# drscotthawley/flocoder

Hardware: AMD Instinct MI355X
Metric: latent samples/sec (64-step Euler, SD-VAE 4x32x32) (higher is better)
Workload: dtype f32; 1 GPU; flowers_sd.yaml shape: 64-step legacy Euler, batch 64 per GPU, latents 4x32x32, U-Net dim=32 dim_mults [1,2,4,8] n_classes=102, class-conditional, no CFG, ODE loop only (no VAE decode); global_batch=64, parallelism=sample-shard x1, weights broadcast once, plan_entries_per_forward=59, kernel_launches_per_forward=68, kernel_launches_per_euler_step=66, plan=exclusive device (cross-workgroup Block tails)

## Files before the change

### flocoder_amd/_binding.py

```python
from __future__ import annotations

import ctypes as C
import os
from typing import Optional

_HERE = os.path.dirname(os.path.abspath(__file__))
LIB_PATH = os.environ.get("FLOCODER_AMD_LIB") or os.path.join(_HERE, "_lib", "libflocoder_amd.so")

FC_OK, FC_E_ARG, FC_E_SHAPE, FC_E_ARCH, FC_E_HIP, FC_E_STATE = 0, -1, -2, -3, -4, -5
FC_METHOD_EULER, FC_METHOD_RK4 = 0, 1
FC_JACOBIAN_IDENTITY, FC_JACOBIAN_EXACT = 0, 1
FC_SDE_EULER_MARUYAMA, FC_SDE_HEUN = 0, 1
FC_LL_MAX_PROBES = 64
FC_PROBE_RADEMACHER, FC_PROBE_GAUSSIAN = 0, 1
FC_HIST_LDS_BINS = 8192
TILE_AUTO = -1
TILES = {"M128N32": 0, "M128N64": 1, "M64N32K2": 2, "M32N32K4": 3, "M64N64K2": 4, "M256N64": 5}


class fc_unet_config(C.Structure):
    _fields_ = [("dim", C.c_int), ("channels", C.c_int), ("n_levels", C.c_int), ("dim_mults", C.c_int * 8),
                ("groups", C.c_int), ("n_classes", C.c_int), ("mask_cond", C.c_int)]


_vp, _i, _f, _i64 = C.c_void_p, C.c_int, C.c_float, C.c_int64
_pi, _pf = C.POINTER(C.c_int), C.POINTER(C.c_float)

SIGNATURES = {
    "fc_abi_version": (_i, []),
    "fc_last_error": (C.c_char_p, []),
    "fc_check_device": (_i, [_i]),
    "fc_unet_create": (_i, [C.POINTER(fc_unet_config), _i, C.POINTER(_vp)]),
    "fc_unet_destroy": (None, [_vp]),
    "fc_unet_param_count": (_i, [_vp]),
    "fc_unet_param_info": (_i, [_vp, _i, C.POINTER(C.c_char_p), C.POINTER(_i64 * 4), C.POINTER(_i64)]),
    "fc_unet_param_numel": (_i64, [_vp]),
    "fc_unet_load_params": (_i, [_vp, _vp, _i64, _i, _vp]),
    "fc_unet_reserve": (_i, [_vp, _i, _i, _i]),
    "fc_unet_reserved": (_i, [_vp, _pi, _pi, _pi]),
    "fc_unet_forward": (_i, [_vp, _vp, _vp, _vp, _vp, _i, _vp, _i, _i, _i, _vp]),
    "fc_unet_integrate": (_i, [_vp, _i, _vp, _i, _i, _i, _pf, _i, _f, _f, _vp, _f, _vp, _i, _vp]),
    "fc_unet_integrate_rk45": (_i, [_vp, _vp, _i, _i, _i, C.c_double, C.c_double, C.c_double, C.c_double, _f, _vp, _f, _vp, _i, _pi, _vp]),
    "fc_unet_integrate_rk45_per_sample": (_i, [_vp, _vp, _i, _i, _i, C.c_double, C.c_double, C.c_double, C.c_double, _f, _vp, _f, _vp, _i,
                                              _pi, _vp]),
    "fc_unet_integrate_rk45_dense": (_i, [_vp, _i, _vp, _i, _i, _i, C.c_double, C.c_double, C.c_double, C.c_double, _f, _vp, _f, _vp, _i,
                                         C.POINTER(C.c_double), _i, _vp, _pi, _vp]),
    "fc_unet_chains": (_i, [_vp, _pi]),
    "fc_unet_plan_launches": (_i, [_vp]),
    "fc_unet_flops_per_sample": (C.c_double, [_vp]),
    "fc_unet_op_info": (_i, [_vp, _i, C.POINTER(C.c_char_p), C.POINTER(C.c_char_p), C.POINTER(C.c_double)]),
    "fc_unet_profile_ops": (_i, [_vp, _i, _i, _pf, _i, _vp]),
    "fc_unet_set_time_freqs": (_i, [_vp, _pf, _i]),
    "fc_unet_debug_tensor": (_i, [_vp, C.c_char_p, C.POINTER(_vp), _pi, _pi, _pi]),
    "fc_debug_copy": (_i, [_vp, _vp, _i64, _vp]),
    "fc_debug_set_poison": (_i, [_i]),
    "fc_debug_poison_check": (_i, [_pi, _pi]),
    "fc_debug_set_conv_stamps": (_i, [_vp]),
    "fc_debug_set_stamp_op": (_i, [_i, _vp]),
    "fc_debug_conv_routes": (_i, [_i]),
    "fc_debug_conv_routes_read": (_i, [C.c_char_p, _i]),
    "fc_debug_linattn_routes_read": (_i, [C.c_char_p, _i]),
    "fc_debug_conv": (_i, [_vp, _i, _vp, _i, _vp, _vp, _vp, _vp, _vp, _i, _pi, _pf, _i, _i, _i, _i, _i, _i, _i, _i, _i, _i, _i, _pf, _vp]),
    "fc_debug_set_fused_tail": (_i, [_i]),
    "fc_unet_fused_tail_errors": (_i, [_vp, C.POINTER(_i)]),
    "fc_unet_set_shared": (_i, [_vp, _i]),
    "fc_unet_meeting_launches": (_i, [_vp]),
    "fc_unet_check": (_i, [_vp, _vp, _i]),
    "fc_debug_unet_break_meeting": (_i, [_vp]),
    "fc_debug_unet_break_meeting_kind": (_i, [_vp, _i]),
    "fc_unet_train_reserve": (_i, [_vp, _i, _i, _i]),
    "fc_unet_backward": (_i, [_vp, _vp, _vp, _vp, _vp, _vp, _i64, _i, _i, _i, _vp]),
    "fc_unet_backward_ex": (_i, [_vp, _vp, _vp, _vp, _vp, _i, _vp, _vp, _i64, _vp, _vp, _i, _i, _i, _vp]),
    "fc_unet_backward_parts": (_i, [_vp, _vp, _vp, _vp, _vp, _i, _vp, _vp, _i64, _vp, _vp, _i, _i, _i, _i, _i, _vp]),
    "fc_unet_backward_accumulate": (_i, [_vp, _vp, _vp, _vp, _vp, _i, _vp, _vp, _i64, _vp, _vp, _i, _i, _i, _i, _i, _vp]),
    "fc_unet_grad_buckets": (_i, [_vp, C.POINTER(_i64)]),
    "fc_unet_set_grad_buckets": (_i, [_vp, _i]),
    "fc_unet_backward_launches": (_i, [_vp]),
    "fc_unet_backward_op_info": (_i, [_vp, _i, C.POINTER(C.c_char_p), C.POINTER(C.c_char_p)]),
    "fc_unet_vjp_x": (_i, [_vp, _vp, _vp, _vp, _vp, _i, _vp, _vp, _i, _i, _i, _vp]),
    "fc_unet_vjp_launches": (_i, [_vp]),
    "fc_unet_train_form": (_i, [_vp]),
    "fc_unet_train_release": (_i, [_vp]),
    "fc_unet_vjp_op_info": (_i, [_vp, _i, C.POINTER(C.c_char_p), C.POINTER(C.c_char_p)]),
    "fc_unet_log_likelihood": (_i, [_vp, _vp, _i, _i, _i, _pf, _i, _f, _vp, _vp, _i, _vp, _vp, _vp, _vp]),
    "fc_unet_log_likelihood_rk45": (_i, [_vp, _vp, _i, _i, _i, C.c_double, C.c_double, C.c_double, C.c_double, _f, _vp, _vp, _i, _vp, _i, _vp,
                                         _vp, _pi, _vp]),
    "fc_unet_log_likelihood_probes": (_i, [_vp, _vp, _i, _i, _i, _pf, _i, _f, _vp, _vp, _i, _vp, _i, _vp, _vp, _vp, _vp, _vp]),
    "fc_unet_log_likelihood_rk45_probes": (_i, [_vp, _vp, _i, _i, _i, C.c_double, C.c_double, C.c_double, C.c_double, _f, _vp, _vp, _i, _vp,
                                                _i, _i, _vp, _vp, _vp, _vp, _pi, _vp]),
    "fc_ode_probe_field": (_i, [_vp, _i, C.c_uint64, _i64, _vp, _i, _i64, _vp]),
    "fc_debug_probe_dot": (_i, [_vp, _vp, _vp, _i, _i64, _vp]),
    "fc_unet_integrate_guided": (_i, [_vp, _vp, _i, _i, _i, _pf, _i, _f, _vp, _f, _vp, _i, _vp, _vp, _f, _f, _i, _vp]),
    "fc_ode_guided_correct": (_i, [_vp, _vp, _vp, _vp, _i64, _f, _f, _f, _vp, _vp]),
    "fc_unet_integrate_sde": (_i, [_vp, _i, _vp, _i, _i, _i, _pf, _i, _f, _vp, _f, _vp, _i, _f, C.c_uint64, _vp, _vp, _vp]),
    "fc_ode_normal_field": (_i, [_vp, C.c_uint64, _i64, _vp, _i, _i64, _vp]),
    "fc_inpaint_masks": (_i, [_vp, _vp, C.c_uint64, _vp, _i, _i, _i, _pi, C.POINTER(C.c_double), _i, _i, _vp]),
    "fc_augment_images": (_i, [_vp, _vp, _vp, _i, _vp, _i, _i, _pf, _pf, _pf, _vp]),
    "fc_augment_midi": (_i, [_vp, _vp, _vp, _i, _vp, _i, _i, _i, _i, _f, _vp]),
    "fc_note_confusion": (_i, [_vp, _i, _vp, _i, _vp, _i, _i, _i, _f, C.c_double, _i, C.c_double, _i, _i, _vp, _vp, _vp, _vp, _vp]),
    "fc_index_histogram": (_i, [_vp, _i64, _i, _i, _vp, _vp, _vp, _vp]),
    "fc_debug_unet_guided_buffers": (_i, [_vp, C.POINTER(_vp), C.POINTER(_vp), C.POINTER(_vp), C.POINTER(_vp)]),
    "fc_unet_arena_serial": (C.c_uint64, [_vp]),
    "fc_unet_class_param_range": (_i, [_vp, C.POINTER(_i64), C.POINTER(_i64)]),
    "fc_flow_interp": (_i, [_vp, _vp, _vp, _vp, _vp, _i, _i64, _vp]),
    "fc_flow_prepare": (_i, [_vp, _vp, _vp, _vp, _f, _f, _f, _vp, _i, _vp, _vp, _vp, _vp, _vp, _i, _i64, _vp]),
    "fc_flow_prepare_rows": (_i, [_vp, _vp, _vp, _vp, _f, _f, _f, _vp, _i, _vp, _vp, _vp, _vp, _vp, _i, _i, _i, _i64, _vp]),
    "fc_mse_loss_grad_scaled": (_i, [_vp, _vp, _vp, _vp, _vp, _i64, _f, _vp]),
    "fc_mse_loss_grad": (_i, [_vp, _vp, _vp, _vp, _vp, _i64, _vp]),
    "fc_grad_clip_coef": (_i, [_vp, _i64, _vp, _i64, C.c_float, _vp, _vp, _vp]),
    "fc_adam_ema_step": (_i, [_vp, _vp, _vp, _vp, _vp, _i64, _vp, C.c_float, C.c_float, C.c_float, C.c_float, _i, C.c_float, _i, _vp]),
    "fc_adam_ema_step_guarded": (_i, [_vp, _vp, _vp, _vp, _vp, _i64, _vp, C.c_float, C.c_float, C.c_float, C.c_float, _i, C.c_float, _i, _vp, _vp]),
    "fc_debug_conv_wgrad": (_i, [_vp, _i, _vp, _i, _vp, _i, _i, _i, _i, _i, _i, _i, _i, _vp, _vp, _vp]),
    "fc_debug_conv_wgrad_ex": (_i, [_vp, _i, _vp, _i, _vp, _i, _i, _i, _i, _i, _i, _i, _i, _vp, _vp, _i, _i, _pi, _pi, _pi, _vp]),
    "fc_vae_create": (_i, [_i, C.POINTER(_vp)]),
# ... 101 lines not shown
```

### flocoder_amd/csrc/common.h

```cpp
#pragma once
#include <hip/hip_runtime.h>
#include <stdint.h>
#include <string>
#include <vector>

#include "../../include/flocoder_amd.h"

namespace fc {

void set_error(const std::string& msg);
int fail(int code, const std::string& msg);

#define FC_HIP(expr)                                                                              \
    do {                                                                                          \
        hipError_t _e = (expr);                                                                   \
        if (_e != hipSuccess)                                                                     \
            return ::fc::fail(FC_E_HIP, std::string(#expr) + ": " + hipGetErrorString(_e));       \
    } while (0)

#define FC_TRY(expr)                \
    do {                            \
        int _r = (expr);            \
        if (_r != FC_OK) return _r; \
    } while (0)

int dev_alloc(void** out, size_t bytes, const char* tag);
void dev_free(void* p);

static inline int ilog2(int v) { int l = 0; while ((1 << l) < v) ++l; return l; }
static inline bool is_pow2(int v) { return v > 0 && (v & (v - 1)) == 0; }
static inline int cdiv(int a, int b) { return (a + b - 1) / b; }

struct StatsRef {
    float* p = nullptr;
    int G = 0, T = 0;
    float n_t = 0.f;
};

struct SrcXform {
    int mode = 0;
    const float* stats = nullptr;
    int G = 1, T = 1;
    float n_t = 1.f;
    const float* gamma = nullptr;
    const float* beta = nullptr;
    const float* ss = nullptr;
    int ss_stride = 0;
    float eps = 1e-5f;
};

struct ConvSrc {
    const float* p = nullptr;
    int C = 0;
    SrcXform xf;
};

struct ConvFin {
    const float* gamma = nullptr;
    const float* beta = nullptr;
    float eps = 1e-5f;
    const float* res = nullptr;
    float* gn1_out = nullptr;
    unsigned* sync = nullptr;
    unsigned long long* gran = nullptr;
    int* err = nullptr;
};

struct ConvArgs {
    ConvSrc s0, s1;
    const float* w = nullptr;
    const float* bias = nullptr;
    float* out = nullptr;
    int out_act = 0;
    const float* add = nullptr;
    float* stats_out = nullptr;
    int Gout = 0;
    int stats_post = 0;
    const float* res_w = nullptr;
    const float* res_b = nullptr;
    float* res_out = nullptr;
    int B = 0, H = 0, W = 0;
    int Hs = 0, Ws = 0;
    int Cin = 0, Cout = 0;
    int KS = 1, pad = 0, stride = 1, ups = 0;
    int w_batch_stride = 0;
    const float* w4 = nullptr;
    const float* res_w4 = nullptr;
    const float* w_b3 = nullptr;
    int pad_y = -1, pad_x = -1;
    int out_sh = 0, out_oy = 0, out_ox = 0;
    int stats_tmul = 1, stats_toff = 0;
    int par4 = 0;
    int split_long_k = 0;
    int prec = 0;
    ConvFin fin;
};

enum ConvTile { TILE_AUTO = -1, TILE_M128N32 = 0, TILE_M128N64 = 1, TILE_M64N32K2 = 2, TILE_M32N32K4 = 3, TILE_M64N64K2 = 4,
                TILE_M256N64 = 5, TILE_COUNT = 6 };

struct ConvGeom {
    int tile = 0, grid = 0, T = 0, pipe = 0;
    float n_t = 0.f;
    size_t lds = 0;
    int T1 = 0;
    float n_t1 = 0.f;
    int groups = 0;
    int fin_local = 0;
};
bool conv_fin_possible(const ConvArgs& a, int tile);
int conv_init();
unsigned long long* conv_stamp_buffer();
void conv_set_stamp_buffer(unsigned long long* p);
void conv_route_log_set(bool on);
std::string conv_route_log_get();
int conv_plan(const ConvArgs& a, int tile, ConvGeom* g);
int conv_launch(const ConvArgs& a, int tile, hipStream_t s);

struct FinalizeArgs {
    const float* h = nullptr;
    SrcXform xf;
    const float* res = nullptr;
    SrcXform xf_res;
    int act_after_add = 0;
    float* y = nullptr;
    float* stats_out = nullptr;
    int B = 0, HW = 0, C = 0;
};
int finalize_blocks_per_sample(int HW, int C);
int finalize_launch(const FinalizeArgs& a, hipStream_t s);
size_t finalize_lds_bytes(const FinalizeArgs& a);
int finalize_table_launch(const FinalizeArgs* jobs_dev, const int* bps_dev, const int2* blocks_dev, int nblocks, size_t lds_bytes, hipStream_t s);
int gn_stats_launch(const float* x_nhwc, float* stats , int B, int HW, int C, int G, hipStream_t s);
int gn_fold_launch(const float* in, float* out, int B, int G, int T, float n_t, hipStream_t s);

struct CondFetch {
    const float* all = nullptr;
    const int* evalc = nullptr;
    float* dst = nullptr;
    int n4 = 0;
};

int init_conv_launch(const CondFetch& fetch, const float* x_nchw, int x_batch_mod, const float* w , const float* bias, float* out_nhwc,
                     int B, int Cin, int HW, int Cout, hipStream_t s);
struct EulerTail {
    int* evalc = nullptr;
    float* y = nullptr;
    float dt = 0.f;
    int* step = nullptr;
    const float* ts = nullptr;
    float t_scale = 1.f;
    float* sc = nullptr;
    float* tvec = nullptr;
    int rows = 0;
};
int final_conv_launch(const float* x_nhwc, const float* w , const float* bias, float* out_nchw, int B, int Cin,
                      int HW, int Cout, const EulerTail& tail, hipStream_t s);
int nchw_to_nhwc_launch(const float* src, float* dst, int B, int C, int HW, int Cpad, int src_batch_mod, hipStream_t s);
int nhwc_to_nchw_launch(const float* src, float* dst, int B, int C, int HW, int Cpad, hipStream_t s);
int pixel_shuffle2_nhwc_launch(const float* src, float* dst, int B, int H, int W, int C, hipStream_t s);
int bilinear_nhwc_launch(const float* src, float* dst, int B, int C, int Hs, int Ws, int Hd, int Wd, hipStream_t s);

struct TembArgs {
    const float* time = nullptr;
    const int64_t* class_ids = nullptr;
    int class_batch_mod = 0;
    int null_from = 0;
    int rows_per_eval = 0;
    const float* freqs = nullptr;
    const float *w1t, *b1, *w2t, *b2;
    const float *emb, *cw1t, *cb1, *cw2t, *cb2;
    int n_classes = 0;
    float* t_out = nullptr;
    int B = 0, dim = 0, td = 0;
};
int temb_init();
int temb_launch(const TembArgs& a, float* h, float* c1, hipStream_t s);
int ss_launch(const float* t, const float* wt, const float* bias, float* ss, int B, int td, int S, hipStream_t s);

int linattn_ctx_launch(const float* qkv, float* ctx , int B, int n, int heads, hipStream_t s);
int linattn_apply_launch(const float* qkv, const float* ctx, float* out , int B, int n, int heads,
                         hipStream_t s);
struct LaArgs {
    const float* x = nullptr;
    SrcXform xf;
    const float* wqkv = nullptr;
    const float* wout = nullptr;
    const float* wqkv4 = nullptr;
    const float* bout = nullptr;
    float* ctx = nullptr;
    float* y = nullptr;
    float* stats_out = nullptr;
    int B = 0, n = 0, C = 0, heads = 4;
    const float* g2 = nullptr;
    const float* b2 = nullptr;
    float eps2 = 1e-5f;
    float* out = nullptr;
    float* part = nullptr;
    unsigned long long* gran = nullptr;
    unsigned* sync = nullptr;
    int* err = nullptr;
};
int linattn_fused_init();
bool linattn_fused_supported(int n, int C, int heads);
int linattn_fused_tiles(int n);
float linattn_fused_nt(int n, int C);
int linattn_fused_launch(const LaArgs& a, hipStream_t s);
void linattn_route_log_set(bool on);
std::string linattn_route_log_get();
bool linattn_fused_meeting_ok(int B, int n, int C);
int linattn_sample_init();
bool linattn_sample_supported(int n, int C, int heads);
int linattn_sample_launch(const LaArgs& a, hipStream_t s);
bool attn_sample_supported(int n, int C, int heads);
int attn_sample_launch(const LaArgs& a, hipStream_t s);
int rope_attn_launch(const float* x, const float* wq, const float* bq, const float* wk, const float* bk, const float* wv, const float* bv,
                     const float* wo, const float* bo, float* out, int B, int n, int C, int Cr, hipStream_t s);
int attn_small_launch(const float* qkv, float* out, int B, int n, int heads, hipStream_t s);

int na2d_launch(const float* qkv, float* out, const float* gamma, int B, int H, int W, int C, int heads, int ksize, int mode, hipStream_t s);

int ode_all_times_launch(const float* ts, int n_steps, int rk4 , float t_scale, float* tv_out, hipStream_t s);
int ode_time_launch(int* step, const float* ts, float t_scale, int rk4, float* sc, float* tvec, int rows, hipStream_t s);
int ode_euler_update_launch(float* x, const float* v2, int n, int cfg_on, float cfg, float dt, hipStream_t s);
struct Rk4Guide { const float *gsc, *xin, *ym, *keep, *q; int tcur; };
int ode_rk4_stage_launch(const float* sc, const float* y, float* xs, float* k_out, const float* v2, int n, int cfg_on, float cfg,
                         int full, int tsel, float t_scale, float* tvec, int rows, const Rk4Guide* g, hipStream_t s);
int ode_rk4_final_launch(const float* sc, float* y, const float* k1, const float* k2, const float* k3, const float* v2, int n,
                         int cfg_on, float cfg, const Rk4Guide* g, hipStream_t s);
int ode_guide_w_launch(const float* sc, const float* gsc, const float* v, const float* xin, const float* ym, const float* keep, float* w,
                       int n, int tcur, hipStream_t s);
int ode_guided_correct_launch(const float* v, const float* x, const float* ym, const float* keep, float* out, int n, float t, float s2,
                              float gamma, hipStream_t s);
int ode_ll_stage_launch(const float* sc, const float* y, float* xs, float* k_out, const float* v, const float* g, const float* eps,
                        double* dst, int slot, int B, int m, int full, int tsel, float t_scale, float* tvec, int K, hipStream_t s);
int ode_ll_final_launch(const float* sc, float* y, const float* k1, const float* k2, const float* k3, const float* v, const float* g,
                        const float* eps, const double* dst, double* a, int B, int m, int K, hipStream_t s);
int ode_ll_logp_launch(const float* z, const double* a, double* logp, int B, int m, hipStream_t s);
int ode_ll_dot_launch(const float* eps, const float* g, double* out, double* dk, int B, int m, int K, hipStream_t s);
int ode_ll_mean_launch(const double* ak, int K, int B, double* abar, double* se, int mean_given, hipStream_t s);
int ode_probe_normal_field_launch(float* out, unsigned long long seed, unsigned probe, const int64_t* sids, int n, int m, hipStream_t s);
int ode_rademacher_field_launch(float* out, unsigned long long seed, unsigned probe, const int64_t* sids, int n, int m, hipStream_t s);
struct SdeParams { unsigned long long seed; const float* noise; };
int ode_sde_update_launch(const int* step, const float* ts, const SdeParams* prm, const int64_t* sids, float* y, float* xs, float* b1,
                          const float* v2, int n, int m, int cfg_on, float cfg, float sigma, int stage, int use_noise, float t_scale,
                          float* tvec, int rows, hipStream_t s);
int ode_normal_field_launch(float* out, unsigned long long seed, unsigned draw, const int64_t* sids, int n, int m, hipStream_t s);
int ode_iota_launch(int64_t* ids, int B, hipStream_t s);

struct Rk45State {
    double t, t_new, t_bound, dir, h, h_abs, rtol, atol, h0, d1, err, t_old;
    int nfev, accepted, rejected, attempts, done, failed, step_rejected, accepted_last, max_attempts, ev_cursor, ev_first, ev_end;
};
struct Rk45K { float* k[7]; };
struct Rk45Eval { float* frames; int n_eval, pad; };
__host__ __device__ inline const double* rk45_eval_times(const Rk45Eval* ev) { return reinterpret_cast<const double*>(ev + 1); }
struct Rk45Status { int unfinished, failed, pad0, pad1; };
struct Rk45Groups { int G, spg, m, chunks; };
struct Rk45LL { double *a, *d; int B; int K = 1; double *dk = nullptr, *ak = nullptr; };
int rk45_chunks(int m, int cap);
int rk45_setup_launch(const Rk45Groups& g, const float* x, double* y, float* xs, Rk45State* st, double t0, double t1, double rtol,
                      double atol, int max_attempts, float t_scale, float* tvec, int cfg_on, hipStream_t s);
// ... 136 lines not shown
```

### flocoder_amd/csrc/conv_dev.h

```cpp
#pragma once
#include "common.h"

namespace fc {

typedef float f32x16 __attribute__((ext_vector_type(16)));
typedef __attribute__((address_space(1))) unsigned long long gu64;
typedef __attribute__((address_space(1))) unsigned gu32;

struct ConvDev {
    ConvArgs a;
    int TWl, THl, TB, PH, PW, P;
    int tiles_x, tiles_y, ntiles, nblocks;
    int cpg, cpgt, NPG, rps;
    int gsz, o_fin;
    int fin_local;
    int act0, act1, any_xf;
    int o_pixoff, o_pixtb, o_gstat, o_aff, o_patch, o_wl, o_wres, o_red, o_part;
    int txl, tyl;
    unsigned magic_nt;
    int loader_prio;
    int o_out;
    int o_epoch, o_gran;
    const float* zeros16;
    int patch_stride, wl_stride;
// ... 12 lines not shown
        }
    }
}

struct TileInfo { int BM, BN, CC, WK, MTNT, WMWN; };

__device__ __forceinline__ int fastdiv(int x, unsigned magic) { return magic ? (int)__umulhi((unsigned)x, magic) : x; }

__device__ __forceinline__ float silu_f(float z) { return z / (1.0f + __expf(-z)); }
__device__ __forceinline__ void lds_only_barrier() { asm volatile("s_waitcnt lgkmcnt(0)\n\ts_barrier" ::: "memory"); }

__device__ __forceinline__ int xcd_remap(int bid, int nwg) {
    const int q = nwg >> 3, r = nwg & 7, xcd = bid & 7;
    return (xcd < r ? xcd * (q + 1) : r * (q + 1) + (xcd - r) * q) + (bid >> 3);
}
__device__ __forceinline__ int conv_parity_select(ConvDev& p, int bid) {
    if (!p.a.par4) return bid;
    const int nb1 = p.nblocks >> 2, par = bid >= 2 * nb1 ? (bid >= 3 * nb1 ? 3 : 2) : (bid >= nb1 ? 1 : 0);
    p.a.w += (size_t)par * 4 * p.a.Cin * p.a.Cout;
    if (p.a.w_b3) p.a.w_b3 += (size_t)par * 4 * (16 * p.nchunks) * p.a.Cout;
    p.a.pad_y = 1 - (par >> 1); p.a.pad_x = 1 - (par & 1);
    p.a.out_oy = par >> 1; p.a.out_ox = par & 1;
    p.a.stats_toff = par;
    return bid - par * nb1;
}


template <class T>
__device__ __forceinline__ T* as_global(T* q) {
    typedef __attribute__((address_space(1))) T* gp;
    return (T*)(gp)(size_t)q;
}
__device__ __forceinline__ void conv_params_from_lanes(ConvDev& p) {
    constexpr int ND = (int)(sizeof(ConvDev) / 4);
    static_assert(sizeof(ConvDev) % 4 == 0 && ND <= 256, "ConvDev must fit four lane-loads");
    const unsigned* ka = (const unsigned*)as_global((const unsigned*)__builtin_amdgcn_kernarg_segment_ptr());
    const int lane = threadIdx.x & 63;
    unsigned w[(ND + 63) / 64];
#pragma unroll
    for (int j = 0; j < (ND + 63) / 64; ++j) w[j] = (64 * j + lane < ND) ? ka[64 * j + lane] : 0u;
    unsigned* d = reinterpret_cast<unsigned*>(&p);
#pragma unroll
    for (int i = 0; i < ND; ++i) d[i] = __builtin_amdgcn_readlane(w[i / 64], i % 64);
    ConvArgs& a = p.a;
    a.s0.p = as_global(a.s0.p); a.s0.xf.stats = as_global(a.s0.xf.stats); a.s0.xf.gamma = as_global(a.s0.xf.gamma);
    a.s0.xf.beta = as_global(a.s0.xf.beta); a.s0.xf.ss = as_global(a.s0.xf.ss);
    a.s1.p = as_global(a.s1.p); a.s1.xf.stats = as_global(a.s1.xf.stats); a.s1.xf.gamma = as_global(a.s1.xf.gamma);
    a.s1.xf.beta = as_global(a.s1.xf.beta); a.s1.xf.ss = as_global(a.s1.xf.ss);
    a.w4 = as_global(a.w4); a.res_w4 = as_global(a.res_w4);
    a.w = as_global(a.w); a.bias = as_global(a.bias); a.out = as_global(a.out); a.add = as_global(a.add);
    a.stats_out = as_global(a.stats_out); a.res_w = as_global(a.res_w); a.res_b = as_global(a.res_b); a.res_out = as_global(a.res_out);
    a.fin.gamma = as_global(a.fin.gamma); a.fin.beta = as_global(a.fin.beta); a.fin.res = as_global(a.fin.res);
    a.fin.gn1_out = as_global(a.fin.gn1_out); a.fin.sync = as_global(a.fin.sync); a.fin.gran = as_global(a.fin.gran); a.fin.err = as_global(a.fin.err);
    p.zeros16 = as_global(p.zeros16); p.stamps = as_global(p.stamps);
}

constexpr int FL_FIN = 1, FL_RES = 2, FL_POST = 4, FL_XF = 8, FL_CAT = 16, FL_STAMP = 32, FL_STATS = 64, FL_GN1 = 128, FL_POSTOP = 256,
              FL_NARROW = 512, FL_MULTI = 1024, FL_MEET = 2048, FL_ALL = 4095, FL_W4 = 4096;
constexpr int FL_WW = 8192;
constexpr int GEO_PAIR = 1, GEO_FAST = 2;
constexpr int geo_log2(int v) { return v <= 1 ? 0 : 1 + geo_log2(v >> 1); }
constexpr int geo_key(int form, int TB, int TW, int cpg, int Tst) { return form | ((TB == 2 ? 1 : 0) << 2) | (geo_log2(TW) << 3) | (geo_log2(cpg) << 6) | (Tst << 10); }
constexpr int geo_form(int k) { return k & 3; }
constexpr int geo_TB(int k) { return 1 + ((k >> 2) & 1); }
constexpr int geo_TWl(int k) { return (k >> 3) & 7; }
constexpr int geo_cpg(int k) { return 1 << ((k >> 6) & 15); }
constexpr int geo_Tst(int k) { return (k >> 10) & 63; }
constexpr bool geo_conv1_mask(int FL) { return (FL & ~(FL_W4 | FL_STAMP)) == FL_STATS || (FL & ~(FL_W4 | FL_STAMP)) == (FL_STATS | FL_CAT | FL_RES); }

template <int WM, int WN, int WK, int MT, int NT, int FL = FL_ALL, int GEO = 0>
__device__ __forceinline__ void conv_epilogue(const ConvDev& p, f32x16 (&acc)[MT][NT], f32x16 (&accr)[MT][NT], float* smem, int tid, int lane,
                                              int wave, int b0, int y0, int x0, int n0, int tx, int ty, bool active = true,
                                              int nthr = 256, const float* pre = nullptr, bool staged_dead = false) {
    constexpr int BM = 32 * MT * WM, BN = 32 * NT * WN;
    const ConvArgs& a = p.a;
    const int half = lane >> 5, l31 = lane & 31;
    const int wk = wave % WK, wn = (wave / WK) % WN, wm = wave / (WK * WN);
    constexpr bool GEOC = GEO != 0;
    constexpr bool GEO1 = GEOC && !(FL & FL_FIN);
    static_assert(!GEOC || (FL != FL_ALL && (FL & FL_STATS) && !(FL & (FL_MULTI | FL_POST)) && ((FL & FL_FIN) ? !(FL & FL_RES) : geo_conv1_mask(FL))),
                  "a geometry key belongs to a lean Block-closing flavour or to a lean conv1 flavour");
    static_assert(!GEOC || geo_Tst(GEO) >= 1, "statistics slots of the key");
    static_assert(!GEOC || GEO1 || geo_TB(GEO) * (geo_cpg(GEO) >= BN ? 1 : BN / geo_cpg(GEO)) * geo_Tst(GEO) * 2 <= 512, "one granule per thread");
    const int g_TB = GEOC ? geo_TB(GEO) : p.TB;
    const int g_TWl = GEOC ? geo_TWl(GEO) : p.TWl;
    const int g_tbsh = GEOC ? geo_log2(BM / geo_TB(GEO)) : p.TWl + p.THl;
    const int g_THl = GEOC ? geo_log2(BM / geo_TB(GEO)) - geo_TWl(GEO) : p.THl;
    const int g_rps = GEOC ? BM / geo_TB(GEO) : p.rps;
    const int g_cpg = GEOC ? geo_cpg(GEO) : p.cpg;
    const int g_cpgt = GEOC ? (geo_cpg(GEO) < BN ? geo_cpg(GEO) : BN) : p.cpgt;
    const int g_NPG = GEOC ? (geo_cpg(GEO) >= BN ? geo_cpg(GEO) / BN : 1) : p.NPG;
    const int g_mt = GEOC ? (geo_TB(GEO) > 1 ? 1 : geo_Tst(GEO) / (geo_cpg(GEO) >= BN ? geo_cpg(GEO) / BN : 1)) : (p.TB > 1 ? 1 : p.tiles_x * p.tiles_y);
    const int TW = 1 << g_TWl, TH = 1 << g_THl, Cout = a.Cout;
    constexpr bool LEAN = FL != FL_ALL;
    const bool has_res = LEAN ? bool(FL & FL_RES) : a.res_out != nullptr;
    const bool stats_post = (FL & FL_POST) && a.stats_post;
    if (WK > 1) {
        if (!staged_dead) __syncthreads();
        float* red = smem + p.o_red;
        constexpr int TILE = 16 * 64;
        const int slot = ((wm * WN + wn) * (WK - 1) + (wk - 1)) * MT * NT * (has_res ? 2 : 1);
        if (active && wk > 0) {
#pragma unroll
            for (int mt = 0; mt < MT; ++mt)
#pragma unroll
                for (int nt = 0; nt < NT; ++nt) {
                    float* d = red + (size_t)(slot + mt * NT + nt) * TILE + lane;
#pragma unroll
                    for (int r = 0; r < 16; ++r) d[r * 64] = acc[mt][nt][r];
                    if (has_res) {
                        float* dr = red + (size_t)(slot + MT * NT + mt * NT + nt) * TILE + lane;
#pragma unroll
                        for (int r = 0; r < 16; ++r) dr[r * 64] = accr[mt][nt][r];
                    }
                }
        }
        __syncthreads();
        if (active && wk == 0) {
            for (int k2 = 1; k2 < WK; ++k2) {
                const int sl = ((wm * WN + wn) * (WK - 1) + (k2 - 1)) * MT * NT * (has_res ? 2 : 1);
#pragma unroll
                for (int mt = 0; mt < MT; ++mt)
#pragma unroll
                    for (int nt = 0; nt < NT; ++nt) {
                        const float* d = red + (size_t)(sl + mt * NT + nt) * TILE + lane;
#pragma unroll
// ... 132 lines not shown
        }
    };
    constexpr bool CAN_MULTI = (FL & FL_MULTI) || (WM * MT == 1);
    const bool fast_stats = GEOC ? geo_form(GEO) == GEO_FAST : (!CAN_MULTI || p.TB == 1);
    constexpr bool PAIR_TILE = (WM * MT == 1 && WN * NT == 1);
    const bool pair_stats = GEOC ? geo_form(GEO) == GEO_PAIR : (PAIR_TILE && p.TB == 2 && p.rps == 16);
    static_assert(!GEOC || geo_form(GEO) == GEO_FAST || (geo_form(GEO) == GEO_PAIR && PAIR_TILE && geo_TB(GEO) == 2), "statistics form of the key");
    auto stats_pair = [&](float* dst, int G, int cpg, int cpgt, int NPG, bool coherent, bool ltab, bool whole = false) {
        if (owner) {
            float s0 = 0.f, q0 = 0.f, s1 = 0.f, q1 = 0.f;
#pragma unroll
            for (int r = 0; r < 8; ++r) { const float v = acc[0][0][r], w = acc[0][0][r + 8]; s0 += v; q0 += v * v; s1 += w; q1 += w * w; }
            s0 += __shfl_xor(s0, 32); q0 += __shfl_xor(q0, 32); s1 += __shfl_xor(s1, 32); q1 += __shfl_xor(q1, 32);
            for (int o = cpgt >> 1; o > 0; o >>= 1) {
                s0 += __shfl_xor(s0, o); q0 += __shfl_xor(q0, o); s1 += __shfl_xor(s1, o); q1 += __shfl_xor(q1, o);
            }
            const int ncols = min(BN, Cout - n0);
            if (half == 0 && (l31 & (cpgt - 1)) == 0 && l31 < ncols) {
                if (b0 < a.B) publish(dst, G, cpg, cpgt, NPG, coherent, ltab, 0, l31 / cpgt, s0, q0, whole);
                if (b0 + 1 < a.B) publish(dst, G, cpg, cpgt, NPG, coherent, ltab, 1, l31 / cpgt, s1, q1, whole);
            }
        }
    };

    if (owner) {
#pragma unroll
        for (int mt = 0; mt < MT; ++mt)
#pragma unroll
            for (int nt = 0; nt < NT; ++nt) {
                const int ncol = (wn * NT + nt) * 32 + l31, n = n0 + ncol;
                const bool nok = n < Cout;
                const float bias = pre ? pre[nt] : ((a.bias && nok) ? a.bias[n] : 0.f);
#pragma unroll
                for (int r = 0; r < 16; ++r) acc[mt][nt][r] += bias;
                if (stats_post) {
                    float ad[16];
                    const bool addp = a.add && nok;
#pragma unroll
                    for (int r = 0; r < 16; ++r) {
                        const int px = pix_of(mt, r);
                        ad[r] = (addp && px >= 0) ? a.add[(size_t)px * Cout + n] : 0.f;
                    }
#pragma unroll
                    for (int r = 0; r < 16; ++r) {
                        float v = acc[mt][nt][r];
                        if (a.out_act) v = silu_f(v);
                        acc[mt][nt][r] = v + ad[r];
                    }
                }
            }
    }
    if (do_stats && !fast_stats && !pair_stats) block_sums();

    if (FL & FL_STAMP) conv_stamp(p, 7);
    if (do_stats) {
        if (pair_stats) stats_pair(a.stats_out, a.Gout, g_cpg, g_cpgt, g_NPG, meeting, fin && !meeting);
        else if (fast_stats) stats_fast(a.stats_out, a.Gout, g_cpg, g_cpgt, g_NPG, meeting, fin && !meeting);
        else {
            __syncthreads();
            emit(a.stats_out, a.Gout, p.cpg, p.cpgt, p.NPG, meeting, fin && !meeting);
        }
    }
    if (FL & FL_STAMP) conv_stamp(p, 14);

    if (fin) {
        float* tab = smem + p.o_fin;
        const int ngt = g_cpg >= BN ? 1 : BN / g_cpg;
        float rs[MT][NT][16];
        if (owner) {
#pragma unroll
            for (int mt = 0; mt < MT; ++mt)
#pragma unroll
                for (int nt = 0; nt < NT; ++nt) {
                    const int n = n0 + (wn * NT + nt) * 32 + l31;
                    const bool nok = n < Cout;
#pragma unroll
                    for (int r = 0; r < 16; ++r) {
                        const int px = pix_of(mt, r);
                        rs[mt][nt][r] = (a.fin.res && nok && px >= 0) ? a.fin.res[(size_t)px * Cout + n] : 0.f;
                    }
                }
        }
        if (meeting) {
            const int Tst = GEOC ? geo_Tst(GEO) : (p.TB > 1 ? 1 : p.tiles_x * p.tiles_y) * p.NPG;
            const int cnt = g_TB * ngt * Tst * 2;
            float* gv = smem + p.o_gran;
            for (int i = tid; i < cnt; i += nthr) {
                const int k = i & 1, t = (i >> 1) % Tst, j = (i >> 1) / Tst, tb = j / ngt, gl = j - tb * ngt;
                const int b = b0 + tb, g = n0 / g_cpg + gl;
                float val = 0.f;
                if (b < a.B && g < a.Gout) {
                    const gu64* gp = (const gu64*)(a.fin.gran + ((size_t)(b * a.Gout + g) * Tst + t) * 2 + k);
                    unsigned long long v = __hip_atomic_load(gp, __ATOMIC_RELAXED, __HIP_MEMORY_SCOPE_AGENT);
                    int spins = 0;
                    while ((unsigned)(v >> 32) != epoch) {
                        if (++spins > (1 << 20)) { if (a.fin.err) *a.fin.err = 1; v = 0x7fc00000ull; break; }
                        __builtin_amdgcn_s_sleep(2);
                        v = __hip_atomic_load(gp, __ATOMIC_RELAXED, __HIP_MEMORY_SCOPE_AGENT);
                    }
                    val = __uint_as_float((unsigned)v);
                }
                gv[i] = val;
                if (GEOC) break;
            }
            lds_only_barrier();
            for (int i = tid; i < g_TB * ngt; i += nthr) {
                const int tb = i / ngt, gl = i - tb * ngt, b = b0 + tb, g = n0 / g_cpg + gl;
                float mean = 0.f, rstd = 0.f;
                if (b < a.B && g < a.Gout) {
                    const float* sp = gv + (size_t)i * Tst * 2;
                    const float nt_ = (float)(g_rps * g_cpgt);
                    float sm = 0.f;
                    for (int t = 0; t < Tst; ++t) sm += sp[2 * t];
                    mean = sm / (float)Tst;
                    float m2 = 0.f, dv = 0.f;
                    for (int t = 0; t < Tst; ++t) {
                        const float d = sp[2 * t] - mean;
                        m2 += sp[2 * t + 1];
                        dv += d * d;
                    }
                    rstd = 1.0f / sqrtf((m2 + nt_ * dv) / (nt_ * (float)Tst) + a.fin.eps);
                }
                tab[2 * i] = mean;
                tab[2 * i + 1] = rstd;
                if (GEOC) break;
            }
        }
        lds_only_barrier();
        if ((FL & FL_STAMP) && active) conv_stamp(p, 12);
        if (owner) {
#pragma unroll
            for (int mt = 0; mt < MT; ++mt)
#pragma unroll
                for (int nt = 0; nt < NT; ++nt) {
                    const int ncol = (wn * NT + nt) * 32 + l31, n = n0 + ncol;
                    const bool nok = n < Cout;
                    const int gl = g_cpg >= BN ? 0 : ncol / g_cpg;
                    const float gam = pre ? pre[2 * NT + nt] : (nok ? a.fin.gamma[n] : 0.f), bet = pre ? pre[3 * NT + nt] : (nok ? a.fin.beta[n] : 0.f);
#pragma unroll
                    for (int r = 0; r < 16; ++r) {
                        const int m = (wm * MT + mt) * 32 + (r & 3) + 8 * (r >> 2) + 4 * half;
                        const int tb = m >> g_tbsh;
                        const float mean = tab[2 * (tb * ngt + gl)], rstd = tab[2 * (tb * ngt + gl) + 1];
                        const float A = rstd * gam;
                        const float v = silu_f(A * acc[mt][nt][r] + (bet - mean * A)) + rs[mt][nt][r];
                        acc[mt][nt][r] = (nok && b0 + tb < a.B) ? v : 0.f;
                    }
                }
        }
        if ((FL & FL_STAMP) && active) conv_stamp(p, 2);
        if (LEAN ? bool(FL & FL_GN1) : a.fin.gn1_out != nullptr) {
            lds_only_barrier();
            const int cpg1 = Cout, cpgt1 = GEOC ? BN : (Cout < BN ? Cout : BN), NPG1 = GEOC ? p.ntiles : (Cout >= BN ? Cout / BN : 1);
            if (pair_stats) stats_pair(a.fin.gn1_out, 1, cpg1, cpgt1, NPG1, false, false, GEOC);
            else if (fast_stats) stats_fast(a.fin.gn1_out, 1, cpg1, cpgt1, NPG1, false, false, GEOC);
            else {
                block_sums();
                lds_only_barrier();
                emit(a.fin.gn1_out, 1, cpg1, cpgt1, NPG1, false, false);
            }
        }
        if ((FL & FL_STAMP) && active) conv_stamp(p, 13);
    }

    const bool post = !stats_post && !fin;
    const bool act = (FL & FL_POSTOP) && post && a.out_act;
    const float* addp = ((FL & FL_POSTOP) && post) ? a.add : nullptr;
    if (owner) {
#pragma unroll
        for (int mt = 0; mt < MT; ++mt) {
            int pix[16];
#pragma unroll
            for (int r = 0; r < 16; ++r) pix[r] = pix_of(mt, r);
#pragma unroll
            for (int nt = 0; nt < NT; ++nt) {
                const int ncol = (wn * NT + nt) * 32 + l31, n = n0 + ncol;
                if (n >= Cout) continue;
                float* op = a.out + n;
                if (addp) {
                    float ad[16];
#pragma unroll
                    for (int r = 0; r < 16; ++r) ad[r] = pix[r] >= 0 ? addp[(size_t)pix[r] * Cout + n] : 0.f;
#pragma unroll
                    for (int r = 0; r < 16; ++r) acc[mt][nt][r] = (act ? silu_f(acc[mt][nt][r]) : acc[mt][nt][r]) + ad[r];
                } else if (act) {
#pragma unroll
                    for (int r = 0; r < 16; ++r) acc[mt][nt][r] = silu_f(acc[mt][nt][r]);
                }
                if (!LEAN && p.o_out < 0) {
#pragma unroll
                    for (int r = 0; r < 16; ++r)
                        if (pix[r] >= 0) op[(size_t)pix[r] * Cout] = acc[mt][nt][r];
                    if (has_res) {
                        const float rbias = pre ? pre[NT + nt] : (a.res_b ? a.res_b[n] : 0.f);
                        float* rp = a.res_out + n;
#pragma unroll
                        for (int r = 0; r < 16; ++r)
                            if (pix[r] >= 0) rp[(size_t)pix[r] * Cout] = accr[mt][nt][r] + rbias;
                    }
                }
            }
        }
    }
    if ((FL & FL_STAMP) && active) conv_stamp(p, 3);
    if (LEAN || p.o_out >= 0) {
        constexpr int OS = BN + 4, Q4 = BN / 4;
        float* ot = smem + p.o_out;
        for (int pass = 0; pass < (has_res ? 2 : 1); ++pass) {
            if (pass) lds_only_barrier();
            if (owner) {
#pragma unroll
                for (int mt = 0; mt < MT; ++mt)
#pragma unroll
                    for (int nt = 0; nt < NT; ++nt) {
                        const int ncol = (wn * NT + nt) * 32 + l31;
                        const float rbias = pass ? (pre ? pre[NT + nt] : ((a.res_b && n0 + ncol < Cout) ? a.res_b[n0 + ncol] : 0.f)) : 0.f;
#pragma unroll
                        for (int r = 0; r < 16; ++r) {
                            const int m = (wm * MT + mt) * 32 + (r & 3) + 8 * (r >> 2) + 4 * half;
                            ot[m * OS + ncol] = pass ? accr[mt][nt][r] + rbias : acc[mt][nt][r];
                        }
                    }
            }
            if (active && !pass) conv_stamp(p, 9);
            lds_only_barrier();
            if (active && !pass) conv_stamp(p, 10);
            float* gout = pass ? a.res_out : a.out;
            for (int i = tid; i < BM * Q4; i += nthr) {
                const int m = i / Q4, c4 = (i - m * Q4) * 4, n = n0 + c4;
                const int tw = m & (TW - 1), th = (m >> g_TWl) & (TH - 1), tb = m >> g_tbsh;
                const int b = b0 + tb;
                if (GEO1) {
                    if (b < a.B) *reinterpret_cast<float4*>(gout + (size_t)((b * a.H + y0 + th) * a.W + x0 + tw) * Cout + n) = *reinterpret_cast<const float4*>(ot + m * OS + c4);
                } else if (b < a.B && n < Cout) {
                    const float4 v = *reinterpret_cast<const float4*>(ot + m * OS + c4);
                    *reinterpret_cast<float4*>(gout + (size_t)((b * (a.H << a.out_sh) + ((y0 + th) << a.out_sh) + a.out_oy) * (a.W << a.out_sh) + ((x0 + tw) << a.out_sh) + a.out_ox) * Cout + n) = v;
                }
            }
        }
    }
    if (FL & FL_STAMP) conv_stamp(p, 8);
}

int conv_pipe_launch(const ConvDev& d, int tile, int grid, size_t lds, hipStream_t s);
int conv_pipe_blocks_per_cu(const ConvDev& d, int tile, size_t lds);
int conv_pipe_init();
bool conv_pipe_supports_ks(int ks);
const float* conv_zeros16();

}
```

### flocoder_amd/csrc/conv_igemm.hip

```cpp
#include <cstdlib>
#include <string>

#include "conv_dev.h"

namespace fc {

template <int WM, int WN, int WK, int MT, int NT, int CC>
__global__ void __launch_bounds__(256) conv_igemm_kernel(const ConvDev p) {
    constexpr int BN = 32 * NT * WN, CS = CC + 1, KSTEPS = CC / 2, KPW = KSTEPS / WK, Q = CC / 4;
    static_assert(WM * WN * WK == 4, "4 waves per workgroup");
    extern __shared__ __attribute__((aligned(16))) float smem[];
    const ConvArgs& a = p.a;
    int* pixoff = reinterpret_cast<int*>(smem + p.o_pixoff);
    int* pixtb = reinterpret_cast<int*>(smem + p.o_pixtb);
    float* gstat = smem + p.o_gstat;
    float2* aff = reinterpret_cast<float2*>(smem + p.o_aff);
    float* patch = smem + p.o_patch;
    float* wl = smem + p.o_wl;
    float* wres = smem + p.o_wres;

    const int tid = threadIdx.x, lane = tid & 63, wave = tid >> 6;
    const int half = lane >> 5, l31 = lane & 31;
    const int wk = wave % WK, wn = (wave / WK) % WN, wm = wave / (WK * WN);

// ... 245 lines not shown
        p.NPG = p.cpg >= t.BN ? p.cpg / t.BN : 1;
        g->T = (TB > 1 ? 1 : p.tiles_x * p.tiles_y) * p.NPG;
        g->n_t = (float)(p.rps * p.cpgt);
    }
    g->pipe = pipe ? 1 : 0;
    if (pipe) {
        if (!conv_pipe_supports_ks(a.KS)) return fail(FC_E_SHAPE, "conv: kernel size not instantiated in the pipelined kernel");
        if (p.P * (t.CC / 4) > (a.KS == 1 ? 256 : kPipeLoaderThreads[tile]) * kPipeNPL) return fail(FC_E_SHAPE, "conv: patch too large for the pipelined kernel");
        const int G0 = a.s0.xf.mode ? a.s0.xf.G : 0, G1 = a.s1.xf.mode ? a.s1.xf.G : 0;
        int o = 0;
        p.o_pixoff = p.o_pixtb = 0;
        p.o_epoch = o; o += 4;
        p.o_gstat = o; o += align4(2 * TB * (G0 + G1));
        p.o_aff = o; o += p.any_xf ? align4(2 * TB * a.Cin) : 0;
        p.o_patch = o;
        const bool direct_b = (t.WMWN == 1 && t.MTNT == 1 && a.KS == 3);
        p.bf3 = (a.prec == 1 && a.w_b3 && (tile == TILE_M128N32 || tile == TILE_M128N64 || tile == TILE_M256N64) && (a.KS == 1 || a.KS == 2 || a.KS == 3) && !a.res_out &&
                 !a.fin.gamma && !a.w_batch_stride) ? 1 : 0;
        p.patch_stride = align4(p.P * (t.CC + ((direct_b || p.bf3) ? 4 : 1)));
        p.o_wl = o + 2 * p.patch_stride;
        p.wl_stride = direct_b ? 0 : a.KS * a.KS * t.CC * t.BN + (a.res_out ? t.CC * t.BN : 0);
        p.o_wres = 0;
        p.nchunks = cdiv(a.Cin, t.CC);
        p.nwb = (p.nchunks >= 3 && (size_t)(o + 2 * p.patch_stride + 3 * p.wl_stride) * sizeof(float) <= 160 * 1024) ? 3 : 2;
        const int main_sz = 2 * p.patch_stride + p.nwb * p.wl_stride;
        int epi = 0;
        p.o_red = o;
        if (t.WK > 1) epi = t.WMWN * (t.WK - 1) * t.MTNT * (a.res_out ? 2 : 1) * 1024;
        p.o_part = o + epi;
        if (a.stats_out) epi += 2 * (t.BM / 16) * t.BN + 2 * TB * t.BN;
        p.o_fin = o + epi;
        if (a.fin.gamma) epi += 2 * TB * t.BN;
        p.o_gran = o + epi;
        if (a.fin.gamma) epi += align4(TB * (p.cpg >= t.BN ? 1 : t.BN / p.cpg) * g->T * 2);
        p.o_out = -1;
        if ((size_t)(o + epi + t.BM * (t.BN + 4)) * sizeof(float) <= 160 * 1024) { p.o_out = o + epi; epi += t.BM * (t.BN + 4); }
        o += main_sz > epi ? main_sz : epi;
        p.zeros16 = conv_zeros16();
        p.stamps = conv_stamp_buffer();
        p.loader_prio = 1;
        g->tile = tile; g->grid = p.nblocks; g->lds = (size_t)o * sizeof(float);
        if (g->lds > 160 * 1024) return fail(FC_E_SHAPE, "conv: tile does not fit in LDS");
        p.gsz = 1; p.fin_local = 0;
        if (a.fin.gamma) {
            if (!a.stats_out || a.stats_post || a.out_act || a.add || a.res_out) return fail(FC_E_ARG, "conv: fused tail excludes act / add / res outputs");
            if (a.Cout % t.BN && a.Cout > t.BN) return fail(FC_E_SHAPE, "conv: fused tail needs Cout to fill its column tiles");
            p.gsz = p.tiles_x * p.tiles_y * p.ntiles;
            g->groups = cdiv(a.B, TB);
            const int cpgt1 = a.Cout < t.BN ? a.Cout : t.BN, NPG1 = a.Cout >= t.BN ? a.Cout / t.BN : 1;
            g->T1 = (TB > 1 ? 1 : p.tiles_x * p.tiles_y) * NPG1;
            g->n_t1 = (float)(p.rps * cpgt1);
            p.fin_local = g->fin_local = (g->T == 1) ? 1 : 0;
            if (p.fin_local) p.gsz = 1;
            else {
                int per_cu = conv_pipe_blocks_per_cu(p, tile, g->lds);
                if (per_cu <= 0) return fail(FC_E_SHAPE, "conv: fused tail: occupancy of the kernel unknown");
                if (per_cu > 2) per_cu = 2;
                if (p.nblocks > conv_cu_count() * per_cu) return fail(FC_E_SHAPE, "conv: fused tail needs the whole grid resident");
            }
        }
        return FC_OK;
    }
    if (a.fin.gamma) return fail(FC_E_SHAPE, "conv: fused tail is implemented in the pipelined kernel only");
    if (tile == TILE_M256N64) return fail(FC_E_SHAPE, "conv: M256N64 exists in the pipelined kernel only");
    int o = 0;
    p.o_pixoff = o; o += align4(p.P);
    p.o_pixtb = o; o += align4(p.P);
    const int G0 = a.s0.xf.mode ? a.s0.xf.G : 0, G1 = a.s1.xf.mode ? a.s1.xf.G : 0;
    p.o_gstat = o; o += align4(2 * TB * (G0 + G1));
    p.o_aff = o; o += align4(2 * TB * t.CC);
    p.o_patch = o;
    int main_sz = align4(p.P * (t.CC + 1));
    p.o_wl = o + main_sz; main_sz += a.KS * a.KS * t.CC * t.BN;
    p.o_wres = o + main_sz; if (a.res_out) main_sz += t.CC * t.BN;
    int epi = 0;
    p.o_red = o;
    if (t.WK > 1) epi = t.WMWN * (t.WK - 1) * t.MTNT * (a.res_out ? 2 : 1) * 1024;
    p.o_part = o + epi;
    if (a.stats_out) epi += 2 * (t.BM / 16) * t.BN + 2 * TB * t.BN;
    o += main_sz > epi ? main_sz : epi;
    g->tile = tile; g->grid = p.nblocks; g->lds = (size_t)o * sizeof(float);
    if (g->lds > 160 * 1024) return fail(FC_E_SHAPE, "conv: tile does not fit in LDS");
    return FC_OK;
}

bool conv_fin_possible(const ConvArgs& a, int tile) {
    ConvDev d;
    ConvGeom g;
    ConvArgs b = a;
    if (!b.fin.gamma) b.fin.gamma = reinterpret_cast<const float*>(16);
    if (!b.stats_out) b.stats_out = reinterpret_cast<float*>(16);
    return conv_geometry(b, tile, true, &d, &g) == FC_OK;
}

static int auto_tile(const ConvArgs& a) {
    const long M = (long)a.B * a.H * a.W;
    const int hw = a.H * a.W;
    auto blocks = [&](int t) { return (M / kTiles[t].BM) * cdiv(a.Cout, kTiles[t].BN) * (a.par4 ? 4 : 1); };
    auto ok = [&](int t) { return !(a.w_batch_stride && hw < kTiles[t].BM) && M >= kTiles[t].BM; };
    if (a.split_long_k && hw <= 16 && (long)a.Cin * a.KS * a.KS >= 2048 && ok(TILE_M32N32K4)) return TILE_M32N32K4;
    if (a.Cout >= 64 && ok(TILE_M256N64) && blocks(TILE_M256N64) >= 512) {
        ConvDev d;
        ConvGeom g;
        if (conv_geometry(a, TILE_M256N64, true, &d, &g) == FC_OK) return TILE_M256N64;
    }
    if (a.par4) {
        if (ok(TILE_M128N32) && blocks(TILE_M128N32) >= 512) return TILE_M128N32;
        if (ok(TILE_M64N32K2) && blocks(TILE_M64N32K2) >= 512) return TILE_M64N32K2;
        return TILE_M32N32K4;
    }
    if ((a.KS == 1 || a.Cout >= 512) && a.Cout >= 64 && ok(TILE_M128N64) && blocks(TILE_M128N64) >= 512) return TILE_M128N64;
    if (ok(TILE_M128N32) && blocks(TILE_M128N32) >= 256) return TILE_M128N32;
    if (a.Cout >= 64 && ok(TILE_M64N64K2) && blocks(TILE_M64N64K2) >= 384) return TILE_M64N64K2;
    if (ok(TILE_M64N32K2) && blocks(TILE_M64N32K2) >= 256) return TILE_M64N32K2;
    return TILE_M32N32K4;
}

static unsigned long long* g_stamps = nullptr;
unsigned long long* conv_stamp_buffer() { return g_stamps; }
void conv_set_stamp_buffer(unsigned long long* p) { g_stamps = p; }

static int geometry_best(const ConvArgs& a, int tile, ConvDev* d, ConvGeom* g) {
    if (conv_geometry(a, tile, true, d, g) == FC_OK) return FC_OK;
    return conv_geometry(a, tile, false, d, g);
}

int conv_plan(const ConvArgs& a, int tile, ConvGeom* g) {
    ConvDev d;
    if (tile == TILE_AUTO) tile = auto_tile(a);
    return geometry_best(a, tile, &d, g);
}

template <int WM, int WN, int WK, int MT, int NT, int CC>
static int launch_t(const ConvDev& d, const ConvGeom& g, hipStream_t s) {
    hipLaunchKernelGGL((conv_igemm_kernel<WM, WN, WK, MT, NT, CC>), dim3(g.grid), dim3(256), g.lds, s, d);
    FC_HIP(hipGetLastError());
    return FC_OK;
}

template <int WM, int WN, int WK, int MT, int NT, int CC>
static int allow_big_lds() {
    FC_HIP(hipFuncSetAttribute(reinterpret_cast<const void*>(&conv_igemm_kernel<WM, WN, WK, MT, NT, CC>),
                               hipFuncAttributeMaxDynamicSharedMemorySize, 160 * 1024));
    return FC_OK;
}

int conv_init() {
// ... 37 lines not shown
```

### flocoder_amd/csrc/conv_pipe.hip

```cpp
#include <cstdlib>
#include <map>
#include <mutex>
#include <string>
#include <tuple>
#include "conv_dev.h"
#include "stats_dev.h"

namespace fc {

typedef __attribute__((address_space(3))) void* lptr_t;

__device__ __forceinline__ void lds_dma16(const float* gsrc, unsigned lds_byte) {
    const unsigned dst = __builtin_amdgcn_readfirstlane(lds_byte);
    unsigned keep;
    asm volatile("s_mov_b32 %0, m0\n\ts_mov_b32 m0, %2\n\ts_nop 0\n\tglobal_load_lds_dwordx4 %1, off\n\ts_mov_b32 m0, %0"
                 : "=&s"(keep) : "v"(gsrc), "s"(dst) : "memory");
}
typedef float f32x4 __attribute__((ext_vector_type(4)));
__device__ __forceinline__ void hidden_load16(f32x4& dst, const float* gsrc) {
    asm volatile("global_load_dwordx4 %0, %1, off" : "=v"(dst) : "v"(gsrc) : "memory");
}
__device__ __forceinline__ void wait_vmcnt(int n) {
    switch (__builtin_amdgcn_readfirstlane(n)) {
        case 0: asm volatile("s_waitcnt vmcnt(0)" ::: "memory"); break;
// ... 58 lines not shown
#ifndef FC_DB4_CHAINS
#define FC_DB4_CHAINS 2
#endif
    constexpr int DB4_CHAINS = FC_DB4_CHAINS;
    constexpr bool WW = (FL & FL_WW) != 0;
    static_assert(!WW || (DB4 && FL != FL_ALL && (FL & FL_FIN) && (FL & FL_XF) && !(FL & (FL_CAT | FL_RES))), "whole-window staging: register-fed Block-closing flavours");
    constexpr bool BF3 = PREC == 1;
    static_assert(!BF3 || (!DB && CC == 16 && FL == FL_ALL), "split-bf16: LDS-fed tiles, one 16-channel k-step per chunk, the all-in-one flavour");
    constexpr int CS = (DB4 || BF3) ? CC + 4 : CC + 1;
    extern __shared__ __attribute__((aligned(16))) float smem[];
    const ConvArgs& a = p.a;
    float* gstat = smem + p.o_gstat;
    float2* aff = reinterpret_cast<float2*>(smem + p.o_aff);
    float* patch0 = smem + p.o_patch;
    float* wl0 = smem + p.o_wl;
    const unsigned smem_lds = (unsigned)(size_t)(lptr_t)smem;

    const int tid = threadIdx.x, lane = tid & 63, wave8 = tid >> 6;
    const bool consumer = wave8 < 4;
    const int wave = wave8 & 3;
    const int lw = (wave8 - 4) & (NL - 1), ltid = (tid - 256) & (LT - 1);
    const int half = lane >> 5, l31 = lane & 31;
    const int wk = wave % WK, wn = (wave / WK) % WN, wm = wave / (WK * WN);

    constexpr bool GEOC = GEO != 0, GEO1 = GEOC && !(FL & FL_FIN);
    constexpr int G1_NT = GEO1 ? geo_cpg(GEO) * kFinGeomGroups / BN : 1;
    static_assert(!GEO1 || (KS == 3 && geo_conv1_mask(FL) && geo_cpg(GEO) * kFinGeomGroups % BN == 0), "conv1 geometry flavours: 3x3, whole column tiles");
    const int bid = GEO1 ? xcd_remap(blockIdx.x, p.nblocks) : conv_parity_select(p, xcd_remap(blockIdx.x, p.nblocks));
    const int mt_i = GEO1 ? bid / G1_NT : (p.ntiles == 1 ? bid : (p.magic_nt ? (int)__umulhi((unsigned)bid, p.magic_nt) : bid / p.ntiles));
    const int nt_i = bid - mt_i * (GEO1 ? G1_NT : p.ntiles);
    const int tx = mt_i & (p.tiles_x - 1), ty = (mt_i >> p.txl) & (p.tiles_y - 1), bg = mt_i >> (p.txl + p.tyl);
    constexpr int BM = 32 * MT * WM;
    static_assert(!GEOC || GEO1 || (!(FL & FL_CAT) && (FL & FL_XF) && geo_Tst(GEO) <= kPartPre), "Block-closing geometry flavours: transform loader, one source");
    const int g_TB = GEOC ? geo_TB(GEO) : p.TB;
    const int g_TWl = GEOC ? geo_TWl(GEO) : p.TWl;
    const int g_tbsh = GEOC ? geo_log2(BM / geo_TB(GEO)) : p.TWl + p.THl;
    const int g_THl = GEOC ? geo_log2(BM / geo_TB(GEO)) - geo_TWl(GEO) : p.THl;
    const int TW = 1 << g_TWl, TH = 1 << g_THl;
    const int b0 = bg * g_TB, y0 = ty * TH, x0 = tx * TW, n0 = nt_i * BN;
    constexpr int G1_PW = GEO1 ? (1 << geo_TWl(GEO)) + 2 : 1, G1_PHW = GEO1 ? (BM / geo_TB(GEO) / (1 << geo_TWl(GEO)) + 2) * G1_PW : 1;
    const int PW = GEO1 ? G1_PW : p.PW, PHW = GEO1 ? G1_PHW : p.PH * p.PW;
    const int C0 = a.s0.C, C1 = a.s1.C, Cin = a.Cin, Cout = a.Cout;
    constexpr bool LEAN = FL != FL_ALL;
    const bool has_res = LEAN ? bool(FL & FL_RES) : a.res_out != nullptr;
    const bool xf_on = LEAN ? bool(FL & FL_XF) : p.any_xf != 0;
    const int nchunks = p.nchunks;
    if (FL & FL_STAMP) conv_stamp(p, 0);
    const bool meet = LEAN ? bool(FL & FL_MEET) : (a.fin.gamma != nullptr && !p.fin_local);
    unsigned arrival = 0;
    if (meet && tid == 0) {
        const gu32* cnt = (const gu32*)(a.fin.sync + b0 / g_TB);
        asm volatile("global_atomic_add %0, %1, %2, off sc0" : "=v"(arrival) : "v"(cnt), "v"(1u) : "memory");
    }

    auto gn_tables = [&](const bool worker, const int id, const int nthr) {
      if (xf_on) {
        const int G0 = a.s0.xf.mode ? a.s0.xf.G : 0, G1 = ((FL & FL_CAT) && a.s1.xf.mode) ? a.s1.xf.G : 0;
        float pg = 1.f, pbt = 0.f, psc = 0.f, psh = 0.f;
        bool p_on = false, p_ss = false;
        int p_gs = 0;
       if (worker) {
        if (id < g_TB * Cin) {
            const int tb = GEOC ? ((geo_TB(GEO) > 1 && id >= Cin) ? 1 : 0) : id / Cin, c = id - tb * Cin, b = b0 + tb;
            const bool first = !(FL & FL_CAT) || c < C0;
            const SrcXform& xf = first ? a.s0.xf : a.s1.xf;
            if (b < a.B && xf.mode) {
                const int cs = first ? c : c - C0, Cs = first ? C0 : C1;
                p_on = true;
                p_gs = 2 * ((first ? 0 : p.TB * G0) + tb * xf.G + (GEOC ? cs / geo_cpg(GEO) : cs / (Cs / xf.G)));
                pg = xf.gamma[cs];
                pbt = xf.beta[cs];
                if (xf.ss) {
                    p_ss = true;
                    psc = xf.ss[(size_t)b * xf.ss_stride + cs];
                    psh = xf.ss[(size_t)b * xf.ss_stride + Cs + cs];
                }
            }
        }
        for (int i = id; i < g_TB * (G0 + G1); i += nthr) {
            const bool first = !(FL & FL_CAT) || i < p.TB * G0;
            const SrcXform& xf = first ? a.s0.xf : a.s1.xf;
            const int j = first ? i : i - p.TB * G0;
            const int tb = GEOC ? ((geo_TB(GEO) > 1 && j >= xf.G) ? 1 : 0) : j / xf.G, g = j - tb * xf.G, b = b0 + tb;
            float mean = 0.f, rstd = 0.f;
            if (b < a.B) {
                if constexpr (GEOC) combine_partials_fixed<geo_Tst(GEO)>(xf, b, g, &mean, &rstd);
                else combine_partials(xf, b, g, &mean, &rstd);
            }
            gstat[2 * i] = mean;
            gstat[2 * i + 1] = rstd;
            if (GEOC) break;
        }
       }
        if ((FL & FL_STAMP) && worker) conv_stamp(p, 2);
        lds_only_barrier();
        if ((FL & FL_STAMP) && worker) conv_stamp(p, 4);
       if (worker) {
        if (id < g_TB * Cin) {
            float A = 1.f, Bv = 0.f;
            if (p_on) {
                A = gstat[p_gs + 1] * pg;
                Bv = pbt - gstat[p_gs] * A;
                if (p_ss) {
                    const float sc = psc + 1.0f;
                    A *= sc;
                    Bv = Bv * sc + psh;
// ... 255 lines not shown
        __builtin_amdgcn_s_setprio(0);
      }
    } else {
        int abase[MT];
#pragma unroll
        for (int mt = 0; mt < MT; ++mt) {
            const int m = (wm * MT + mt) * 32 + l31;
            const int tw = m & (TW - 1), th = (m >> g_TWl) & (TH - 1), tb = m >> g_tbsh;
            const int st = GEO1 ? 1 : a.stride;
            abase[mt] = (tb * PHW + th * st * PW + tw * st) * CS + half;
        }
        const int bbase = half * BN + wn * NT * 32 + l31;
        const int kk0 = wk * KPW;
        const int abase4 = abase[0] - half + 8 * wk + 4 * half;
        unsigned long long dbg_cbar = 0;
        constexpr int NB = (DB && !DB4) ? KK * KPW : 1, NR = (DB && !DB4) ? KPW : 1;
        float wcur[NB], wnxt[NB], rcur[NR], rnxt[NR];
        const int ncol = n0 + l31;
        const bool colok = ncol < Cout;
        const float* wq = colok ? a.w + (size_t)b0 * a.w_batch_stride + ncol : p.zeros16;
        const float* rq = (colok && has_res) ? a.res_w + ncol : p.zeros16;
        const size_t wcs = colok ? (size_t)Cout : 0, wts = colok ? (size_t)Cin * Cout : 0;
        auto fetch_w = [&](int i, float (&w)[NB], float (&r)[NR]) {
#pragma unroll
            for (int kk = 0; kk < KPW; ++kk) {
                int c = i * CC + 2 * (kk0 + kk) + half;
                c = c < Cin ? c : Cin - 1;
                const float* q = wq + (size_t)c * wcs;
#pragma unroll
                for (int tap = 0; tap < KK; ++tap) w[tap * KPW + kk] = q[(size_t)tap * wts];
                if (has_res) r[kk] = rq[(size_t)c * wcs];
            }
        };
        constexpr int NQ = DB4 ? KK : 1;
        f32x4 wA[NQ], wB[NQ], rA, rB;
        const unsigned lane_off4 = DB4 ? (unsigned)(half * Cout + ncol) * 4u : 0u;
        const int wk_u = __builtin_amdgcn_readfirstlane(wk);
        auto fetch4 = [&](int i, f32x4 (&w)[NQ], f32x4& r) {
            const size_t blk = (size_t)((i * (CC / 8) + wk_u) * 2) * (size_t)Cout * 4;
            const float* ub = a.w4 + blk;
#pragma unroll
            for (int tap = 0; tap < NQ; ++tap) w[tap] = *reinterpret_cast<const f32x4*>(ub + (size_t)tap * ((size_t)Cin * Cout) + lane_off4);
            if (has_res) r = *reinterpret_cast<const f32x4*>(a.res_w4 + blk + lane_off4);
        };
        if (DB4) fetch4(0, wA, rA);
        else if (DB) fetch_w(0, wcur, rcur);
        if constexpr (WW) ww_request();
        if (FL & FL_STAMP) conv_stamp(p, 1);
        gn_tables(false, 0, 1);
        if constexpr (WW) ww_store();
        if (meet && tid == 0) {
            asm volatile("s_waitcnt vmcnt(0)" : "+v"(arrival) :: "memory");
            smem[p.o_epoch] = __uint_as_float(arrival / (unsigned)p.gsz + 1u);
        }
        __syncthreads();
        if (FL & FL_STAMP) conv_stamp(p, 4);
        f32x16 acc2;
#pragma unroll
        for (int r = 0; r < 16; ++r) acc2[r] = 0.f;
        if constexpr (DB4) {
            auto chunk = [&](int i, f32x4 (&wc)[NQ], f32x4& rc, f32x4 (&wn)[NQ], f32x4& rn) {
                const float* patch = patch0 + (WW ? i : (i & 1)) * p.patch_stride;
                fetch4(i + 1 < nchunks ? i + 1 : i, wn, rn);
                __builtin_amdgcn_sched_barrier(0);
                static_assert(!DB4 || KPW == 4, "one 16-byte operand read = the four k-steps of a wave");
                (void)patch;
                const unsigned pl = smem_lds + 4u * (unsigned)(p.o_patch + (WW ? i : (i & 1)) * p.patch_stride + abase4);
                const unsigned prow = 4u * (unsigned)(PW * CS);
                auto lds_quad = [&](f32x4& dst, int tapn) {
                    const unsigned ad = pl + (unsigned)(tapn / KS) * prow;
                    switch (tapn % KS) {
                        case 0: asm volatile("ds_read_b128 %0, %1" : "=v"(dst) : "v"(ad) : "memory"); break;
                        case 1: asm volatile("ds_read_b128 %0, %1 offset:%2" : "=v"(dst) : "v"(ad), "n"(4 * CS) : "memory"); break;
                        default: asm volatile("ds_read_b128 %0, %1 offset:%2" : "=v"(dst) : "v"(ad), "n"(8 * CS) : "memory"); break;
                    }
                };
                f32x4 av, an;
                lds_quad(av, 0);
                asm volatile("s_waitcnt lgkmcnt(0)" : "+v"(av) :: "memory");
                an = av;
#pragma unroll
                for (int tap = 0; tap < KK; ++tap) {
                    if (tap + 1 < KK || has_res) lds_quad(an, tap + 1 < KK ? tap + 1 : KK / 2);
                    __builtin_amdgcn_sched_barrier(0);
                    if (DB4_CHAINS == 2) {
                        acc[0][0] = __builtin_amdgcn_mfma_f32_32x32x2f32(av[0], wc[tap][0], acc[0][0], 0, 0, 0);
                        acc2 = __builtin_amdgcn_mfma_f32_32x32x2f32(av[1], wc[tap][1], acc2, 0, 0, 0);
                        acc[0][0] = __builtin_amdgcn_mfma_f32_32x32x2f32(av[2], wc[tap][2], acc[0][0], 0, 0, 0);
                        acc2 = __builtin_amdgcn_mfma_f32_32x32x2f32(av[3], wc[tap][3], acc2, 0, 0, 0);
                    } else {
#pragma unroll
                        for (int kk = 0; kk < KPW; ++kk) acc[0][0] = __builtin_amdgcn_mfma_f32_32x32x2f32(av[kk], wc[tap][kk], acc[0][0], 0, 0, 0);
                    }
                    __builtin_amdgcn_sched_barrier(0);
                    if (tap + 1 < KK || has_res) asm volatile("s_waitcnt lgkmcnt(0)" : "+v"(an) :: "memory");
                    av = an;
                }
                if (has_res) {
#pragma unroll
                    for (int kk = 0; kk < KPW; ++kk) accr[0][0] = __builtin_amdgcn_mfma_f32_32x32x2f32(av[kk], rc[kk], accr[0][0], 0, 0, 0);
                }
                if constexpr (!WW) {
                unsigned long long t0 = ((FL & FL_STAMP) && p.stamps) ? __builtin_amdgcn_s_memtime() : 0ull;
                loader_handover();
                if ((FL & FL_STAMP) && p.stamps) dbg_cbar += __builtin_amdgcn_s_memtime() - t0;
                }
// ... 49 lines not shown
            if (DB && i + 1 < nchunks) fetch_w(i + 1, wnxt, rnxt);
#pragma unroll
            for (int tap = 0; tap < KK; ++tap) {
                const int tapoff = ((tap / KS) * PW + (tap % KS)) * CS;
#pragma unroll
                for (int kk = 0; kk < KPW; ++kk) {
                    const int k = 2 * (kk0 + kk);
                    float av[MT], bv[NT];
#pragma unroll
                    for (int mt = 0; mt < MT; ++mt) av[mt] = patch[abase[mt] + tapoff + k];
#pragma unroll
                    for (int nt = 0; nt < NT; ++nt) bv[nt] = DB ? wcur[tap * KPW + kk] : wl[(tap * CC + k) * BN + nt * 32];
#pragma unroll
                    for (int mt = 0; mt < MT; ++mt)
#pragma unroll
                        for (int nt = 0; nt < NT; ++nt)
                            acc[mt][nt] = __builtin_amdgcn_mfma_f32_32x32x2f32(av[mt], bv[nt], acc[mt][nt], 0, 0, 0);
                }
            }
            if (has_res) {
                const int tapoff = GEO1 ? (PW + 1) * CS : (a.pad * PW + a.pad) * CS;
#pragma unroll
                for (int kk = 0; kk < KPW; ++kk) {
                    const int k = 2 * (kk0 + kk);
                    float av[MT], bv[NT];
#pragma unroll
                    for (int mt = 0; mt < MT; ++mt) av[mt] = patch[abase[mt] + tapoff + k];
#pragma unroll
                    for (int nt = 0; nt < NT; ++nt) bv[nt] = DB ? rcur[kk] : wl[(KK * CC + k) * BN + nt * 32];
#pragma unroll
                    for (int mt = 0; mt < MT; ++mt)
#pragma unroll
                        for (int nt = 0; nt < NT; ++nt)
                            accr[mt][nt] = __builtin_amdgcn_mfma_f32_32x32x2f32(av[mt], bv[nt], accr[mt][nt], 0, 0, 0);
                }
            }
            unsigned long long t0 = ((FL & FL_STAMP) && p.stamps) ? __builtin_amdgcn_s_memtime() : 0ull;
            if (DB) {
                loader_handover();
#pragma unroll
                for (int j = 0; j < NB; ++j) wcur[j] = wnxt[j];
#pragma unroll
                for (int j = 0; j < NR; ++j) rcur[j] = rnxt[j];
            } else {
                __syncthreads();
            }
            if ((FL & FL_STAMP) && p.stamps) dbg_cbar += __builtin_amdgcn_s_memtime() - t0;
        }
        }
        if ((FL & FL_STAMP) && p.stamps && lane == 0) p.stamps[((size_t)blockIdx.x * 8 + wave8) * 16 + 11] = dbg_cbar;
        if (FL & FL_STAMP) conv_stamp(p, 5);
    }
    if constexpr (WW) loader_handover();
    conv_epilogue<WM, WN, WK, MT, NT, FL, GEO>(p, acc, accr, smem, tid, lane, wave, b0, y0, x0, n0, tx, ty, consumer, NTHR, pre, true);
}

static float* g_zeros16 = nullptr;
const float* conv_zeros16() { return g_zeros16; }

#define FC_PIPE_TILES(X, KS)               \
    X(TILE_M128N32, 4, 1, 1, 1, 1, 16, KS, 4)  \
    X(TILE_M128N64, 4, 1, 1, 1, 2, 16, KS, 4)  \
    X(TILE_M64N32K2, 2, 1, 2, 1, 1, 32, KS, (KS == 1 ? 4 : 8)) \
    X(TILE_M32N32K4, 1, 1, 4, 1, 1, 32, KS, (KS == 1 ? 4 : 8)) \
    X(TILE_M64N64K2, 2, 1, 2, 1, 2, 16, KS, 4) \
    X(TILE_M256N64, 4, 1, 1, 2, 2, 16, KS, 4)

template <int KS>
static int pipe_attr_ks() {
#define X(T, WM, WN, WK, MT, NT, CC, K, NL)                                                                               \
    FC_HIP(hipFuncSetAttribute(reinterpret_cast<const void*>(&conv_pipe_kernel<WM, WN, WK, MT, NT, CC, 8, K, NL>),        \
                               hipFuncAttributeMaxDynamicSharedMemorySize, 160 * 1024));
    FC_PIPE_TILES(X, KS)
#undef X
    return FC_OK;
}

#define FC_LEAN_TILES(X, KS)               \
    X(TILE_M128N32, 4, 1, 1, 1, 1, 16, KS, 4)  \
    X(TILE_M64N32K2, 2, 1, 2, 1, 1, 32, KS, (KS == 1 ? 4 : 8)) \
    X(TILE_M32N32K4, 1, 1, 4, 1, 1, 32, KS, (KS == 1 ? 4 : 8))

#define FC_LEAN_FLAVOURS_3(X) X(0) X(FL_POSTOP) X(FL_STATS) X(FL_STATS | FL_STAMP) X(FL_STATS | FL_CAT | FL_STAMP) X(FL_STATS | FL_RES) X(FL_STATS | FL_CAT) X(FL_STATS | FL_RES | FL_CAT) X(FL_STATS | FL_XF) \
    X(FL_STATS | FL_XF | FL_FIN) X(FL_STATS | FL_XF | FL_FIN | FL_GN1) X(FL_STATS | FL_XF | FL_FIN | FL_MEET) X(FL_STATS | FL_XF | FL_FIN | FL_GN1 | FL_MEET) \
    X(FL_STATS | FL_XF | FL_FIN | FL_STAMP) X(FL_STATS | FL_XF | FL_FIN | FL_GN1 | FL_STAMP) X(FL_STATS | FL_XF | FL_FIN | FL_MEET | FL_STAMP) X(FL_STATS | FL_XF | FL_FIN | FL_GN1 | FL_MEET | FL_STAMP)
#define FC_LEAN_FLAVOURS_1(X) X(0) X(FL_POSTOP) X(FL_XF) X(FL_STATS) X(FL_STATS | FL_XF)

#define FC_LEAN_TILES_WIDE1(X)             \
    X(TILE_M128N64, 4, 1, 1, 1, 2, 16, 1, 4)   \
    X(TILE_M256N64, 4, 1, 1, 2, 2, 16, 1, 4)

constexpr int kLeanNPL = 4;
template <int KS, int FL>
static int lean_attr() {
#define X(T, WM, WN, WK, MT, NT, CC, K, NL)                                                                               \
    FC_HIP(hipFuncSetAttribute(reinterpret_cast<const void*>(&conv_pipe_kernel<WM, WN, WK, MT, NT, CC, kLeanNPL, K, NL, FL>),  \
                               hipFuncAttributeMaxDynamicSharedMemorySize, 160 * 1024));
    FC_LEAN_TILES(X, KS)
#undef X
    return FC_OK;
}

constexpr bool ww_flavour(int FL) { return (FL & FL_FIN) && (FL & FL_XF) && !(FL & (FL_CAT | FL_RES)); }
template <int FL>
static int lean_attr_db4() {
    FC_HIP(hipFuncSetAttribute(reinterpret_cast<const void*>(&conv_pipe_kernel<1, 1, 4, 1, 1, 32, kLeanNPL, 3, 8, FL | FL_W4>),
                               hipFuncAttributeMaxDynamicSharedMemorySize, 160 * 1024));
// ... 107 lines not shown
    const int cpg = d.cpg, NPG = cpg >= BN ? cpg / BN : 1, ngt = cpg >= BN ? 1 : BN / cpg;
    if (cpg < 1 || (cpg & (cpg - 1)) || cpg > (1 << 15) || d.cpgt != (cpg < BN ? cpg : BN) || d.NPG != NPG) return 0;
    const int Tst = (d.TB > 1 ? 1 : d.tiles_x * d.tiles_y) * NPG;
    if (Tst < 1 || Tst > kPartPre) return 0;
    if (a.Cout % BN || a.Cin != a.Cout || a.s0.xf.G <= 0 || a.s0.C != a.s0.xf.G * cpg || a.s0.xf.T != Tst) return 0;
    if (d.TB * a.Cin > nthr - 256 || d.TB * a.s0.xf.G > nthr - 256 || d.TB * ngt * Tst * 2 > nthr) return 0;
    return geo_key(form, d.TB, 1 << d.TWl, cpg, Tst);
}

template <int WM, int WN, int WK, int MT, int NT, int CC, int NL, int W4, int MEET, int GEO>
static int fin_geom_row_attr() {
#define Y(V) FC_HIP(hipFuncSetAttribute(reinterpret_cast<const void*>(&conv_pipe_kernel<WM, WN, WK, MT, NT, CC, kLeanNPL, 3, NL, kFinBase | W4 | MEET | (V), 0, GEO>), \
                                        hipFuncAttributeMaxDynamicSharedMemorySize, 160 * 1024));
    FC_FIN_VARIANTS(Y)
#undef Y
    if constexpr (W4 != 0) {
#define Y(V) FC_HIP(hipFuncSetAttribute(reinterpret_cast<const void*>(&conv_pipe_kernel<WM, WN, WK, MT, NT, CC, kLeanNPL, 3, NL, kFinBase | W4 | FL_WW | MEET | (V), 0, GEO>), \
                                        hipFuncAttributeMaxDynamicSharedMemorySize, 160 * 1024));
        FC_FIN_VARIANTS(Y)
#undef Y
    }
    return FC_OK;
}
static int fin_geom_attr() {
#define X(T, WM, WN, WK, MT, NT, CC, NL, W4, MEET, GEO) FC_TRY((fin_geom_row_attr<WM, WN, WK, MT, NT, CC, NL, W4, MEET, GEO>()));
    FC_FIN_GEOMS(X)
#undef X
    return FC_OK;
}

template <int WM, int WN, int WK, int MT, int NT, int CC, int NL, int W4, int MEET, int GEO>
static int fin_geom_row_launch(const ConvDev& d, int need, int grid, size_t lds, size_t lds_ww, hipStream_t s, int* occ) {
    if constexpr (W4 != 0) {
        if (lds_ww && d.a.Cin == kFinGeomGroups * geo_cpg(GEO)) {
#define Y(V) if (need == (kFinBase | MEET | (V))) return launch_pipe<WM, WN, WK, MT, NT, CC, kLeanNPL, 3, NL, kFinBase | W4 | FL_WW | MEET | (V), 0, GEO>(d, grid, lds_ww, s, occ);
            FC_FIN_VARIANTS(Y)
#undef Y
        }
    }
#define Y(V) if (need == (kFinBase | MEET | (V))) return launch_pipe<WM, WN, WK, MT, NT, CC, kLeanNPL, 3, NL, kFinBase | W4 | MEET | (V), 0, GEO>(d, grid, lds, s, occ);
    FC_FIN_VARIANTS(Y)
#undef Y
    return -1;
}

static int fin_geom_launch(const ConvDev& d, int tile, bool w4, int need, int grid, size_t lds, size_t lds_ww, hipStream_t s, int* occ) {
#define X(T, WM, WN, WK, MT, NT, CC, NL, W4, MEET, GEO)                                                         \
    if (tile == T && (w4 ? FL_W4 : 0) == (W4) && d.P * (CC / 4) <= 64 * NL * kLeanNPL &&                        \
        fin_geo_key(d, 32 * MT * WM, 32 * NT * WN, 256 + 64 * NL, WM * MT == 1 && WN * NT == 1) == (GEO))       \
        return fin_geom_row_launch<WM, WN, WK, MT, NT, CC, NL, W4, MEET, GEO>(d, need, grid, lds, lds_ww, s, occ);
    FC_FIN_GEOMS(X)
#undef X
    return -1;
}

constexpr int kConv1Up = FL_STATS | FL_CAT | FL_RES;
#define FC_CONV1_GEOMS(X)                                                                                    \
    X(TILE_M128N32, 4, 1, 1, 1, 1, 16, 4, 0, FL_STATS, geo_key(GEO_FAST, 1, 16, 8, 8))            \
    X(TILE_M128N32, 4, 1, 1, 1, 1, 16, 4, 0, kConv1Up, geo_key(GEO_FAST, 1, 16, 8, 8))       \
    X(TILE_M128N32, 4, 1, 1, 1, 1, 16, 4, 0, kConv1Up, geo_key(GEO_FAST, 1, 16, 16, 2))             \
    X(TILE_M64N32K2, 2, 1, 2, 1, 1, 32, 8, 0, FL_STATS, geo_key(GEO_FAST, 1, 16, 8, 4))           \
    X(TILE_M64N32K2, 2, 1, 2, 1, 1, 32, 8, 0, kConv1Up, geo_key(GEO_FAST, 1, 8, 32, 1))             \
    X(TILE_M32N32K4, 1, 1, 4, 1, 1, 32, 8, FL_W4, FL_STATS, geo_key(GEO_FAST, 1, 8, 16, 2))       \
    X(TILE_M32N32K4, 1, 1, 4, 1, 1, 32, 8, FL_W4, FL_STATS, geo_key(GEO_PAIR, 2, 4, 32, 1))       \
    X(TILE_M32N32K4, 1, 1, 4, 1, 1, 32, 8, FL_W4, FL_STATS, geo_key(GEO_PAIR, 2, 4, 64, 2))  \
    X(TILE_M32N32K4, 1, 1, 4, 1, 1, 32, 8, FL_W4, kConv1Up, geo_key(GEO_PAIR, 2, 4, 64, 2))

static int conv1_geo_key(const ConvDev& d, int BM, int BN, bool pair_tile) {
    const ConvArgs& a = d.a;
    if (a.fin.gamma || !a.stats_out || a.stats_post || a.par4 || a.stats_tmul != 1 || a.stats_toff != 0 || d.any_xf || a.out_act || a.add || d.o_out < 0) return 0;
    if (a.KS != 3 || a.stride != 1 || a.ups || a.pad != 1 || a.pad_y >= 0 || a.pad_x >= 0 || a.out_sh || a.out_oy || a.out_ox || a.Hs != a.H || a.Ws != a.W) return 0;
    if (d.TB != 1 && d.TB != 2) return 0;
    if (d.rps != BM / d.TB || (1 << (d.TWl + d.THl)) * d.TB != BM) return 0;
    const int form = (pair_tile && d.TB == 2 && d.rps == 16) ? GEO_PAIR : (d.TB == 1 ? GEO_FAST : 0);
    if (!form) return 0;
    const int cpg = d.cpg, NPG = cpg >= BN ? cpg / BN : 1;
    if (cpg < 1 || (cpg & (cpg - 1)) || cpg > (1 << 15) || d.cpgt != (cpg < BN ? cpg : BN) || d.NPG != NPG) return 0;
    const int Tst = (d.TB > 1 ? 1 : d.tiles_x * d.tiles_y) * NPG;
    if (Tst < 1 || Tst > 63) return 0;
    if (a.Gout != kFinGeomGroups || a.Cout != kFinGeomGroups * cpg || a.Cout % BN || d.ntiles != a.Cout / BN) return 0;
    const int TW = 1 << d.TWl, TH = 1 << d.THl;
    if (d.PW != TW + 2 || d.PH != TH + 2 || d.P != d.TB * d.PH * d.PW) return 0;
    return geo_key(form, d.TB, TW, cpg, Tst);
}

static int conv1_geom_attr() {
#define X(T, WM, WN, WK, MT, NT, CC, NL, W4, MASK, GEO)                                                                                            \
    FC_HIP(hipFuncSetAttribute(reinterpret_cast<const void*>(&conv_pipe_kernel<WM, WN, WK, MT, NT, CC, kLeanNPL, 3, NL, (MASK) | (W4), 0, 0, GEO>),    \
                               hipFuncAttributeMaxDynamicSharedMemorySize, 160 * 1024));                                                           \
    FC_HIP(hipFuncSetAttribute(reinterpret_cast<const void*>(&conv_pipe_kernel<WM, WN, WK, MT, NT, CC, kLeanNPL, 3, NL, (MASK) | (W4) | FL_STAMP, 0, 0, GEO>), \
                               hipFuncAttributeMaxDynamicSharedMemorySize, 160 * 1024));
    FC_CONV1_GEOMS(X)
#undef X
    return FC_OK;
}

static int conv1_geom_launch(const ConvDev& d, int tile, bool w4, int need, int grid, size_t lds, hipStream_t s, int* occ) {
#define X(T, WM, WN, WK, MT, NT, CC, NL, W4, MASK, GEO)                                                                                        \
    if (tile == T && (w4 ? FL_W4 : 0) == (W4) && (need & ~FL_STAMP) == (MASK) && d.P * (CC / 4) <= 64 * NL * kLeanNPL &&                       \
        conv1_geo_key(d, 32 * MT * WM, 32 * NT * WN, WM * MT == 1 && WN * NT == 1) == (GEO))                                                   \
        return (need & FL_STAMP) ? launch_pipe<WM, WN, WK, MT, NT, CC, kLeanNPL, 3, NL, (MASK) | (W4) | FL_STAMP, 0, 0, GEO>(d, grid, lds, s, occ) \
                                 : launch_pipe<WM, WN, WK, MT, NT, CC, kLeanNPL, 3, NL, (MASK) | (W4), 0, 0, GEO>(d, grid, lds, s, occ);
    FC_CONV1_GEOMS(X)
#undef X
    return -1;
}

#define FC_BF3_TILES(X, KS)                \
    X(TILE_M128N32, 4, 1, 1, 1, 1, 16, KS, 4)  \
    X(TILE_M128N64, 4, 1, 1, 1, 2, 16, KS, 4)  \
    X(TILE_M256N64, 4, 1, 1, 2, 2, 16, KS, 4)
template <int KS>
static int bf3_attr_ks() {
#define X(T, WM, WN, WK, MT, NT, CC, K, NL)                                                                                  \
    FC_HIP(hipFuncSetAttribute(reinterpret_cast<const void*>(&conv_pipe_kernel<WM, WN, WK, MT, NT, CC, 8, K, NL, FL_ALL, 1>), \
                               hipFuncAttributeMaxDynamicSharedMemorySize, 160 * 1024));
    FC_BF3_TILES(X, KS)
#undef X
    return FC_OK;
}
template <int KS>
static int bf3_launch_ks(const ConvDev& d, int tile, int grid, size_t lds, hipStream_t s, int* occ) {
    switch (tile) {
#define X(T, WM, WN, WK, MT, NT, CC, K, NL) \
    case T: return launch_pipe<WM, WN, WK, MT, NT, CC, 8, K, NL, FL_ALL, 1>(d, grid, lds, s, occ);
        FC_BF3_TILES(X, KS)
#undef X
        default: return fail(FC_E_ARG, "conv: no split-bf16 form of this tile");
    }
}

int conv_pipe_init() {
    static bool done = false;
    if (done) return FC_OK;
    FC_TRY(bf3_attr_ks<1>());
    FC_TRY(bf3_attr_ks<2>());
    FC_TRY(bf3_attr_ks<3>());
    {
        int dev = 0;
        hipDeviceProp_t prop;
        FC_HIP(hipGetDevice(&dev));
        FC_HIP(hipGetDeviceProperties(&prop, dev));
        g_pipe_cus = prop.multiProcessorCount;
    }
    FC_HIP(hipMalloc(reinterpret_cast<void**>(&g_zeros16), 256));
    FC_HIP(hipMemset(g_zeros16, 0, 256));
    FC_TRY(pipe_attr_ks<1>());
    FC_TRY(pipe_attr_ks<2>());
    FC_TRY(pipe_attr_ks<3>());
    FC_TRY(pipe_attr_ks<5>());
#define X(F) FC_TRY((lean_attr<3, (F)>())); FC_TRY((lean_attr_db4<(F)>()));
    FC_LEAN_FLAVOURS_3(X)
#undef X
#define X(F) FC_TRY((lean_attr<1, (F)>())); FC_TRY((lean_attr_wide1<(F)>()));
    FC_LEAN_FLAVOURS_1(X)
#undef X
    FC_TRY((lean_attr<2, 0>()));
    FC_TRY(fin_geom_attr());
    FC_TRY(conv1_geom_attr());
    done = true;
    return FC_OK;
}

bool conv_pipe_supports_ks(int ks) { return ks == 1 || ks == 2 || ks == 3 || ks == 5; }

template <int KS>
static int pipe_launch_ks(const ConvDev& d, int tile, int grid, size_t lds, hipStream_t s, int* occ) {
    switch (tile) {
#define X(T, WM, WN, WK, MT, NT, CC, K, NL) \
    case T: return launch_pipe<WM, WN, WK, MT, NT, CC, 8, K, NL>(d, grid, lds, s, occ);
        FC_PIPE_TILES(X, KS)
#undef X
        default: return fail(FC_E_ARG, "conv: bad tile id");
    }
}

static int conv_pipe_dispatch(const ConvDev& d, int tile, int grid, size_t lds, hipStream_t s, int* occ) {
    if (d.bf3) return d.a.KS == 1 ? bf3_launch_ks<1>(d, tile, grid, lds, s, occ) : d.a.KS == 2 ? bf3_launch_ks<2>(d, tile, grid, lds, s, occ) : bf3_launch_ks<3>(d, tile, grid, lds, s, occ);
    static const bool lean = [] { const char* e = std::getenv("FLOCODER_AMD_LEAN_KERNELS"); return !(e && std::string(e) == "0"); }();
    if (lean) {
        const bool small_tile = tile == TILE_M32N32K4;
        const int need = (d.a.fin.gamma ? FL_FIN : 0) | (d.a.res_out ? FL_RES : 0) | (d.a.stats_post ? FL_POST : 0) | (d.any_xf ? FL_XF : 0) |
                         (d.a.s1.C ? FL_CAT : 0) | (d.stamps ? FL_STAMP : 0) | (d.a.stats_out ? FL_STATS : 0) | (d.a.fin.gn1_out ? FL_GN1 : 0) |
                         ((d.a.out_act || d.a.add) ? FL_POSTOP : 0) | (d.o_out < 0 ? FL_NARROW : 0) |
                         ((d.TB > 1 && !small_tile) ? FL_MULTI : 0) |
                         ((d.a.fin.gamma && !d.fin_local) ? FL_MEET : 0);
        int r = -1;
        if (d.a.KS == 3) {
            const bool w4 = small_tile && d.a.w4 && d.a.Cin % 32 == 0 && d.a.Cout % 32 == 0 && d.a.pad == 1 && !d.a.w_batch_stride &&
                            (!d.a.res_out || d.a.res_w4);
            const size_t lds_ww = (w4 && (need & FL_FIN)) ? ww_lds(d, tile, lds) : 0;
            if (need & FL_FIN) r = fin_geom_launch(d, tile, w4, need, grid, lds, lds_ww, s, occ);
            else if (need & FL_STATS) r = conv1_geom_launch(d, tile, w4, need, grid, lds, s, occ);
            if (lds_ww) {
#define X(F) if (r == -1 && need == (F)) r = lean_launch_ww<(F)>(d, tile, grid, lds_ww, s, occ);
                FC_LEAN_FLAVOURS_3(X)
#undef X
            }
            if (w4) {
#define X(F) if (r == -1 && need == (F)) r = lean_launch_db4<(F)>(d, tile, grid, lds, s, occ);
                FC_LEAN_FLAVOURS_3(X)
#undef X
            }
#define X(F) if (r == -1 && need == (F)) r = lean_launch<3, (F)>(d, tile, grid, lds, s, occ);
            FC_LEAN_FLAVOURS_3(X)
#undef X
        } else if (d.a.KS == 1) {
#define X(F) if (r == -1 && need == (F)) { r = lean_launch<1, (F)>(d, tile, grid, lds, s, occ); if (r == -1) r = lean_launch_wide1<(F)>(d, tile, grid, lds, s, occ); }
            FC_LEAN_FLAVOURS_1(X)
#undef X
        } else if (d.a.KS == 2 && need == 0) {
            r = lean_launch<2, 0>(d, tile, grid, lds, s, occ);
        }
        if (r != -1) return r;
    }
    switch (d.a.KS) {
        case 1: return pipe_launch_ks<1>(d, tile, grid, lds, s, occ);
        case 2: return pipe_launch_ks<2>(d, tile, grid, lds, s, occ);
        case 3: return pipe_launch_ks<3>(d, tile, grid, lds, s, occ);
        case 5: return pipe_launch_ks<5>(d, tile, grid, lds, s, occ);
    }
    return fail(FC_E_SHAPE, "conv: kernel size not instantiated in the pipelined kernel");
}

int conv_pipe_launch(const ConvDev& d, int tile, int grid, size_t lds, hipStream_t s) { return conv_pipe_dispatch(d, tile, grid, lds, s, nullptr); }

int conv_pipe_blocks_per_cu(const ConvDev& d, int tile, size_t lds) {
    if (!d.a.fin.gamma) {
        int occ = 0;
        return conv_pipe_dispatch(d, tile, 1, lds, nullptr, &occ) == FC_OK ? occ : 0;
    }
    static std::map<std::tuple<int, int, int, size_t, int, int>, int> cache;
    static std::mutex mu;
    const int mask = (d.a.fin.gamma ? FL_FIN : 0) | (d.a.res_out ? FL_RES : 0) | (d.a.stats_post ? FL_POST : 0) | (d.any_xf ? FL_XF : 0) |
                     (d.a.s1.C ? FL_CAT : 0) | (d.stamps ? FL_STAMP : 0) | (d.a.stats_out ? FL_STATS : 0) | (d.a.fin.gn1_out ? FL_GN1 : 0) |
                     ((d.a.out_act || d.a.add) ? FL_POSTOP : 0) | (d.o_out < 0 ? FL_NARROW : 0) | (d.TB > 1 ? FL_MULTI : 0) |
                     ((d.a.fin.gamma && !d.fin_local) ? FL_MEET : 0);
    const int ww = (d.a.KS == 3 && d.a.w4 && ww_lds(d, tile, lds)) ? d.a.Cin : 0;
    const auto key = std::make_tuple(tile, d.a.KS, mask | (d.a.w4 ? FL_W4 : 0), lds, d.cpg, d.TB * 4096 + (d.TWl << 8) + d.tiles_x * d.tiles_y * d.NPG + (ww << 13));
    std::lock_guard<std::mutex> lk(mu);
    auto it = cache.find(key);
    if (it != cache.end()) return it->second;
    int occ = 0;
    if (conv_pipe_dispatch(d, tile, 1, lds, nullptr, &occ) != FC_OK) occ = 0;
    cache[key] = occ;
    return occ;
}

}
```

### flocoder_amd/csrc/elementwise.hip

```cpp
#include "common.h"
#include "stats_dev.h"

namespace fc {

__device__ __forceinline__ void finalize_body(const FinalizeArgs& a, const int bps, const int bx, const int b) {
    extern __shared__ __attribute__((aligned(16))) float sm[];
    float* gm = sm;
    float* A = sm + 2 * a.xf.G;
    float* Bv = A + a.C;
    float* gr = Bv + a.C;
    float* Ar = gr + 2 * (a.xf_res.mode ? a.xf_res.G : 0);
    float* Br = Ar + (a.xf_res.mode ? a.C : 0);
    __shared__ float red[4];
    const int tid = threadIdx.x;
    const int per = a.HW * a.C / bps;
    const size_t base = (size_t)b * a.HW * a.C + (size_t)bx * per;
    const bool act = a.xf.mode == 2 && !a.act_after_add, act2 = a.act_after_add != 0, nres = a.xf_res.mode != 0;
    constexpr int NPF = 4;
    float4 hv[NPF], rv[NPF];
#pragma unroll
    for (int k = 0; k < NPF; ++k) {
        const int i = 4 * tid + 1024 * k;
        hv[k] = rv[k] = make_float4(0.f, 0.f, 0.f, 0.f);
        if (i < per) {
            hv[k] = *reinterpret_cast<const float4*>(a.h + base + i);
            if (a.res) rv[k] = *reinterpret_cast<const float4*>(a.res + base + i);
        }
    }
    float pg = 1.f, pb = 0.f, psc = 0.f, psh = 0.f;
    if (tid < a.C) {
        pg = a.xf.gamma[tid];
        pb = a.xf.beta[tid];
        if (a.xf.ss) {
            psc = a.xf.ss[(size_t)b * a.xf.ss_stride + tid];
            psh = a.xf.ss[(size_t)b * a.xf.ss_stride + a.C + tid];
        }
    }
    for (int g = tid; g < a.xf.G; g += 256) combine_partials(a.xf, b, g, &gm[2 * g], &gm[2 * g + 1]);
    if (a.xf_res.mode)
        for (int g = tid; g < a.xf_res.G; g += 256) combine_partials(a.xf_res, b, g, &gr[2 * g], &gr[2 * g + 1]);
    __syncthreads();
    if (a.xf_res.mode) {
        const int cpr = a.C / a.xf_res.G;
        for (int c = tid; c < a.C; c += 256) {
            const float s = gr[2 * (c / cpr) + 1] * a.xf_res.gamma[c];
            Ar[c] = s;
            Br[c] = a.xf_res.beta[c] - gr[2 * (c / cpr)] * s;
        }
    }
    const int cpg = a.C / a.xf.G;
    for (int c = tid; c < a.C; c += 256) {
        const int g = c / cpg;
// ... 103 lines not shown
    const float* sp = in + (size_t)(b * G + g) * T * 2;
    float sm = 0.f;
    for (int t = lane; t < T; t += 64) sm += sp[2 * t];
#pragma unroll
    for (int o = 32; o > 0; o >>= 1) sm += __shfl_xor(sm, o);
    const float mean = sm / (float)T;
    float m2 = 0.f, dv = 0.f;
    for (int t = lane; t < T; t += 64) { const float d = sp[2 * t] - mean; m2 += sp[2 * t + 1]; dv += d * d; }
#pragma unroll
    for (int o = 32; o > 0; o >>= 1) { m2 += __shfl_xor(m2, o); dv += __shfl_xor(dv, o); }
    if (lane == 0) {
        out[(size_t)(b * G + g) * 2] = mean;
        out[(size_t)(b * G + g) * 2 + 1] = m2 + n_t * dv;
    }
}
int gn_fold_launch(const float* in, float* out, int B, int G, int T, float n_t, hipStream_t s) {
    hipLaunchKernelGGL(gn_fold_kernel, dim3(G, B), dim3(64), 0, s, in, out, G, T, n_t);
    FC_HIP(hipGetLastError());
    return FC_OK;
}

int gn_stats_launch(const float* x, float* stats, int B, int HW, int C, int G, hipStream_t s) {
    hipLaunchKernelGGL(gn_stats_kernel, dim3(G, B), dim3(256), 0, s, x, stats, HW, C, G);
    FC_HIP(hipGetLastError());
    return FC_OK;
}

__global__ void __launch_bounds__(256) init_conv_kernel(const float* x, int bmod, const float* w, const float* bias, float* out,
                                                        int B, int Cin, int HW, int Cout, int conv_blocks, const CondFetch f) {
    if ((int)blockIdx.x >= conv_blocks) {
        const float4* src = reinterpret_cast<const float4*>(f.all) + (size_t)(*f.evalc) * f.n4;
        float4* dst = reinterpret_cast<float4*>(f.dst);
        const int nb = gridDim.x - conv_blocks;
        for (int i = (blockIdx.x - conv_blocks) * 256 + threadIdx.x; i < f.n4; i += nb * 256) dst[i] = src[i];
        return;
    }
    const int q = Cout / 4;
    const size_t total = (size_t)B * HW * q;
    for (size_t i = blockIdx.x * 256ull + threadIdx.x; i < total; i += (size_t)conv_blocks * 256) {
        const int co = (int)(i % q) * 4;
        const size_t bp = i / q;
        const int pix = (int)(bp % HW), b = (int)(bp / HW);
        const float* xb = x + (size_t)(b % bmod) * Cin * HW + pix;
        float4 acc = bias ? *reinterpret_cast<const float4*>(bias + co) : make_float4(0.f, 0.f, 0.f, 0.f);
        for (int ci = 0; ci < Cin; ++ci) {
            const float xv = xb[(size_t)ci * HW];
            const float4 wv = *reinterpret_cast<const float4*>(w + (size_t)ci * Cout + co);
            acc.x += xv * wv.x; acc.y += xv * wv.y; acc.z += xv * wv.z; acc.w += xv * wv.w;
        }
        *reinterpret_cast<float4*>(out + bp * Cout + co) = acc;
    }
}

int init_conv_launch(const CondFetch& fetch, const float* x, int bmod, const float* w, const float* bias, float* out, int B, int Cin, int HW,
                     int Cout, hipStream_t s) {
    if (Cout & 3) return fail(FC_E_SHAPE, "init_conv: Cout must be a multiple of 4");
    const size_t total = (size_t)B * HW * (Cout / 4);
    const int grid = (int)((total + 255) / 256 < 4096 ? (total + 255) / 256 : 4096);
    const int extra = fetch.all ? (fetch.n4 + 255) / 256 < 512 ? (fetch.n4 + 255) / 256 : 512 : 0;
    hipLaunchKernelGGL(init_conv_kernel, dim3(grid + extra), dim3(256), 0, s, x, bmod, w, bias, out, B, Cin, HW, Cout, grid, fetch);
    FC_HIP(hipGetLastError());
    return FC_OK;
}

__global__ void __launch_bounds__(256) final_conv_kernel(const float* x, const float* w, const float* bias, float* out, int B, int Cin,
                                                         int HW, int Cout, const EulerTail e) {
    extern __shared__ float wsm[];
    for (int i = threadIdx.x; i < Cin * Cout; i += 256) wsm[i] = w[i];
    for (int i = threadIdx.x; i < Cout; i += 256) wsm[Cin * Cout + i] = bias ? bias[i] : 0.f;
    __syncthreads();
    const size_t total = (size_t)B * HW;
    for (size_t i = blockIdx.x * 256ull + threadIdx.x; i < total; i += (size_t)gridDim.x * 256) {
        const int pix = (int)(i % HW), b = (int)(i / HW);
        const float* xp = x + i * Cin;
        for (int co0 = 0; co0 < Cout; co0 += 4) {
            float acc[4];
#pragma unroll
            for (int j = 0; j < 4; ++j) acc[j] = (co0 + j < Cout) ? wsm[Cin * Cout + co0 + j] : 0.f;
            for (int ci = 0; ci < Cin; ci += 4) {
                const float4 xv = *reinterpret_cast<const float4*>(xp + ci);
                const float xs[4] = {xv.x, xv.y, xv.z, xv.w};
#pragma unroll
                for (int k = 0; k < 4; ++k)
#pragma unroll
                    for (int j = 0; j < 4; ++j)
                        if (co0 + j < Cout) acc[j] += xs[k] * wsm[(ci + k) * Cout + co0 + j];
            }
#pragma unroll
            for (int j = 0; j < 4; ++j)
                if (co0 + j < Cout) {
                    const size_t o = ((size_t)b * Cout + co0 + j) * HW + pix;
                    if (e.y) e.y[o] = __fadd_rn(e.y[o], __fmul_rn(acc[j], e.dt));
                    else out[o] = acc[j];
                }
        }
    }
    if (e.y && blockIdx.x == 0) {
        const int i = *e.step;
        const float t = e.ts[i];
        __syncthreads();
        if (threadIdx.x == 0) {
            e.sc[0] = t;
            e.sc[1] = 0.f;
            *e.step = i + 1;
        }
        const float tv = __fmul_rn(t, e.t_scale);
        for (int r = threadIdx.x; r < e.rows; r += 256) e.tvec[r] = tv;
    }
    if (e.evalc && blockIdx.x == 0 && threadIdx.x == 0) *e.evalc += 1;
// ... 6 lines not shown
    const size_t total = (size_t)B * HW, i = blockIdx.x * 256ull + threadIdx.x;
    float4 xv[CIN / 4];
    float yv[4] = {0.f, 0.f, 0.f, 0.f};
    const int pix = (int)(i % HW), b = (int)(i / HW);
    if (i < total) {
#pragma unroll
        for (int k = 0; k < CIN / 4; ++k) xv[k] = *reinterpret_cast<const float4*>(x + i * CIN + 4 * k);
        if (e.y) {
#pragma unroll
            for (int j = 0; j < 4; ++j) if (j < Cout) yv[j] = e.y[((size_t)b * Cout + j) * HW + pix];
        }
    }
    for (int k = threadIdx.x; k < CIN * 4; k += 256) wsm[k] = (k & 3) < Cout ? w[(k >> 2) * Cout + (k & 3)] : 0.f;
    if (threadIdx.x < 4) wsm[CIN * 4 + threadIdx.x] = (bias && (int)threadIdx.x < Cout) ? bias[threadIdx.x] : 0.f;
    __syncthreads();
    if (i < total) {
        float acc[4];
#pragma unroll
        for (int j = 0; j < 4; ++j) acc[j] = wsm[CIN * 4 + j];
#pragma unroll
        for (int k = 0; k < CIN / 4; ++k) {
            const float xs[4] = {xv[k].x, xv[k].y, xv[k].z, xv[k].w};
#pragma unroll
            for (int q = 0; q < 4; ++q)
#pragma unroll
                for (int j = 0; j < 4; ++j) acc[j] += xs[q] * wsm[(4 * k + q) * 4 + j];
        }
#pragma unroll
        for (int j = 0; j < 4; ++j)
            if (j < Cout) {
                const size_t o = ((size_t)b * Cout + j) * HW + pix;
                if (e.y) e.y[o] = __fadd_rn(yv[j], __fmul_rn(acc[j], e.dt));
                else out[o] = acc[j];
            }
    }
    if (e.y && blockIdx.x == 0) {
        const int s = *e.step;
        const float t = e.ts[s];
        __syncthreads();
        if (threadIdx.x == 0) {
            e.sc[0] = t;
            e.sc[1] = 0.f;
            *e.step = s + 1;
        }
        const float tv = __fmul_rn(t, e.t_scale);
        for (int r = threadIdx.x; r < e.rows; r += 256) e.tvec[r] = tv;
    }
    if (e.evalc && blockIdx.x == 0 && threadIdx.x == 0) *e.evalc += 1;
}

int final_conv_launch(const float* x, const float* w, const float* bias, float* out, int B, int Cin, int HW, int Cout, const EulerTail& tail,
                      hipStream_t s) {
    if (Cin & 3) return fail(FC_E_SHAPE, "final_conv: Cin must be a multiple of 4");
    const size_t total = (size_t)B * HW;
    if (Cout <= 4 && total < (1ull << 31) && (Cin == 8 || Cin == 16 || Cin == 32 || Cin == 64)) {
        const dim3 g((unsigned)((total + 255) / 256));
        switch (Cin) {
            case 8: hipLaunchKernelGGL(final_conv_small_kernel<8>, g, dim3(256), 0, s, x, w, bias, out, B, HW, Cout, tail); break;
            case 16: hipLaunchKernelGGL(final_conv_small_kernel<16>, g, dim3(256), 0, s, x, w, bias, out, B, HW, Cout, tail); break;
            case 32: hipLaunchKernelGGL(final_conv_small_kernel<32>, g, dim3(256), 0, s, x, w, bias, out, B, HW, Cout, tail); break;
            default: hipLaunchKernelGGL(final_conv_small_kernel<64>, g, dim3(256), 0, s, x, w, bias, out, B, HW, Cout, tail); break;
        }
        FC_HIP(hipGetLastError());
        return FC_OK;
    }
    const int grid = (int)((total + 255) / 256 < 4096 ? (total + 255) / 256 : 4096);
    hipLaunchKernelGGL(final_conv_kernel, dim3(grid), dim3(256), (size_t)(Cin * Cout + Cout) * sizeof(float), s, x, w, bias, out, B,
                       Cin, HW, Cout, tail);
    FC_HIP(hipGetLastError());
    return FC_OK;
}

__global__ void __launch_bounds__(256) nchw_to_nhwc_kernel(const float* src, float* dst, int B, int C, int HW, int Cpad, int bmod) {
    const size_t total = (size_t)B * HW * Cpad;
    for (size_t i = blockIdx.x * 256ull + threadIdx.x; i < total; i += (size_t)gridDim.x * 256) {
        const int c = (int)(i % Cpad);
        const size_t bp = i / Cpad;
        const int pix = (int)(bp % HW), b = (int)(bp / HW);
        dst[i] = c < C ? src[((size_t)(b % bmod) * C + c) * HW + pix] : 0.f;
    }
}
__global__ void __launch_bounds__(256) nhwc_to_nchw_kernel(const float* src, float* dst, int B, int C, int HW, int Cpad) {
    const size_t total = (size_t)B * C * HW;
    for (size_t i = blockIdx.x * 256ull + threadIdx.x; i < total; i += (size_t)gridDim.x * 256) {
        const int pix = (int)(i % HW);
        const size_t bc = i / HW;
        const int c = (int)(bc % C), b = (int)(bc / C);
        dst[i] = src[((size_t)b * HW + pix) * Cpad + c];
    }
}
static int grid_for(size_t total) { size_t g = (total + 255) / 256; return (int)(g < 8192 ? (g ? g : 1) : 8192); }

int nchw_to_nhwc_launch(const float* src, float* dst, int B, int C, int HW, int Cpad, int bmod, hipStream_t s) {
    hipLaunchKernelGGL(nchw_to_nhwc_kernel, dim3(grid_for((size_t)B * HW * Cpad)), dim3(256), 0, s, src, dst, B, C, HW, Cpad,
                       bmod > 0 ? bmod : B);
    FC_HIP(hipGetLastError());
    return FC_OK;
}
int nhwc_to_nchw_launch(const float* src, float* dst, int B, int C, int HW, int Cpad, hipStream_t s) {
    hipLaunchKernelGGL(nhwc_to_nchw_kernel, dim3(grid_for((size_t)B * C * HW)), dim3(256), 0, s, src, dst, B, C, HW, Cpad);
    FC_HIP(hipGetLastError());
    return FC_OK;
}

__global__ void __launch_bounds__(256) pixel_shuffle2_kernel(const float* src, float* dst, int B, int H, int W, int C) {
    const size_t total = (size_t)B * 4 * H * W * C;
// ... 41 lines not shown
```

### flocoder_amd/csrc/plan.h

```cpp
#pragma once
#include <cmath>
#include <functional>
#include <map>
#include <string>
#include <unordered_map>
#include <vector>

#include "common.h"

namespace fc {

struct Param {
    std::string name;
    int64_t shape[4] = {0, 0, 0, 0};
    int64_t numel = 0, offset = 0;
};

struct Act { float* p = nullptr; int C = 0, H = 0, W = 0; };
struct Stat { float* p = nullptr; int G = 0, T = 0; float n_t = 0.f; };

struct FwdCtx {
    const float* x = nullptr;
    int x_mod = 0;
    const float* time = nullptr;
    const int64_t* ids = nullptr;
    int ids_mod = 0, null_from = 0;
    const float* mask = nullptr;
    int mask_fuse = 0;
    float* out = nullptr;
    int B = 0;
    const float* d_out = nullptr;
    float* grads = nullptr;
    bool grads_acc = false;
    float* dx_out = nullptr;
    float* dmask_out = nullptr;
    EulerTail euler;
    CondFetch fetch;
};
using Op = std::function<int(const FwdCtx&, hipStream_t)>;

struct ResRec { std::string p; Act x, skip, h1, h2, rb, out; Stat st1, st2; int cout = 0; };
struct LinRec { std::string p; Act x, qkv, lao, yb, out; float* ctx = nullptr; Stat gn1, sty; };
struct MidRec { Act x, qkv, ao, out; Stat gn1; };
struct ConvRec { std::string name; Act x, out; int KS = 1, pad = 0, stride = 1, ups = 0; };
struct InjRec { std::string name; Act x, mr, z, out; };
struct FuseRec { bool present = false; Act xi, mask, z1, f1, z2, f2, x0; };
struct TapeItem { int kind, idx; };

struct Plan {
    int maxB = 0, H = 0, W = 0;
    std::vector<Op> ops;
    std::vector<std::string> op_kernel, op_what;
    std::vector<double> op_flops;
    std::vector<char> op_param_only;
    std::vector<double> op_bytes_ps, op_bytes_fixed;
    std::vector<void*> allocs;
    double flops = 0.0;
    double flops_executed = 0.0;
    float *t_emb = nullptr, *ss = nullptr;
    std::map<std::string, Act> named;
    std::vector<ResRec> res; std::vector<LinRec> lin; std::vector<MidRec> mid; std::vector<ConvRec> convs; std::vector<InjRec> inj;
    FuseRec fuse;
    std::vector<TapeItem> tape;
    Act x0, head;
    int n_meet = 0;
    std::vector<unsigned*> fin_sync;
    std::vector<int> fin_kind;
    void release() {
        for (void* p : allocs) dev_free(p);
        *this = Plan();
    }
};

struct PackOp { int kind; int64_t src, dst; int a, b, c, d, e = 0; };

static const char* const kTileNames[] = {"conv_igemm<M128,N32>", "conv_igemm<M128,N64>", "conv_igemm<M64,N32,K2>", "conv_igemm<M32,N32,K4>",
                                         "conv_igemm<M64,N64,K2>", "conv_igemm<M256,N64>"};

struct ParamStore {
    std::vector<Param> params;
    std::unordered_map<std::string, int> pidx;
    int64_t raw_numel = 0, packed_numel = 0;
    float *raw = nullptr, *packed = nullptr;
    std::unordered_map<std::string, int64_t> pk;
    std::vector<PackOp> packops;
    PackTable pack_table;
    bool loaded = false;

    bool want_b3 = false;
    std::unordered_map<int64_t, int64_t> b3_of;
    const float* B3(const float* w) const {
        auto it = b3_of.find(w - packed);
        return it == b3_of.end() ? nullptr : packed + it->second;
    }
    bool want_k8 = false;
    const float* P8(const std::string& n) const { auto it = pk.find(n + "#k8"); return it == pk.end() ? nullptr : packed + it->second; }
    const float* R(const std::string& n) const { return raw + params[pidx.at(n)].offset; }
    const float* P(const std::string& n) const { return packed + pk.at(n); }
    bool has(const std::string& n) const { return pidx.count(n) != 0; }

    void declare(const std::string& name, std::initializer_list<int64_t> shape) {
        Param p;
        p.name = name;
        p.numel = 1;
        int i = 0;
        for (int64_t s : shape) { p.shape[i++] = s; p.numel *= s; }
        p.offset = raw_numel;
        raw_numel += (p.numel + 3) & ~3ll;
        pidx[name] = (int)params.size();
        params.push_back(p);
    }
    int64_t pk_alloc(const std::string& name, int64_t numel) {
        const int64_t off = packed_numel;
        pk[name] = off;
        packed_numel += (numel + 3) & ~3ll;
        return off;
    }
    void decl_conv(const std::string& n, int O, int I, int K, bool bias = true) {
        declare(n + ".weight", {O, I, K, K});
        if (bias) declare(n + ".bias", {O});
// ... 41 lines not shown
        FC_HIP(hipMemset(raw, 0, (size_t)(raw_numel ? raw_numel : 4) * sizeof(float)));
        std::vector<PackJob> jobs;
        for (const PackOp& o : packops) jobs.push_back({raw + o.src, packed + o.dst, o.kind, o.a, o.b, o.kind == 0 ? o.c * o.d : o.c, o.d, o.e, 0});
        return pack_table_build(jobs, &pack_table);
    }
    void free_device() {
        pack_table.release();
        if (raw) dev_free(raw);
        if (packed) dev_free(packed);
        raw = packed = nullptr;
    }
    int run_pack(hipStream_t s) const {
        if (pack_table.nblocks) return pack_table_launch(pack_table, s);
        for (const PackOp& o : packops) {
            const float* src = raw + o.src;
            float* dst = packed + o.dst;
            switch (o.kind) {
                case 0: FC_TRY(pack_conv_launch(src, dst, o.a, o.b, o.c, o.d, s)); break;
                case 1: FC_TRY(pack_s2d_conv_launch(src, dst, o.a, o.b, s)); break;
                case 2: FC_TRY(pack_transpose_launch(src, dst, o.a, o.b, o.c, o.d, s)); break;
                case 3: FC_HIP(hipMemcpyAsync(dst, src, (size_t)o.a * sizeof(float), hipMemcpyDeviceToDevice, s)); break;
                case 4: FC_TRY(pack_conv_pad_launch(src, dst, o.a, o.b, o.c, o.d, o.e, s)); break;
                case 6: return fail(FC_E_STATE, "pack: the k-step-quad layout exists in the table launch only");
            }
        }
        return FC_OK;
    }
    int load(const float* flat, int64_t numel, int on_device, hipStream_t s) {
        if (numel != raw_numel) return fail(FC_E_ARG, "load_params: expected " + std::to_string(raw_numel) + " floats (padded table layout)");
        FC_HIP(hipMemcpyAsync(raw, flat, (size_t)numel * sizeof(float), on_device ? hipMemcpyDeviceToDevice : hipMemcpyHostToDevice, s));
        FC_TRY(run_pack(s));
        if (!on_device) FC_HIP(hipStreamSynchronize(s));
        loaded = true;
        return FC_OK;
    }
    int info(int i, const char** name, int64_t shape[4], int64_t* offset) const {
        if (i < 0 || i >= (int)params.size()) return fail(FC_E_ARG, "param_info: index out of range");
        const Param& p = params[i];
        if (name) *name = p.name.c_str();
        if (shape) for (int k = 0; k < 4; ++k) shape[k] = p.shape[k];
        if (offset) *offset = p.offset;
        return FC_OK;
    }
};

struct PlanBuilder {
    Plan* pl = nullptr;
    int B = 0;
    int err = FC_OK;
    std::string scope;
    int* fin_err_word = nullptr;
    int conv_prec = 0;
    const ParamStore* store = nullptr;

    int guard = 0;
    bool param_only = false;
    void push(Op op, const std::string& kernel, double flops = 0.0, double bytes_ps = 0.0, double bytes_fixed = 0.0, double flops_ref = 0.0) {
        if (guard) {
            const int g = guard;
            Op inner = std::move(op);
            op = [inner, g](const FwdCtx& c, hipStream_t s) -> int {
                const bool on = g == 1 ? c.mask != nullptr : g == 2 ? c.mask_fuse != 0 : g == 3 ? c.mask == nullptr : (c.mask != nullptr && !c.mask_fuse);
                return on ? inner(c, s) : FC_OK;
            };
        }
        pl->ops.push_back(std::move(op));
        pl->op_kernel.push_back(kernel);
        pl->op_what.push_back(scope);
        pl->op_flops.push_back(flops);
        pl->op_param_only.push_back(param_only ? 1 : 0);
        pl->op_bytes_ps.push_back(bytes_ps);
        pl->op_bytes_fixed.push_back(bytes_fixed);
        pl->flops += flops_ref > 0.0 ? flops_ref : flops;
        pl->flops_executed += flops;
    }
    float* dmalloc(size_t floats) {
        void* p = nullptr;
        if (dev_alloc(&p, (floats ? floats : 1) * sizeof(float), scope.c_str()) != FC_OK) { err = fail(FC_E_HIP, "hipMalloc failed while reserving the arena"); return nullptr; }
        pl->allocs.push_back(p);
        return static_cast<float*>(p);
    }
    std::multimap<size_t, float*> pool;
    Act act(int C, int H, int W) {
        Act a; a.C = C; a.H = H; a.W = W;
        const size_t n = (size_t)B * H * W * C;
        auto it = pool.find(n);
        if (it != pool.end()) { a.p = it->second; pool.erase(it); }
        else a.p = dmalloc(n);
        return a;
    }
    bool keep_all = false;
    void release(const Act& a) { if (a.p && !keep_all) pool.emplace((size_t)B * a.H * a.W * a.C, a.p); }
    void tap(const std::string& name, const Act& a) { if (keep_all && !err) pl->named[name] = a; }
    Stat stat(int G, int T, float n_t) { Stat s; s.G = G; s.T = T; s.n_t = n_t; s.p = dmalloc((size_t)B * G * T * 2); return s; }

    static SrcXform xf_of(const Stat& st, int mode, const float* gamma, const float* beta, const float* ss = nullptr, int ss_stride = 0,
                          float eps = 1e-5f) {
        SrcXform x;
        x.mode = mode; x.stats = st.p; x.G = st.G; x.T = st.T; x.n_t = st.n_t;
        x.gamma = gamma; x.beta = beta; x.ss = ss; x.ss_stride = ss_stride; x.eps = eps;
        return x;
    }

    static double conv_bytes_ps(const ConvArgs& a) {
        double e = (double)a.Hs * a.Ws * a.Cin + (double)a.H * a.W * a.Cout;
        if (a.res_out) e += (double)a.H * a.W * a.Cout;
// ... 46 lines not shown
        a.s0 = src; a.Hs = x.H; a.Ws = x.W; a.KS = 2; a.pad = 0; a.stride = 1;
        a.B = B; a.H = x.H; a.W = x.W; a.Cout = out.C; a.out = out.p; a.bias = bias;
        a.Cin = a.s0.C;
        a.prec = conv_prec;
        a.w = w4;
        if (conv_prec && store) a.w_b3 = store->B3(w4);
        a.par4 = 1; a.out_sh = 1; a.stats_tmul = 4; a.pad_y = 1; a.pad_x = 1;
        const bool fused = want_G > 0;
        ConvGeom g;
        if (fused) { a.Gout = want_G; a.stats_out = reinterpret_cast<float*>(1); }
        if (conv_plan(a, TILE_AUTO, &g) != FC_OK || !g.pipe) return false;
        if (fused) { *st = stat(want_G, 4 * g.T, g.n_t); a.stats_out = st->p; }
        const int tile = g.tile;
        const double fl = 2.0 * out.H * out.W * 4.0 * (double)a.Cin * a.Cout;
        push([a, tile](const FwdCtx& c, hipStream_t s) { ConvArgs b = a; b.B = c.B; return conv_launch(b, tile, s); }, kTileNames[tile], fl,
             4.0 * ((double)x.H * x.W * a.Cin + (double)out.H * out.W * a.Cout), 4.0 * 16.0 * a.Cin * a.Cout,
             2.0 * out.H * out.W * 9.0 * (double)a.Cin * a.Cout);
        if (fused && st->T > 16) {
            const Stat raw = *st;
            *st = stat(want_G, 1, raw.n_t * (float)raw.T);
            const float* ip = raw.p; float* op = st->p;
            const int G = want_G, T = raw.T; const float nt = raw.n_t;
            push([=](const FwdCtx& c, hipStream_t s) { return gn_fold_launch(ip, op, c.B, G, T, nt, s); }, "gn_fold");
        }
        return true;
    }

    bool conv_fin(ConvArgs a, const Act& out, int G, const float* gamma, const float* beta, const float* res, bool want_gn1, Stat* gn1,
                  bool only_local = false) {
        if (err) return false;
        a.B = B; a.H = out.H; a.W = out.W; a.Cout = out.C; a.out = out.p;
        a.Cin = a.s0.C + a.s1.C;
        if ((out.H * out.W) % 16) return false;
        a.Gout = G; a.stats_out = reinterpret_cast<float*>(16);
        a.fin.gamma = gamma; a.fin.beta = beta; a.fin.res = res;
        if (want_gn1) a.fin.gn1_out = reinterpret_cast<float*>(16);
        ConvGeom g;
        if (conv_plan(a, TILE_AUTO, &g) != FC_OK || !g.pipe) return false;
        if (only_local && !g.fin_local) return false;
        Stat st = stat(G, g.T, g.n_t);
        a.stats_out = st.p;
        if (want_gn1) { *gn1 = stat(1, g.T1, g.n_t1); a.fin.gn1_out = gn1->p; }
        unsigned* sync = reinterpret_cast<unsigned*>(dmalloc((size_t)g.groups + 1));
        if (err) return false;
        if (hipMemset(sync, 0, ((size_t)g.groups + 1) * sizeof(unsigned)) != hipSuccess) { err = fail(FC_E_HIP, "hipMemset failed"); return false; }
        const size_t ngran = (size_t)B * G * g.T * 2;
        a.fin.gran = reinterpret_cast<unsigned long long*>(dmalloc(2 * ngran));
        if (err) return false;
        if (hipMemset(a.fin.gran, 0, ngran * sizeof(unsigned long long)) != hipSuccess) { err = fail(FC_E_HIP, "hipMemset failed"); return false; }
        a.fin.sync = sync;
        a.fin.err = fin_err_word ? fin_err_word : reinterpret_cast<int*>(sync + g.groups);
        if (!g.fin_local) { ++pl->n_meet; pl->fin_sync.push_back(sync); pl->fin_kind.push_back(0); }
        const int tile = g.tile;
        const double fl = 2.0 * out.H * out.W * a.KS * a.KS * (double)a.Cin * a.Cout;
        push([a, tile](const FwdCtx& c, hipStream_t s) { ConvArgs b = a; b.B = c.B; return conv_launch(b, tile, s); }, std::string(kTileNames[tile]) + "+fin", fl,
             conv_bytes_ps(a), conv_bytes_fixed(a));
        return true;
    }

    struct AttnWeights { const float *wq, *bq, *wk, *bk, *wv, *bv, *wo, *bo; };
    Act attention_block(const Act& x, const SrcXform& norm_x, const AttnWeights& w, int want_G, Stat* so) {
        const int C = x.C, hw = x.H * x.W;
        Act q = act(C, x.H, x.W), k = act(C, x.H, x.W), vv = act(C, x.H, x.W);
        const float* ws[3] = {w.wq, w.wk, w.wv};
        const float* bs[3] = {w.bq, w.bk, w.bv};
        const Act* outs[3] = {&q, &k, &vv};
        for (int i = 0; i < 3; ++i) {
            ConvArgs a;
            a.s0.p = x.p; a.s0.C = C; a.s0.xf = norm_x;
            a.Hs = x.H; a.Ws = x.W; a.KS = 1;
            a.w = ws[i]; a.bias = bs[i];
            conv(a, *outs[i], 0, nullptr);
        }
        float* kt = dmalloc((size_t)B * C * hw);
        const float* kp = k.p;
        push([=](const FwdCtx& c, hipStream_t s) { return transpose_batched_launch(kp, kt, c.B, hw, C, s); }, "transpose");
        Act sc = act(hw, x.H, x.W);
        {
            ConvArgs a;
            a.s0.p = q.p; a.s0.C = C; a.Hs = x.H; a.Ws = x.W; a.KS = 1;
            a.w = kt; a.w_batch_stride = C * hw;
            conv(a, sc, 0, nullptr);
        }
        float* sp = sc.p;
        const float scale = 1.0f / sqrtf((float)C);
        push([=](const FwdCtx& c, hipStream_t s) { return softmax_rows_launch(sp, (long)c.B * hw, hw, scale, s); }, "softmax_rows");
        Act o = act(C, x.H, x.W);
        {
            ConvArgs a;
            a.s0.p = sc.p; a.s0.C = hw; a.Hs = x.H; a.Ws = x.W; a.KS = 1;
            a.w = vv.p; a.w_batch_stride = hw * C;
            conv(a, o, 0, nullptr);
        }
        Act out = act(C, x.H, x.W);
        {
            ConvArgs a;
            a.s0.p = o.p; a.s0.C = C; a.Hs = x.H; a.Ws = x.W; a.KS = 1;
            a.w = w.wo; a.bias = w.bo;
            a.add = x.p; a.stats_post = 1;
            conv(a, out, want_G, so);
        }
        tap(scope + ".q", q); tap(scope + ".k", k); tap(scope + ".v", vv); tap(scope + ".p", sc); tap(scope + ".o", o);
        release(q); release(k); release(vv); release(sc); release(o);
        return out;
    }
};

inline int run_plan(const Plan& pl, const FwdCtx& c, hipStream_t s) {
    for (const Op& op : pl.ops) FC_TRY(op(c, s));
// ... 29 lines not shown
```

### flocoder_amd/csrc/unet.hip

```cpp
#include <algorithm>
#include <cmath>
#include <cstdint>
#include <cstdlib>
#include <cstring>
#include <map>
#include <memory>
#include <mutex>
#include <string>
#include <unordered_map>
#include <vector>

#include "plan.h"
#include "unet_priv.h"
#include "unet_sample.h"

namespace fc {

static thread_local std::string g_err;
void set_error(const std::string& m) { g_err = m; }
int fail(int code, const std::string& m) { g_err = m; return code; }
const char* last_error() { return g_err.c_str(); }

}

// ... 528 lines not shown
    if (!is_pow2(H) || !is_pow2(W) || (H >> (L - 1)) < 1 || (W >> (L - 1)) < 1)
        return fail(FC_E_SHAPE, "unet: latent height/width must be powers of two >= 2^(levels-1)");
    if ((ch & 3) || (dim & 3)) return fail(FC_E_SHAPE, "unet: channels and dim must be multiples of 4");
    Builder b(u, pl, maxB);
    pl->flops = 0.0;
    pl->t_emb = b.dmalloc((size_t)maxB * u->td);
    pl->ss = b.dmalloc((size_t)maxB * u->S);
    const std::vector<int>& cs = u->chans;
    const int td = u->td, S = u->S, ncls = c.n_classes;

    {
        TembArgs t;
        t.freqs = u->freqs;
        t.w1t = u->P("time_mlp.1.weight"); t.b1 = u->R("time_mlp.1.bias");
        t.w2t = u->P("time_mlp.3.weight"); t.b2 = u->R("time_mlp.3.bias");
        t.emb = t.cw1t = t.cb1 = t.cw2t = t.cb2 = nullptr;
        if (ncls > 0) {
            t.emb = u->R("class_cond_mlp.0.weight");
            t.cw1t = u->P("class_cond_mlp.1.weight"); t.cb1 = u->R("class_cond_mlp.1.bias");
            t.cw2t = u->P("class_cond_mlp.3.weight"); t.cb2 = u->R("class_cond_mlp.3.bias");
        }
        t.n_classes = ncls; t.t_out = pl->t_emb; t.dim = dim; t.td = td;
        u->temb_proto = t;
        b.scope = "time_mlp";
        float *hid = b.dmalloc((size_t)maxB * td), *chid = b.dmalloc((size_t)maxB * td);
        b.push([t, hid, chid](const FwdCtx& cx, hipStream_t s) {
            if (cx.fetch.all) return (int)FC_OK;
            TembArgs a = t; a.B = cx.B; a.time = cx.time; a.class_ids = cx.ids; a.class_batch_mod = cx.ids_mod; a.null_from = cx.null_from;
            return temb_launch(a, hid, chid, s);
        }, "temb", 2.0 * ((double)dim * td + (double)td * td * (ncls > 0 ? 3 : 1)));
        const float *te = pl->t_emb, *wt = u->P("__ss_wt"), *sb = u->P("__ss_bias");
        float* ss = pl->ss;
        b.scope = "resblock.mlp";
        b.push([=](const FwdCtx& cx, hipStream_t s) { return cx.fetch.all ? (int)FC_OK : ss_launch(te, wt, sb, ss, cx.B, td, S, s); }, "ss", 2.0 * (double)td * S);
    }

    {
        const int r = build_sample_plan(u, pl, b, maxB, H, W);
        if (r != 1) {
            if (r != FC_OK) return r;
            pl->maxB = maxB; pl->H = H; pl->W = W;
            return FC_OK;
        }
    }
    Act x0 = b.act(dim, H, W);
    pl->named["init"] = x0;
    pl->x0 = x0;
    Act mask_nhwc;
    {
        const float *w = u->P("init_conv.weight"), *bias = u->R("init_conv.bias");
        float* x0p = x0.p;
        b.scope = "init_conv";
        if (!c.mask_cond) {
            b.push([=](const FwdCtx& cx, hipStream_t s) { return init_conv_launch(cx.fetch, cx.x, cx.x_mod, w, bias, x0p, cx.B, ch, HW, dim, s); }, "init_conv", 2.0 * HW * ch * dim);
        } else {
            Act xi = b.act(dim, H, W), f1 = b.act(2 * dim, H, W), f2 = b.act(2 * dim, H, W);
            const bool keep = u->keep_all;
            Act z1 = keep ? b.act(2 * dim, H, W) : Act(), z2 = keep ? b.act(2 * dim, H, W) : Act();
            mask_nhwc = b.act(ch, H, W);
            float *xip = xi.p, *mp = mask_nhwc.p;
            b.push([=](const FwdCtx& cx, hipStream_t s) -> int {
                if (cx.mask) FC_TRY(nchw_to_nhwc_launch(cx.mask, mp, cx.B, ch, HW, ch, cx.x_mod, s));
                return init_conv_launch(cx.fetch, cx.x, cx.x_mod, w, bias, cx.mask_fuse ? xip : x0p, cx.B, ch, HW, dim, s);
            }, "init_conv", 2.0 * HW * ch * dim);
            ConvArgs a[3];
            const char* names[3] = {"mask_fusion_conv.0", "mask_fusion_conv.2", "mask_fusion_conv.4"};
            const Act* srcs[3] = {&xi, &f1, &f2};
            const Act* dsts[3] = {keep ? &z1 : &f1, keep ? &z2 : &f2, &x0};
            int tiles[3];
            for (int i = 0; i < 3 && !b.err; ++i) {
                a[i].s0.p = srcs[i]->p; a[i].s0.C = srcs[i]->C;
                if (i == 0) { a[i].s1.p = mask_nhwc.p; a[i].s1.C = ch; }
                a[i].Hs = H; a[i].Ws = W; a[i].KS = i == 0 ? 5 : 3; a[i].pad = i == 0 ? 2 : 1; a[i].out_act = (i < 2 && !keep);
                a[i].w = u->P(std::string(names[i]) + ".weight"); a[i].bias = u->R(std::string(names[i]) + ".bias");
                a[i].B = maxB; a[i].H = H; a[i].W = W; a[i].Cout = dsts[i]->C; a[i].out = dsts[i]->p; a[i].Cin = a[i].s0.C + a[i].s1.C;
                ConvGeom g;
                b.err = conv_plan(a[i], TILE_AUTO, &g);
                tiles[i] = g.tile;
            }
            if (b.err) return b.err;
            const ConvArgs a0 = a[0], a1 = a[1], a2 = a[2];
            const int t0 = tiles[0], t1 = tiles[1], t2 = tiles[2];
            const float *z1p = z1.p, *z2p = z2.p;
            float *f1p = f1.p, *f2p = f2.p;
            const size_t nf = (size_t)HW * 2 * dim;
            b.scope = "mask_fusion_conv";
            b.push([=](const FwdCtx& cx, hipStream_t s) -> int {
                if (!cx.mask_fuse) return FC_OK;
                ConvArgs q = a0; q.B = cx.B; FC_TRY(conv_launch(q, t0, s));
                if (keep) FC_TRY(silu_fwd_launch(z1p, nullptr, f1p, nf * cx.B, s));
                q = a1; q.B = cx.B; FC_TRY(conv_launch(q, t1, s));
                if (keep) FC_TRY(silu_fwd_launch(z2p, nullptr, f2p, nf * cx.B, s));
                q = a2; q.B = cx.B; return conv_launch(q, t2, s);
            }, "mask_fusion(3 x conv_igemm)", 2.0 * HW * (25.0 * (dim + ch) * 2 * dim + 9.0 * 2 * dim * 2 * dim + 9.0 * 2 * dim * dim));
            pl->fuse.present = true;
            pl->fuse.xi = xi; pl->fuse.mask = mask_nhwc; pl->fuse.z1 = z1; pl->fuse.f1 = f1; pl->fuse.z2 = z2; pl->fuse.f2 = f2; pl->fuse.x0 = x0;
        }
    }

    std::vector<Act> skips;
    Act x = x0;
    for (int i = 0; i < L && !b.err; ++i) {
        const std::string p = "downs." + std::to_string(i);
        Stat gn1;
        x = b.resblock(p + ".0", x, nullptr, cs[i], false, nullptr);
        skips.push_back(x);
        x = b.resblock(p + ".1", x, nullptr, cs[i], true, &gn1);
// ... 10 lines not shown
            pl->tape.push_back({3, (int)pl->convs.size()});
            pl->convs.push_back({p + ".3", x, o, 3, 1, 1, 0});
            x = o;
            pl->named[p + ".3"] = o;
        } else {
            a.KS = 2; a.pad = 0; a.stride = 2; a.w = u->P(p + ".3.1.weight"); a.bias = u->R(p + ".3.1.bias");
            Act o = b.act(cs[i + 1], x.H / 2, x.W / 2);
            b.conv(a, o, 0, nullptr);
            pl->tape.push_back({3, (int)pl->convs.size()});
            pl->convs.push_back({p + ".3.1", x, o, 2, 0, 2, 0});
            x = o;
            pl->named[p + ".3"] = o;
        }
    }
    {
        Stat gn1;
        x = b.resblock("mid_block1", x, nullptr, cs[L], true, &gn1);
        if (!b.err) x = b.midattn(x, gn1);
        if (!b.err) x = b.resblock("mid_block2", x, nullptr, cs[L], false, nullptr);
    }
    for (int i = 0; i < L && !b.err; ++i) {
        const std::string p = "ups." + std::to_string(i);
        const int din = cs[L - 1 - i], dout = cs[L - i];
        Stat gn1;
        Act s1 = skips.back(); skips.pop_back();
        x = b.resblock(p + ".0", x, &s1, dout, false, nullptr);
        Act s2 = skips.back(); skips.pop_back();
        x = b.resblock(p + ".1", x, &s2, dout, true, &gn1);
        x = b.linattn(p + ".2", x, gn1);
        if (c.mask_cond && i < 2) x = b.mask_inject("up_mask_fusions." + std::to_string(i) + ".0", x, mask_nhwc);
        b.scope = p + ".3";
        ConvArgs a;
        a.s0.p = x.p; a.s0.C = x.C; a.Hs = x.H; a.Ws = x.W; a.KS = 3; a.pad = 1;
        if (i == L - 1) {
            a.w = u->P(p + ".3.weight"); a.bias = u->R(p + ".3.bias"); a.w4 = u->P8(p + ".3.weight");
            Act o = b.act(din, x.H, x.W);
            b.conv(a, o, 0, nullptr);
            pl->tape.push_back({3, (int)pl->convs.size()});
            pl->convs.push_back({p + ".3", x, o, 3, 1, 1, 0});
            x = o;
        } else {
            Act o = b.act(din, x.H * 2, x.W * 2);
            if (!b.conv_up2(a.s0, x, u->PUP(p + ".3.1.weight"), u->R(p + ".3.1.bias"), o, 0, nullptr)) {
                a.ups = 1; a.w = u->P(p + ".3.1.weight"); a.bias = u->R(p + ".3.1.bias"); a.w4 = u->P8(p + ".3.1.weight");
                b.conv(a, o, 0, nullptr);
            }
            pl->tape.push_back({3, (int)pl->convs.size()});
            pl->convs.push_back({p + ".3.1", x, o, 3, 1, 1, 1});
            x = o;
        }
        pl->named[p + ".3"] = x;
    }
    if (b.err) return b.err;
    x = b.resblock("final_res_block", x, &x0, dim, false, nullptr);
    if (b.err) return b.err;
    pl->head = x;
    {
        const float *xp = x.p, *w = u->P("final_conv.weight"), *bias = u->R("final_conv.bias");
        b.scope = "final_conv";
        b.push([=](const FwdCtx& cx, hipStream_t s) { return final_conv_launch(xp, w, bias, cx.out, cx.B, dim, HW, ch, cx.euler, s); }, "final_conv", 2.0 * HW * dim * ch);
    }
    if (b.err) return b.err;
    pl->maxB = maxB; pl->H = H; pl->W = W;
    return FC_OK;
}

struct MeetGuard { std::mutex mu; hipEvent_t ev = nullptr; hipStream_t s = nullptr; const fc_unet* owner = nullptr; };
static MeetGuard g_meet[16];
static MeetGuard& meet_guard(int device) { return g_meet[device & 15]; }

static int plan_meets(const fc_unet* u) { return u->plan.n_meet; }

int meet_enter(fc_unet* u, hipStream_t s) {
    if (!plan_meets(u)) return FC_OK;
    MeetGuard& g = meet_guard(u->device);
    std::lock_guard<std::mutex> lk(g.mu);
    if (g.ev && g.s != s && hipEventQuery(g.ev) != hipSuccess) FC_HIP(hipStreamWaitEvent(s, g.ev, 0));
    return FC_OK;
}
int meet_leave(fc_unet* u, hipStream_t s) {
    if (!plan_meets(u)) return FC_OK;
    MeetGuard& g = meet_guard(u->device);
    std::lock_guard<std::mutex> lk(g.mu);
    FC_HIP(hipEventRecord(u->ev_meet, s));
    g.ev = u->ev_meet; g.s = s; g.owner = u;
    FC_HIP(hipMemcpyAsync(const_cast<int*>(u->host_err), u->dev_err, sizeof(int), hipMemcpyDeviceToHost, s));
    return FC_OK;
}
static void meet_forget(const fc_unet* u) {
    MeetGuard& g = meet_guard(u->device);
    std::lock_guard<std::mutex> lk(g.mu);
    if (g.owner == u) { g.ev = nullptr; g.s = nullptr; g.owner = nullptr; }
}
int check_poison(fc_unet* u) {
    if (u->host_err && *u->host_err) u->tail_failed = true;
    if (u->tail_failed)
        return fail(FC_E_STATE, "unet: a fused Block tail timed out waiting for its sample group (the GPU was shared with other work while "
                                "the exclusive plan ran); the affected samples are NaN.  Rebuild the plan -- fc_unet_set_shared(handle, 1) "
                                "selects the plan without cross-workgroup waits");
    return FC_OK;
}

int check_ready(const fc_unet* u, int rows, int H, int W) {
    if (!u) return fail(FC_E_ARG, "null fc_unet");
    if (u->device < 0) return fail(FC_E_STATE, "unet: created with device < 0 (description only)");
    if (!u->loaded) return fail(FC_E_STATE, "unet: weights not loaded (fc_unet_load_params)");
    if (u->maxB < rows || u->H != H || u->W != W)
        return fail(FC_E_STATE, "unet: no plan for this shape; call fc_unet_reserve(rows >= " + std::to_string(rows) + ")");
    return FC_OK;
}

}

// ... 220 lines not shown

int fc_unet_train_release(fc_unet* u) {
    if (!u) return fail(FC_E_ARG, "fc_unet_train_release: null handle");
    if (u->device < 0 || !u->keep_all) return FC_OK;
    FC_HIP(hipSetDevice(u->device));
    FC_HIP(hipDeviceSynchronize());
    free_plan(u);
    u->keep_all = false;
    u->arena_touched(0);
    return FC_OK;
}

int fc_unet_debug_tensor(const fc_unet* u, const char* name, const float** ptr, int* C, int* H, int* W) {
    if (!u || !name) return fail(FC_E_ARG, "fc_unet_debug_tensor: null argument");
    auto it = u->plan.named.find(name);
    if (it == u->plan.named.end()) {
        it = u->bwd.named.find(name);
        if (it == u->bwd.named.end()) return fail(FC_E_ARG, std::string("fc_unet_debug_tensor: no tap named ") + name);
    }
    *ptr = it->second.p; *C = it->second.C; *H = it->second.H; *W = it->second.W;
    return FC_OK;
}

int fc_debug_unet_break_meeting(fc_unet* u) {
    if (!u || u->plan.fin_sync.empty()) return fail(FC_E_STATE, "fc_debug_unet_break_meeting: the plan has no meeting launch");
    FC_HIP(hipDeviceSynchronize());
    unsigned v = 0;
    FC_HIP(hipMemcpy(&v, u->plan.fin_sync[0], sizeof(unsigned), hipMemcpyDeviceToHost));
    ++v;
    FC_HIP(hipMemcpy(u->plan.fin_sync[0], &v, sizeof(unsigned), hipMemcpyHostToDevice));
    return FC_OK;
}

int fc_debug_unet_break_meeting_kind(fc_unet* u, int kind) {
    if (!u) return fail(FC_E_ARG, "fc_debug_unet_break_meeting_kind: null handle");
    const Plan& pl = u->plan;
    for (size_t i = 0; i < pl.fin_sync.size(); ++i)
        if (pl.fin_kind[i] == kind) {
            FC_HIP(hipDeviceSynchronize());
            unsigned v = 0;
            FC_HIP(hipMemcpy(&v, pl.fin_sync[i], sizeof(unsigned), hipMemcpyDeviceToHost));
            ++v;
            FC_HIP(hipMemcpy(pl.fin_sync[i], &v, sizeof(unsigned), hipMemcpyHostToDevice));
            return FC_OK;
        }
    return fail(FC_E_STATE, "fc_debug_unet_break_meeting_kind: the plan has no meeting launch of that kind");
}

int fc_debug_set_fused_tail(int on) {
    fc::g_fused_tail = on < 0 ? -1 : (on ? 1 : 0);
    return FC_OK;
}

int fc_debug_conv_routes(int on) { conv_route_log_set(on != 0); linattn_route_log_set(on != 0); return FC_OK; }
int fc_debug_conv_routes_read(char* buf, int cap) {
    const std::string r = conv_route_log_get();
    if (buf && cap > 0) { const size_t n = r.size() < (size_t)cap - 1 ? r.size() : (size_t)cap - 1; memcpy(buf, r.data(), n); buf[n] = 0; }
    return (int)r.size();
}

int fc_debug_linattn_routes_read(char* buf, int cap) {
    const std::string r = linattn_route_log_get();
    if (buf && cap > 0) { const size_t n = r.size() < (size_t)cap - 1 ? r.size() : (size_t)cap - 1; memcpy(buf, r.data(), n); buf[n] = 0; }
    return (int)r.size();
}

int fc_debug_set_conv_stamps(void* buf_dev) {
    conv_set_stamp_buffer(static_cast<unsigned long long*>(buf_dev));
    return FC_OK;
}

int fc_debug_copy(void* dst_dev, const void* src_dev, int64_t bytes, void* stream) {
    FC_HIP(hipMemcpyAsync(dst_dev, src_dev, (size_t)bytes, hipMemcpyDeviceToDevice, static_cast<hipStream_t>(stream)));
    return FC_OK;
}

static int g_debug_conv_prec = 0;
int fc_debug_set_conv_precision(int mode) { g_debug_conv_prec = mode == 1 ? 1 : 0; return FC_OK; }

int fc_debug_conv(const float* src0, int c0, const float* src1, int c1, const float* w_oihw, const float* bias, const float* add,
                  float* out, float* stats_out, int groups_out, int* stats_T, float* stats_nt, int batch, int hs, int ws, int cout,
                  int ksize, int pad, int stride, int upsample, int out_act, int tile_cfg, int repeats, float* ms_out, void* stream) {
    hipStream_t s = static_cast<hipStream_t>(stream);
    FC_TRY(conv_init());
    ConvArgs a;
    a.s0.p = src0; a.s0.C = c0; a.s1.p = src1; a.s1.C = src1 ? c1 : 0;
    a.Cin = a.s0.C + a.s1.C; a.Cout = cout; a.B = batch; a.Hs = hs; a.Ws = ws;
    a.KS = ksize; a.pad = pad; a.stride = stride; a.ups = upsample;
    a.H = upsample ? hs * 2 : (hs + 2 * pad - ksize) / stride + 1;
    a.W = upsample ? ws * 2 : (ws + 2 * pad - ksize) / stride + 1;
    a.bias = bias; a.add = add; a.out = out; a.out_act = out_act;
    a.stats_out = stats_out; a.Gout = groups_out;
    a.prec = g_debug_conv_prec;
    float* wp = nullptr;
    FC_HIP(hipMalloc(reinterpret_cast<void**>(&wp), (size_t)cout * a.Cin * ksize * ksize * sizeof(float)));
    int r = pack_conv_launch(w_oihw, wp, cout, a.Cin, ksize, ksize, s);
    a.w = wp;
    float* wp8 = nullptr;
    if (r == FC_OK && ksize == 3 && a.Cin % 32 == 0 && cout % 32 == 0) {
        FC_HIP(hipMalloc(reinterpret_cast<void**>(&wp8), (size_t)cout * a.Cin * 9 * sizeof(float)));
        r = pack_conv_k8_launch(w_oihw, wp8, cout, a.Cin, 9, s);
        a.w4 = wp8;
    }
    float* wp3 = nullptr;
    if (r == FC_OK && a.prec == 1 && (ksize == 3 || ksize == 1)) {
        const int ipad = (a.Cin + 15) / 16 * 16;
        FC_HIP(hipMalloc(reinterpret_cast<void**>(&wp3), (size_t)cout * ipad * ksize * ksize * sizeof(float)));
// ... 111 lines not shown
```

### flocoder_amd/csrc/unet_integrate.hip

```cpp
#include <algorithm>
#include <cmath>
#include <cstdlib>
#include <cstring>
#include <functional>

#include "plan.h"
#include "unet_priv.h"

using namespace fc;

namespace fc {

void IntegratorState::drop_graphs() {
    for (auto& kv : graphs) (void)hipGraphExecDestroy(kv.second);
    graphs.clear();
}
void IntegratorState::release_plan() {
    drop_graphs();
    for (void* p : allocs) dev_free(p);
    static_cast<IntegratorPlanState&>(*this) = IntegratorPlanState{};
}
void IntegratorState::release_handle() {
    release_plan();
    for (void* p : {(void*)ts_dev, (void*)rk_ev, (void*)pre}) if (p) dev_free(p);
// ... 147 lines not shown

static int ll_reserve(fc_unet* u, int n_probes, hipStream_t s) {
    IntegratorState& ig = u->ig;
    if (n_probes <= ig.ll_k) return FC_OK;
    const size_t m = (size_t)u->cfg.channels * u->H * u->W;
    if (ig.ll_k) FC_HIP(hipStreamSynchronize(s));
    ig.ll_k = 0;
    for (double** b : {&ig.ll_d, &ig.rk_dk, &ig.rk_ak}) ig.drop(b);
    ig.drop(&ig.ll_g);
    FC_TRY(ig.get(&ig.ll_d, (size_t)n_probes * u->maxB * 3, "integrator.likelihood"));
    FC_TRY(ig.get(&ig.ll_g, (size_t)n_probes * u->maxB * m, "integrator.likelihood"));
    ig.ll_k = n_probes;
    return FC_OK;
}

static int check_probes(const char* fn, int n_probes, const double* a_probes_out, const double* stderr_out) {
    if (n_probes < 1 || n_probes > FC_LL_MAX_PROBES)
        return fail(FC_E_ARG, std::string(fn) + ": n_probes must lie in [1, " + std::to_string(FC_LL_MAX_PROBES) + "] (the cap on probes per call)");
    if (!a_probes_out != !stderr_out || (n_probes > 1 && !a_probes_out))
        return fail(FC_E_ARG, std::string(fn) + ": several probes need a_probes_out_dev and stderr_out_dev");
    return FC_OK;
}

static int enqueue_rk4_interval(const CallFrame& f, const Rk4Variant& v, float cfg, float t_scale) {
    fc_unet* u = f.u;
    const IntegratorState& ig = u->ig;
    const int n = f.n, m = f.n / f.B, cf = f.cfg_on ? 1 : 0;
    hipStream_t s = f.s;
    const struct { float* k_out; int full, tcur, tsel; } stages[4] = {{ig.k1, 0, 0, 1}, {ig.k2, 0, 1, 1}, {ig.k3, 1, 1, 2}, {nullptr, 0, 2, 0}};
    FwdCtx c = v.c;
    FC_TRY(ode_time_launch(ig.step, ig.ts_dev, t_scale, 1, ig.sc, ig.tvec, v.trows, s));
    for (int j = 0; j < 4; ++j) {
        const auto& st = stages[j];
        const float* x = c.x = j == 0 ? ig.y : ig.xs;
        FC_TRY(run_plan(u->plan, c, s));
        if (v.eval == Rk4Variant::ForwardGuideWVjp) FC_TRY(ode_guide_w_launch(ig.sc, ig.g_sc, ig.v2, x, ig.g_y, ig.g_keep, ig.g_w, n, st.tcur, s));
        if (v.close == Rk4Variant::Likelihood) {
            FC_TRY(probe_chains(u, c, v.probe, v.n_probes, n, s));
            FC_TRY(j < 3 ? ode_ll_stage_launch(ig.sc, ig.y, ig.xs, st.k_out, ig.v2, ig.ll_g, v.probe, ig.ll_d, j, f.B, m, st.full, st.tsel, t_scale, ig.tvec, v.n_probes, s)
                         : ode_ll_final_launch(ig.sc, ig.y, ig.k1, ig.k2, ig.k3, ig.v2, ig.ll_g, v.probe, ig.ll_d, v.a, f.B, m, v.n_probes, s));
            continue;
        }
        if (v.eval != Rk4Variant::Forward) FC_TRY(vjp_run(u, c, s));
        const Rk4Guide guide{ig.g_sc, x, ig.g_y, ig.g_keep, v.q, st.tcur};
        const Rk4Guide* g = v.close == Rk4Variant::Guided ? &guide : nullptr;
        FC_TRY(j < 3 ? ode_rk4_stage_launch(ig.sc, ig.y, ig.xs, st.k_out, ig.v2, n, cf, cfg, st.full, st.tsel, t_scale, ig.tvec, v.trows, g, s)
                     : ode_rk4_final_launch(ig.sc, ig.y, ig.k1, ig.k2, ig.k3, ig.v2, n, cf, cfg, g, s));
    }
    return FC_OK;
}

static bool euler_tail_ok(int method, bool cfg_on) { return method == FC_METHOD_EULER && !cfg_on; }

static int enqueue_step(const CallFrame& f, int method, float cfg, float dt_euler, float t_scale, bool pre_on) {
    fc_unet* u = f.u;
    const IntegratorState& ig = u->ig;
    const bool cfg_on = f.cfg_on;
    const int rows = f.rows, n = f.n;
    hipStream_t s = f.s;
    FwdCtx c = step_ctx(f, pre_on);
    if (method == FC_METHOD_RK4) return enqueue_rk4_interval(f, {Rk4Variant::Forward, Rk4Variant::Plain, rows, c}, cfg, t_scale);
    if (euler_tail_ok(method, cfg_on)) {
        c.x = ig.y;
        c.euler.y = ig.y; c.euler.dt = dt_euler; c.euler.step = ig.step; c.euler.ts = ig.ts_dev; c.euler.t_scale = t_scale;
        c.euler.sc = ig.sc; c.euler.tvec = ig.tvec; c.euler.rows = rows;
        return run_plan(u->plan, c, s);
    }
    FC_TRY(ode_time_launch(ig.step, ig.ts_dev, t_scale, 0, ig.sc, ig.tvec, rows, s));
    c.x = ig.y;
    FC_TRY(run_plan(u->plan, c, s));
    return ode_euler_update_launch(ig.y, ig.v2, n, cfg_on, cfg, dt_euler, s);
}

static int integrator_prologue(const CallFrame& f, const float* x_dev, const float* ts_host, int n_points) {
    IntegratorState& ig = f.u->ig;
    hipStream_t s = f.s;
    if (n_points + 1 > ig.ts_cap) {
        FC_HIP(hipStreamSynchronize(s));
        if (ig.ts_dev) dev_free(ig.ts_dev);
        ig.ts_cap = n_points < 1024 ? 1024 : n_points + 1;
        FC_TRY(dev_alloc(reinterpret_cast<void**>(&ig.ts_dev), ig.ts_cap * sizeof(float), "integrator.ts"));
        ig.drop_graphs();
    }
    FC_HIP(hipMemcpyAsync(ig.ts_dev, ts_host, n_points * sizeof(float), hipMemcpyHostToDevice, s));
    FC_HIP(hipMemsetAsync(ig.step, 0, 2 * sizeof(int), s));
    FC_HIP(hipMemcpyAsync(ig.y, x_dev, f.nbytes, hipMemcpyDeviceToDevice, s));
    return FC_OK;
}

static constexpr int kTimesPair = 2;
static_assert(FC_METHOD_EULER == 0 && FC_METHOD_RK4 == 1, "ode_all_times_launch takes the method codes as its pattern");
static int cond_table(const CallFrame& f, int pattern, int n_steps, float t_scale, bool* pre_on_out) {
    fc_unet* u = f.u;
    IntegratorState& ig = u->ig;
    const bool has_ids = f.has_ids, cfg_on = f.cfg_on;
    const int rows = f.rows, B = f.B;
    hipStream_t s = f.s;
    const int n_evals = pattern == FC_METHOD_RK4 ? 4 * n_steps : (pattern == kTimesPair ? 2 * n_steps : n_steps);
    const size_t R = (size_t)n_evals * rows, tvn = ((size_t)n_evals + 3) & ~(size_t)3;
    const size_t need = tvn + R * u->td * 3 + R * u->S;
    const bool pre_on = *pre_on_out = n_steps >= 2 && need * sizeof(float) <= (2ull << 30) && R < (1u << 30) / (unsigned)u->S;
    if (!pre_on) return FC_OK;
    {
        if (need > ig.pre_cap) {
            FC_HIP(hipStreamSynchronize(s));
            if (ig.pre) dev_free(ig.pre);
            ig.pre = nullptr; ig.pre_cap = 0;
            FC_TRY(dev_alloc(reinterpret_cast<void**>(&ig.pre), need * sizeof(float), "integrator.cond_table"));
            ig.pre_cap = need;
            ig.drop_graphs();
        }
        float *tv = ig.pre, *te = tv + tvn, *hh = te + R * u->td, *c1 = hh + R * u->td;
        if (ig.pre_ss != c1 + R * u->td)
            ig.drop_graphs();
        ig.pre_ss = c1 + R * u->td;
        FC_TRY(ode_all_times_launch(ig.ts_dev, n_steps, pattern, t_scale, tv, s));
        TembArgs ta = u->temb_proto;
        ta.B = (int)R; ta.time = tv; ta.rows_per_eval = rows; ta.class_ids = has_ids ? ig.ids_own : nullptr; ta.class_batch_mod = B;
// ... 5 lines not shown
        ca.w = u->P("__ss_wt"); ca.bias = u->P("__ss_bias"); ca.out = ig.pre_ss;
        FC_TRY(conv_launch(ca, TILE_AUTO, s));
    }
    return FC_OK;
}

static int replay_steps(const CallFrame& f, GraphKey key, int n_steps, int evals_per_step, const std::function<int()>& step) {
    fc_unet* u = f.u;
    hipStream_t s = f.s;
    if (no_graph()) {
        for (int i = 0; i < n_steps; ++i) FC_TRY(step());
        return FC_OK;
    }
    {
        const int nodes_per_step = (int)u->plan.ops.size() * evals_per_step + 16;
        int per = 6144 / nodes_per_step > 0 ? 6144 / nodes_per_step : 1;
        if (per > 255) per = 255;
        for (int left = n_steps; left > 0;) {
            const int k = left < per ? left : per;
            key.steps = k;
            hipGraphExec_t exec = nullptr;
            FC_TRY(cached_graph(u, key, s, [&] {
                int r = FC_OK;
                for (int j = 0; j < k && r == FC_OK; ++j)
                    r = step();
                return r;
            }, &exec));
            if (left == n_steps) FC_HIP(hipStreamSynchronize(s));
            FC_HIP(hipGraphLaunch(exec, s));
            left -= k;
        }
    }
    return FC_OK;
}

int fc_unet_integrate(fc_unet* u, int method, float* x_dev, int B, int H, int W, const float* ts_host, int n_points, float dt_euler,
                      float t_scale, const int64_t* ids, float cfg_strength, const float* mask, int mask_is_ones, void* stream) {
    if (!u || !x_dev || !ts_host || B < 1 || n_points < 1) return fail(FC_E_ARG, "fc_unet_integrate: bad argument");
    if (method != FC_METHOD_EULER && method != FC_METHOD_RK4) return fail(FC_E_ARG, "fc_unet_integrate: unknown method");
    CallFrame f;
    FC_TRY(f.begin(u, B, H, W, ids, cfg_strength, mask, mask_is_ones, stream));
    FC_TRY(f.enter());
    IntegratorState& ig = u->ig;
    const bool cfg_on = f.cfg_on;
    const int rows = f.rows, n_steps = method == FC_METHOD_RK4 ? n_points - 1 : n_points;
    hipStream_t s = f.s;
    FC_TRY(integrator_prologue(f, x_dev, ts_host, n_points));
    bool pre_on = false;
    FC_TRY(cond_table(f, method, n_steps, t_scale, &pre_on));
    if (euler_tail_ok(method, cfg_on))
        FC_TRY(ode_time_launch(ig.step, ig.ts_dev, t_scale, 0, ig.sc, ig.tvec, rows, s));
    GraphKey key = graph_key(f, method == FC_METHOD_RK4 ? GraphKey::Rk4 : GraphKey::Euler, cfg_strength, t_scale);
    key.pre_on = pre_on; key.dt_euler = fbits(dt_euler);
    FC_TRY(replay_steps(f, key, n_steps, method == FC_METHOD_RK4 ? 4 : 1,
                        [&] { return enqueue_step(f, method, cfg_strength, dt_euler, t_scale, pre_on); }));
    return f.finish(x_dev);
}

static int log_likelihood_rk4(const char* fn, fc_unet* u, float* x_dev, int B, int H, int W, const float* ts_host, int n_points, float t_scale,
                              const int64_t* ids, const float* mask, int mask_is_ones, const float* probes_dev, int n_probes,
                              double* a_out_dev, double* logp_out_dev, double* a_probes_out_dev, double* stderr_out_dev, void* stream) {
    if (!u || !x_dev || !ts_host || !probes_dev || !a_out_dev || !logp_out_dev || B < 1) return fail(FC_E_ARG, std::string(fn) + ": null argument");
    if (n_points < 2) return fail(FC_E_ARG, std::string(fn) + ": the time grid needs at least two points");
    FC_TRY(check_probes(fn, n_probes, a_probes_out_dev, stderr_out_dev));
    FC_TRY(check_aligned16({probes_dev}, (std::string(fn) + ": probe_dev must be 16-byte aligned (the kernels read it as float4)").c_str()));
    CallFrame f;
    FC_TRY(f.begin(u, B, H, W, ids, 0.0f, mask, mask_is_ones, stream));
    if (!u->keep_all) return fail(FC_E_STATE, std::string(fn) + ": no backward plan for this shape; call fc_unet_train_reserve");
    FC_TRY(vjp_check(u, B, H, W, fn));
    IntegratorState& ig = u->ig;
    const int m = u->cfg.channels * H * W;
    FC_TRY(ll_reserve(u, n_probes, f.s));
    FC_TRY(f.enter());
    FC_TRY(integrator_prologue(f, x_dev, ts_host, n_points));
    double* acc = a_probes_out_dev ? a_probes_out_dev : a_out_dev;
    FC_HIP(hipMemsetAsync(acc, 0, (size_t)n_probes * B * sizeof(double), f.s));
    Rk4Variant v{Rk4Variant::ForwardVjp, Rk4Variant::Likelihood, B, integrator_ctx(f)};
    v.probe = probes_dev; v.a = acc; v.n_probes = n_probes;
    for (int i = 0; i + 1 < n_points; ++i) FC_TRY(enqueue_rk4_interval(f, v, 0.0f, t_scale));
    if (a_probes_out_dev) FC_TRY(ode_ll_mean_launch(a_probes_out_dev, n_probes, B, a_out_dev, stderr_out_dev, 0, f.s));
    FC_TRY(ode_ll_logp_launch(ig.y, a_out_dev, logp_out_dev, B, m, f.s));
    return f.finish(x_dev);
}

int fc_unet_log_likelihood(fc_unet* u, float* x_dev, int B, int H, int W, const float* ts_host, int n_points, float t_scale,
                           const int64_t* ids, const float* mask, int mask_is_ones, const float* probe_dev, double* a_out_dev,
                           double* logp_out_dev, void* stream) {
    return log_likelihood_rk4("fc_unet_log_likelihood", u, x_dev, B, H, W, ts_host, n_points, t_scale, ids, mask, mask_is_ones, probe_dev, 1,
                              a_out_dev, logp_out_dev, nullptr, nullptr, stream);
}

int fc_unet_log_likelihood_probes(fc_unet* u, float* x_dev, int B, int H, int W, const float* ts_host, int n_points, float t_scale,
                                  const int64_t* ids, const float* mask, int mask_is_ones, const float* probes_dev, int n_probes,
                                  double* a_out_dev, double* logp_out_dev, double* a_probes_out_dev, double* stderr_out_dev, void* stream) {
    if (!a_probes_out_dev || !stderr_out_dev) return fail(FC_E_ARG, "fc_unet_log_likelihood_probes: null argument");
    return log_likelihood_rk4("fc_unet_log_likelihood_probes", u, x_dev, B, H, W, ts_host, n_points, t_scale, ids, mask, mask_is_ones,
                              probes_dev, n_probes, a_out_dev, logp_out_dev, a_probes_out_dev, stderr_out_dev, stream);
}

int fc_debug_probe_dot(const float* probe_dev, const float* g_dev, double* out_dev, int batch, int64_t per_sample, void* stream) {
    if (!probe_dev || !g_dev || !out_dev) return fail(FC_E_ARG, "fc_debug_probe_dot: null argument");
    FC_TRY(check_aligned16({probe_dev, g_dev}, "fc_debug_probe_dot: inputs must be 16-byte aligned (read as float4)"));
    if (per_sample < 1 || per_sample > 0x7fffffff) return fail(FC_E_SHAPE, "fc_debug_probe_dot: bad element count");
    return ode_ll_dot_launch(probe_dev, g_dev, out_dev, nullptr, batch, (int)per_sample, 1, static_cast<hipStream_t>(stream));
}

static int alloc_guided(fc_unet* u, bool exact) {
    IntegratorState& ig = u->ig;
// ... 413 lines not shown
```

### flocoder_amd/csrc/unet_priv.h

```cpp
#pragma once
#include <algorithm>
#include <map>
#include <tuple>

#include "plan.h"

namespace fc {

struct GraphKey {
    enum Kind { Euler, Rk4, Rk45Coupled, Rk45PerSample, Rk4Guided, Sde };
    Kind kind = Euler;
    int B = 0, mask_mode = 0;
    bool cfg_on = false, has_ids = false;
    bool pre_on = false;
    int steps = 0;
    bool dense = false;
    uint32_t cfg_strength = 0, dt_euler = 0, t_scale = 0;
    int sde_scheme = 0, sde_noise = 0;
    uint32_t sde_sigma = 0;
    auto tie() const {
        return std::tie(kind, B, mask_mode, cfg_on, has_ids, pre_on, steps, dense, cfg_strength, dt_euler, t_scale, sde_scheme, sde_noise,
                        sde_sigma);
    }
    bool operator<(const GraphKey& o) const { return tie() < o.tie(); }
};

struct IntegratorPlanState {
    std::vector<void*> allocs;
    int* step = nullptr;
    float *sc = nullptr, *tvec = nullptr;
    float *y = nullptr, *xs = nullptr, *k1 = nullptr, *k2 = nullptr, *k3 = nullptr, *v2 = nullptr, *mask_own = nullptr;
    int64_t* ids_own = nullptr;
    double *rk_y = nullptr, *rk_ynew = nullptr, *rk_part = nullptr;
    Rk45K rk_k{};
    Rk45State* rk_st = nullptr;
    Rk45Status* rk_sum = nullptr;
    double *rk_a = nullptr, *rk_d = nullptr, *rk_dk = nullptr, *rk_ak = nullptr;
    float* ll_g = nullptr;
    double* ll_d = nullptr;
    int ll_k = 0;
    float *g_y = nullptr, *g_keep = nullptr, *g_sc = nullptr, *g_w = nullptr, *g_q = nullptr;
    SdeParams* sde_prm = nullptr;
    int64_t* sde_ids = nullptr;

    template <class T> int get(T** out, size_t count, const char* tag) {
        void* p = nullptr;
        FC_TRY(dev_alloc(&p, (count ? count : 1) * sizeof(T), tag));
        allocs.push_back(p);
        *out = static_cast<T*>(p);
        return FC_OK;
    }
    template <class T> void drop(T** buf) {
        if (!*buf) return;
        allocs.erase(std::remove(allocs.begin(), allocs.end(), static_cast<void*>(*buf)), allocs.end());
        dev_free(*buf);
        *buf = nullptr;
    }
};
struct IntegratorState : IntegratorPlanState {
    hipStream_t stream = nullptr;
    hipEvent_t ev_in = nullptr, ev_out = nullptr;
    fc::Rk45Status* rk_host = nullptr;
    hipEvent_t ev_rk = nullptr;
    float* ts_dev = nullptr;
    int ts_cap = 0;
    float* pre = nullptr;
    size_t pre_cap = 0;
    float* pre_ss = nullptr;
    Rk45Eval* rk_ev = nullptr;
    int rk_ev_cap = 0;
    std::map<GraphKey, hipGraphExec_t> graphs;

    void drop_graphs();
    void release_plan();
// ... 53 lines not shown
```

### include/flocoder_amd.h

```cpp
#ifndef FLOCODER_AMD_H
#define FLOCODER_AMD_H

#include <stdint.h>

#ifdef __cplusplus
extern "C" {
#endif

#define FC_OK 0
#define FC_E_ARG (-1)
#define FC_E_SHAPE (-2)
#define FC_E_ARCH (-3)
#define FC_E_HIP (-4)
#define FC_E_STATE (-5)

#define FC_ABI_VERSION 1

int fc_abi_version(void);
const char* fc_last_error(void);
int fc_check_device(int device);

typedef struct fc_unet fc_unet;

typedef struct fc_unet_config {
// ... 89 lines not shown
                             const float* y_meas_dev, const float* keep_dev, float sigma_y, float gamma, int jacobian, void* stream);
int fc_ode_guided_correct(const float* v_dev, const float* x_dev, const float* y_dev, const float* a_dev, int64_t n, float t, float sigma_y,
                          float gamma, float* out_dev, void* stream);

#define FC_SDE_EULER_MARUYAMA 0
#define FC_SDE_HEUN 1
int fc_unet_integrate_sde(fc_unet* u, int scheme, float* x_dev, int batch, int height, int width, const float* ts_host, int n_points,
                          float t_scale, const int64_t* class_ids_dev, float cfg_strength, const float* mask_dev, int mask_is_ones,
                          float sigma, uint64_t seed, const int64_t* sample_ids_dev, const float* noise_dev, void* stream);
int fc_ode_normal_field(float* out_dev, uint64_t seed, int64_t draw_index, const int64_t* sample_ids_dev, int batch, int64_t per_sample,
                        void* stream);

#define FC_MASK_TOTAL 0
#define FC_MASK_BRUSH 1
#define FC_MASK_RECTANGLES 2
#define FC_MASK_NOISE 3
#define FC_MASK_NOTHING 4
#define FC_MASK_MIN_SIZE 16
#define FC_MASK_MAX_SIZE 1024
#define FC_MASK_KEY_OFFSET 0x4D41534B464C4431ULL
int fc_inpaint_masks(float* masks_out_dev, int* types_out_dev, uint64_t seed, const int64_t* sample_ids_dev, int batch, int height, int width,
                     const int* choice_types_host, const double* probs_host, int n_choices, int forced_type, void* stream);

int fc_note_confusion(const float* pred_dev, int pred_channels, const float* target_dev, int target_channels, const float* region_dev, int batch,
                      int height, int width, float threshold, double minval, int derive_min, double maxval, int derive_max, int keep_gray,
                      void* ws_dev, int64_t* counts_out_dev, float* masks_out_dev, float* overlay_out_dev, void* stream);

#define FC_HIST_LDS_BINS 8192
int fc_index_histogram(const int64_t* indices_dev, int64_t n, int levels, int codebook_size, int64_t* counts_inout_dev, int64_t* keys_out_dev,
                       int64_t* bad_rows_inout_dev, void* stream);

#define FC_AUG_KEY_OFFSET 0x415547464C443031ULL
#define FC_AUG_MIN_SIZE 16
#define FC_AUG_MAX_SIZE 1024
#define FC_AUG_MAX_SIDE 8192
#define FC_AUG_IMAGE_WORDS 16
#define FC_AUG_MIDI_WORDS 8
#define FC_AUG_LDS_PIXELS 6144
int fc_augment_images(float* out_dev, const uint8_t* pool_dev, const int64_t* table_dev, int n_sources, const int* sample_table_dev, int batch,
                      int size, const float* mean_host, const float* std_host, const float* fill_host, void* stream);
int fc_augment_midi(float* out_dev, const uint8_t* pool_dev, const int64_t* table_dev, int n_sources, const int* sample_table_dev, int batch,
                    int size, int out_channels, int gray, float threshold, void* stream);

int fc_debug_unet_guided_buffers(const fc_unet* u, const float** stage_x, const float** stage_time, const float** w, const float** q);
int fc_debug_probe_dot(const float* probe_dev, const float* g_dev, double* out_dev, int batch, int64_t per_sample, void* stream);
int fc_unet_debug_tensor(const fc_unet* u, const char* name, const float** ptr, int* channels, int* height, int* width);
int fc_debug_copy(void* dst_dev, const void* src_dev, int64_t bytes, void* stream);
int fc_debug_set_poison(int on);
int fc_debug_poison_check(int* corrupted, int* live);
int fc_debug_set_conv_stamps(void* buf_dev);
int fc_debug_conv_routes(int on);
int fc_debug_conv_routes_read(char* buf, int cap);
int fc_debug_linattn_routes_read(char* buf, int cap);
int fc_debug_set_stamp_op(int op_index, void* buf_dev);
int fc_debug_set_conv_precision(int mode);
int fc_debug_conv(const float* src0_nhwc, int c0, const float* src1_nhwc, int c1, const float* w_oihw_dev, const float* bias_dev,
                  const float* add_nhwc, float* out_nhwc, float* stats_out, int groups_out, int* stats_T, float* stats_nt, int batch,
                  int hs, int ws, int cout, int ksize, int pad, int stride, int upsample, int out_act, int tile_cfg, int repeats,
                  float* ms_out, void* stream);

int fc_unet_train_reserve(fc_unet* u, int max_batch, int height, int width);
int fc_unet_backward(fc_unet* u, const float* x_dev, const float* time_dev, const int64_t* class_ids_dev, const float* d_out_dev,
                     float* grads_flat_dev, int64_t numel, int batch, int height, int width, void* stream);
int fc_unet_backward_ex(fc_unet* u, const float* x_dev, const float* time_dev, const int64_t* class_ids_dev, const float* mask_dev,
                        int mask_is_ones, const float* d_out_dev, float* grads_flat_dev, int64_t numel, float* dx_out_dev,
                        float* dmask_out_dev, int batch, int height, int width, void* stream);
int fc_unet_backward_parts(fc_unet* u, const float* x_dev, const float* time_dev, const int64_t* class_ids_dev, const float* mask_dev,
                           int mask_is_ones, const float* d_out_dev, float* grads_flat_dev, int64_t numel, float* dx_out_dev,
                           float* dmask_out_dev, int batch, int height, int width, int first_part, int last_part, void* stream);
int fc_unet_backward_accumulate(fc_unet* u, const float* x_dev, const float* time_dev, const int64_t* class_ids_dev, const float* mask_dev,
                                int mask_is_ones, const float* d_out_dev, float* grads_flat_dev, int64_t numel, float* dx_out_dev,
                                float* dmask_out_dev, int batch, int height, int width, int first_part, int last_part, void* stream);
int fc_unet_set_grad_buckets(fc_unet* u, int on);
int fc_unet_grad_buckets(const fc_unet* u, int64_t* split_offset);
int fc_unet_backward_launches(const fc_unet* u);
int fc_unet_backward_op_info(const fc_unet* u, int i, const char** kernel, const char** module);
int fc_unet_train_form(const fc_unet* u);
int fc_unet_train_release(fc_unet* u);
int fc_unet_vjp_x(fc_unet* u, const float* x_dev, const float* time_dev, const int64_t* class_ids_dev, const float* mask_dev,
                  int mask_is_ones, const float* d_out_dev, float* dx_out_dev, int batch, int height, int width, void* stream);
int fc_unet_vjp_launches(const fc_unet* u);
int fc_unet_vjp_op_info(const fc_unet* u, int i, const char** kernel, const char** module);
uint64_t fc_unet_arena_serial(const fc_unet* u);
int fc_unet_class_param_range(const fc_unet* u, int64_t* lo, int64_t* hi);
int fc_flow_interp(const float* source_dev, const float* target_dev, const float* t_dev, float* x_out_dev, float* v_out_dev, int batch,
                   int64_t per_sample, void* stream);
int fc_flow_prepare(const float* source_dev, const float* target_dev, const int64_t* pairing_dev, const float* u_dev, float t_eps, float warp_s,
                    float t_scale, const int64_t* class_ids_dev, int n_classes, float* t_out_dev, float* time_out_dev, float* x_out_dev,
                    float* v_out_dev, int* id_flag_dev, int batch, int64_t per_sample, void* stream);
int fc_flow_prepare_rows(const float* source_dev, const float* target_dev, const int64_t* pairing_dev, const float* u_dev, float t_eps, float warp_s,
                         float t_scale, const int64_t* class_ids_dev, int n_classes, float* t_out_dev, float* time_out_dev, float* x_out_dev,
                         float* v_out_dev, int* id_flag_dev, int batch, int first_row, int target_rows, int64_t per_sample, void* stream);
int fc_mse_loss_grad_scaled(const float* v_dev, const float* target_dev, float* dv_out_dev, float* loss_acc_dev, float* ws256_dev, int64_t numel,
                            float scale, void* stream);
int fc_mse_loss_grad(const float* v_dev, const float* target_dev, float* dv_out_dev, float* loss_out_dev, float* ws256_dev, int64_t numel,
                     void* stream);
int fc_grad_clip_coef(const float* grads_dev, int64_t numel, const float* grads2_dev, int64_t numel2, float max_norm, float* norm_coef_out_dev,
                      float* ws256_dev, void* stream);
int fc_adam_ema_step(float* params_dev, const float* grads_dev, float* exp_avg_dev, float* exp_avg_sq_dev, float* ema_dev, int64_t numel,
                     const float* clip_coef_dev, float lr, float beta1, float beta2, float eps, int step, float ema_decay, int apply_adam,
                     void* stream);
int fc_adam_ema_step_guarded(float* params_dev, const float* grads_dev, float* exp_avg_dev, float* exp_avg_sq_dev, float* ema_dev, int64_t numel,
                             const float* clip_coef_dev, float lr, float beta1, float beta2, float eps, int step, float ema_decay, int apply_adam,
                             const int* skip_flag_dev, void* stream);
int fc_debug_conv_wgrad(const float* src0, int c0, const float* src1, int c1, const float* dy, int cout, int batch, int hs, int ws, int ksize,
                        int pad, int stride, int upsample, float* dw_out, float* db_out, void* stream);
// ... 90 lines not shown
```

Measured before the change: 919.8 samples/s.

## Fuse final conv, Euler update, and next-step init conv into final resblock tail

Adds a step-closing flavour of the final_res_block's cross-workgroup fused-tail conv. Its epilogue applies final_conv (32→4), performs the Euler update of y, computes the next step's init_conv (4→32) into the x0 buffer, and advances the step and time bookkeeping plus conditioning slices. This removes the separate final_conv and init_conv launches, and the time-setup work, from each Euler step. In exchange it adds a more complex specialised kernel instantiation, a one-time prologue launch, and register and LDS pressure in the epilogue.

```diff
diff --git a/flocoder_amd/_binding.py b/flocoder_amd/_binding.py
--- a/flocoder_amd/_binding.py
+++ b/flocoder_amd/_binding.py
@@ -60,6 +60,7 @@
     "fc_debug_conv_routes": (_i, [_i]),
     "fc_debug_conv_routes_read": (_i, [C.c_char_p, _i]),
     "fc_debug_linattn_routes_read": (_i, [C.c_char_p, _i]),
+    "fc_debug_step_routes_read": (_i, [C.c_char_p, _i]),
     "fc_debug_conv": (_i, [_vp, _i, _vp, _i, _vp, _vp, _vp, _vp, _vp, _i, _pi, _pf, _i, _i, _i, _i, _i, _i, _i, _i, _i, _i, _i, _pf, _vp]),
     "fc_debug_set_fused_tail": (_i, [_i]),
     "fc_unet_fused_tail_errors": (_i, [_vp, C.POINTER(_i)]),
diff --git a/flocoder_amd/csrc/common.h b/flocoder_amd/csrc/common.h
--- a/flocoder_amd/csrc/common.h
+++ b/flocoder_amd/csrc/common.h
@@ -55,6 +55,26 @@
     SrcXform xf;
 };
 
+struct StepCloseHdr {
+    float* y = nullptr;
+    const float* ts = nullptr;
+    float *sc = nullptr, *tvec = nullptr;
+    int *step = nullptr, *evalc = nullptr;
+    const float* ss_all = nullptr;
+    float* ss_dst = nullptr;
+    float dt = 0.f, t_scale = 1.f;
+    int rows = 0, S = 0, n_slices = 0;
+};
+constexpr int kStepDim = 32, kStepCh = 4;
+constexpr int kStepWeights = kStepDim * kStepCh + kStepCh + kStepCh * kStepDim + kStepDim;
+struct StepClose {
+    StepCloseHdr h;
+    float w[kStepWeights];
+    unsigned base[4];
+};
+int step_close_setup_launch(StepClose* blk, const StepCloseHdr& h, const float* fw, const float* fb, const float* iw, const float* ib,
+                            const unsigned* sync, int gsz, hipStream_t s);
+
 struct ConvFin {
     const float* gamma = nullptr;
     const float* beta = nullptr;
@@ -64,6 +84,7 @@
     unsigned* sync = nullptr;
     unsigned long long* gran = nullptr;
     int* err = nullptr;
+    const StepClose* step = nullptr;
 };
 
 struct ConvArgs {
@@ -106,9 +127,11 @@
     int T1 = 0;
     float n_t1 = 0.f;
     int groups = 0;
+    int gsz = 0;
     int fin_local = 0;
 };
 bool conv_fin_possible(const ConvArgs& a, int tile);
+bool conv_step_close_possible(const ConvArgs& a, int tile);
 int conv_init();
 unsigned long long* conv_stamp_buffer();
 void conv_set_stamp_buffer(unsigned long long* p);
@@ -208,6 +231,9 @@
 int linattn_fused_launch(const LaArgs& a, hipStream_t s);
 void linattn_route_log_set(bool on);
 std::string linattn_route_log_get();
+void step_route_log_set(bool on);
+std::string step_route_log_get();
+void step_route_log_add(const char* what);
 bool linattn_fused_meeting_ok(int B, int n, int C);
 int linattn_sample_init();
 bool linattn_sample_supported(int n, int C, int heads);
diff --git a/flocoder_amd/csrc/conv_dev.h b/flocoder_amd/csrc/conv_dev.h
--- a/flocoder_amd/csrc/conv_dev.h
+++ b/flocoder_amd/csrc/conv_dev.h
@@ -88,12 +88,14 @@
     a.stats_out = as_global(a.stats_out); a.res_w = as_global(a.res_w); a.res_b = as_global(a.res_b); a.res_out = as_global(a.res_out);
     a.fin.gamma = as_global(a.fin.gamma); a.fin.beta = as_global(a.fin.beta); a.fin.res = as_global(a.fin.res);
     a.fin.gn1_out = as_global(a.fin.gn1_out); a.fin.sync = as_global(a.fin.sync); a.fin.gran = as_global(a.fin.gran); a.fin.err = as_global(a.fin.err);
+    a.fin.step = as_global(a.fin.step);
     p.zeros16 = as_global(p.zeros16); p.stamps = as_global(p.stamps);
 }
 
 constexpr int FL_FIN = 1, FL_RES = 2, FL_POST = 4, FL_XF = 8, FL_CAT = 16, FL_STAMP = 32, FL_STATS = 64, FL_GN1 = 128, FL_POSTOP = 256,
               FL_NARROW = 512, FL_MULTI = 1024, FL_MEET = 2048, FL_ALL = 4095, FL_W4 = 4096;
 constexpr int FL_WW = 8192;
+constexpr int FL_STEP = 16384;
 constexpr int GEO_PAIR = 1, GEO_FAST = 2;
 constexpr int geo_log2(int v) { return v <= 1 ? 0 : 1 + geo_log2(v >> 1); }
 constexpr int geo_key(int form, int TB, int TW, int cpg, int Tst) { return form | ((TB == 2 ? 1 : 0) << 2) | (geo_log2(TW) << 3) | (geo_log2(cpg) << 6) | (Tst << 10); }
@@ -107,7 +109,8 @@
 template <int WM, int WN, int WK, int MT, int NT, int FL = FL_ALL, int GEO = 0>
 __device__ __forceinline__ void conv_epilogue(const ConvDev& p, f32x16 (&acc)[MT][NT], f32x16 (&accr)[MT][NT], float* smem, int tid, int lane,
                                               int wave, int b0, int y0, int x0, int n0, int tx, int ty, bool active = true,
-                                              int nthr = 256, const float* pre = nullptr, bool staged_dead = false) {
+                                              int nthr = 256, const float* pre = nullptr, bool staged_dead = false,
+                                              const StepCloseHdr* shdr = nullptr) {
     constexpr int BM = 32 * MT * WM, BN = 32 * NT * WN;
     const ConvArgs& a = p.a;
     const int half = lane >> 5, l31 = lane & 31;
@@ -346,6 +349,16 @@
     }
     if (do_stats && !fast_stats && !pair_stats) block_sums();
 
+    constexpr bool STEP = (FL & FL_STEP) != 0;
+    static_assert(!STEP || (GEOC && !GEO1 && (FL & FL_MEET) && !(FL & (FL_GN1 | FL_RES | FL_NARROW)) && WK == 1 && BM == 128 && BN == kStepDim &&
+                            kStepCh == 4 && geo_TB(GEO) == 1 && 2 * (BM / 16) * BN >= kStepWeights),
+                  "the step-closing flavour: final_res_block's closing launch of the dim-32 plan, 512 threads, weights in the dead statistics scratch");
+    const StepClose* sp = STEP ? a.fin.step : nullptr;
+    const StepCloseHdr sh = STEP ? *shdr : StepCloseHdr();
+    const int s_lt = tid - 256, s_m = tid >> 2, s_j = tid & 3;
+    const int s_pix = STEP ? (y0 + ((s_m >> g_TWl) & (TH - 1))) * a.W + x0 + (s_m & (TW - 1)) : 0;
+    float s_y = 0.f, s_w0 = 0.f, s_w1 = 0.f, s_dt = 0.f;
+
     if (FL & FL_STAMP) conv_stamp(p, 7);
     if (do_stats) {
         if (pair_stats) stats_pair(a.stats_out, a.Gout, g_cpg, g_cpgt, g_NPG, meeting, fin && !meeting);
@@ -374,6 +387,26 @@
                         rs[mt][nt][r] = (a.fin.res && nok && px >= 0) ? a.fin.res[(size_t)px * Cout + n] : 0.f;
                     }
                 }
+        }
+        float4 s_cond = make_float4(0.f, 0.f, 0.f, 0.f);
+        float s_t = 0.f;
+        int s_next = 0, s_ci = -1;
+        if constexpr (STEP) {
+            s_next = __float_as_int(smem[p.o_epoch + 1]);
+            s_y = as_global(sh.y)[((size_t)b0 * kStepCh + s_j) * (size_t)(a.H * a.W) + s_pix];
+            s_dt = sh.dt;
+            if (!active) {
+                const float* wq = as_global(sp->w);
+                s_w0 = wq[s_lt];
+                if (s_lt < kStepWeights - 256) s_w1 = wq[256 + s_lt];
+                const int S = sh.S, n4 = S >> 2, per = (n4 + geo_Tst(GEO) - 1) / geo_Tst(GEO);
+                const int i = (ty * p.tiles_x + tx) * per + s_lt;
+                if (s_lt < per && i < n4 && __float_as_int(smem[p.o_epoch + 2])) {
+                    s_ci = i;
+                    s_cond = *reinterpret_cast<const float4*>(as_global(sh.ss_all) + ((size_t)s_next * sh.rows + b0) * (size_t)S + 4 * i);
+                }
+                if (blockIdx.x == 0 && s_lt >= BM) s_t = as_global(sh.ts)[s_next];
+            }
         }
         if (meeting) {
             const int Tst = GEOC ? geo_Tst(GEO) : (p.TB > 1 ? 1 : p.tiles_x * p.tiles_y) * p.NPG;
@@ -421,6 +454,26 @@
             }
         }
         lds_only_barrier();
+        if constexpr (STEP) {
+            if (!active) {
+                float* swl = smem + p.o_part;
+                swl[s_lt] = s_w0;
+                if (s_lt < kStepWeights - 256) swl[256 + s_lt] = s_w1;
+                if (s_ci >= 0) *reinterpret_cast<float4*>(as_global(sh.ss_dst) + (size_t)b0 * (size_t)sh.S + 4 * s_ci) = s_cond;
+                if (blockIdx.x == 0 && s_lt >= BM) {
+                    if (s_lt == BM) {
+                        float* scq = as_global(sh.sc);
+                        scq[0] = s_t;
+                        scq[1] = 0.f;
+                        *as_global(sh.step) = s_next + 1;
+                        *as_global(sh.evalc) = s_next;
+                    }
+                    const float tv = __fmul_rn(s_t, sh.t_scale);
+                    float* tvq = as_global(sh.tvec);
+                    for (int r = s_lt - BM; r < sh.rows; r += 256 - BM) tvq[r] = tv;
+                }
+            }
+        }
         if ((FL & FL_STAMP) && active) conv_stamp(p, 12);
         if (owner) {
 #pragma unroll
@@ -519,6 +572,44 @@
             if (active && !pass) conv_stamp(p, 9);
             lds_only_barrier();
             if (active && !pass) conv_stamp(p, 10);
+            if constexpr (STEP) {
+                {
+                    float* row = ot + s_m * OS;
+                    const float* swl = smem + p.o_part;
+                    float4 xv[kStepDim / 4];
+#pragma unroll
+                    for (int k = 0; k < kStepDim / 4; ++k) xv[k] = *reinterpret_cast<const float4*>(row + 4 * k);
+                    const float* fw = swl + s_j * kStepDim;
+                    float acc1 = swl[kStepCh * kStepDim + s_j];
+#pragma unroll
+                    for (int k = 0; k < kStepDim / 4; ++k) {
+                        const float4 wv = *reinterpret_cast<const float4*>(fw + 4 * k);
+                        acc1 += xv[k].x * wv.x; acc1 += xv[k].y * wv.y; acc1 += xv[k].z * wv.z; acc1 += xv[k].w * wv.w;
+                    }
+                    const float yn = __fadd_rn(s_y, __fmul_rn(acc1, s_dt));
+                    as_global(sh.y)[((size_t)b0 * kStepCh + s_j) * (size_t)(a.H * a.W) + s_pix] = yn;
+                    float y4[kStepCh];
+#pragma unroll
+                    for (int ci = 0; ci < kStepCh; ++ci) y4[ci] = __shfl(yn, (lane & ~3) | ci);
+                    const float* iw = swl + kStepCh * kStepDim + kStepCh;
+                    const float* ib = iw + kStepCh * kStepDim;
+                    float4 o[2];
+#pragma unroll
+                    for (int h = 0; h < 2; ++h) {
+                        const int c = 2 * s_j + h;
+                        o[h] = *reinterpret_cast<const float4*>(ib + 4 * c);
+#pragma unroll
+                        for (int ci = 0; ci < kStepCh; ++ci) {
+                            const float xq = y4[ci];
+                            const float4 wv = *reinterpret_cast<const float4*>(iw + ci * kStepDim + 4 * c);
+                            o[h].x += xq * wv.x; o[h].y += xq * wv.y; o[h].z += xq * wv.z; o[h].w += xq * wv.w;
+                        }
+                    }
+                    *reinterpret_cast<float4*>(row + 8 * s_j) = o[0];
+                    *reinterpret_cast<float4*>(row + 8 * s_j + 4) = o[1];
+                }
+                lds_only_barrier();
+            }
             float* gout = pass ? a.res_out : a.out;
             for (int i = tid; i < BM * Q4; i += nthr) {
                 const int m = i / Q4, c4 = (i - m * Q4) * 4, n = n0 + c4;
@@ -538,6 +629,7 @@
 
 int conv_pipe_launch(const ConvDev& d, int tile, int grid, size_t lds, hipStream_t s);
 int conv_pipe_blocks_per_cu(const ConvDev& d, int tile, size_t lds);
+bool conv_pipe_step_ok(const ConvDev& d, int tile);
 int conv_pipe_init();
 bool conv_pipe_supports_ks(int ks);
 const float* conv_zeros16();
diff --git a/flocoder_amd/csrc/conv_igemm.hip b/flocoder_amd/csrc/conv_igemm.hip
--- a/flocoder_amd/csrc/conv_igemm.hip
+++ b/flocoder_amd/csrc/conv_igemm.hip
@@ -321,7 +321,8 @@
             g->n_t1 = (float)(p.rps * cpgt1);
             p.fin_local = g->fin_local = (g->T == 1) ? 1 : 0;
             if (p.fin_local) p.gsz = 1;
-            else {
+            g->gsz = p.gsz;
+            if (!p.fin_local) {
                 int per_cu = conv_pipe_blocks_per_cu(p, tile, g->lds);
                 if (per_cu <= 0) return fail(FC_E_SHAPE, "conv: fused tail: occupancy of the kernel unknown");
                 if (per_cu > 2) per_cu = 2;
@@ -362,6 +363,18 @@
     return conv_geometry(b, tile, true, &d, &g) == FC_OK;
 }
 
+bool conv_step_close_possible(const ConvArgs& a, int tile) {
+    static StepClose dummy;
+    ConvDev d;
+    ConvGeom g;
+    if (!a.fin.gamma || conv_geometry(a, tile, true, &d, &g) != FC_OK || !conv_pipe_step_ok(d, tile)) return false;
+    d.a.fin.step = &dummy;
+    d.stamps = nullptr;
+    int per_cu = conv_pipe_blocks_per_cu(d, tile, g.lds);
+    if (per_cu > 2) per_cu = 2;
+    return per_cu > 0 && d.nblocks <= conv_cu_count() * per_cu;
+}
+
 static int auto_tile(const ConvArgs& a) {
     const long M = (long)a.B * a.H * a.W;
     const int hw = a.H * a.W;
diff --git a/flocoder_amd/csrc/conv_pipe.hip b/flocoder_amd/csrc/conv_pipe.hip
--- a/flocoder_amd/csrc/conv_pipe.hip
+++ b/flocoder_amd/csrc/conv_pipe.hip
@@ -134,6 +134,13 @@
         const gu32* cnt = (const gu32*)(a.fin.sync + b0 / g_TB);
         asm volatile("global_atomic_add %0, %1, %2, off sc0" : "=v"(arrival) : "v"(cnt), "v"(1u) : "memory");
     }
+    unsigned step_base = 0, step_n = 0;
+    StepCloseHdr step_h;
+    if constexpr ((FL & FL_STEP) != 0) {
+        step_h = a.fin.step->h;
+        step_n = (unsigned)step_h.n_slices;
+        if (tid == 0) step_base = as_global(a.fin.step->base)[b0];
+    }
 
     auto gn_tables = [&](const bool worker, const int id, const int nthr) {
       if (xf_on) {
@@ -495,6 +502,11 @@
         if (meet && tid == 0) {
             asm volatile("s_waitcnt vmcnt(0)" : "+v"(arrival) :: "memory");
             smem[p.o_epoch] = __uint_as_float(arrival / (unsigned)p.gsz + 1u);
+            if constexpr ((FL & FL_STEP) != 0) {
+                const unsigned nxt = min(arrival / (unsigned)p.gsz + 1u - step_base + 1u, step_n);
+                smem[p.o_epoch + 1] = __uint_as_float(nxt);
+                smem[p.o_epoch + 2] = __uint_as_float(nxt < step_n ? 1u : 0u);
+            }
         }
         __syncthreads();
         if (FL & FL_STAMP) conv_stamp(p, 4);
@@ -650,7 +662,7 @@
         if (FL & FL_STAMP) conv_stamp(p, 5);
     }
     if constexpr (WW) loader_handover();
-    conv_epilogue<WM, WN, WK, MT, NT, FL, GEO>(p, acc, accr, smem, tid, lane, wave, b0, y0, x0, n0, tx, ty, consumer, NTHR, pre, true);
+    conv_epilogue<WM, WN, WK, MT, NT, FL, GEO>(p, acc, accr, smem, tid, lane, wave, b0, y0, x0, n0, tx, ty, consumer, NTHR, pre, true, &step_h);
 }
 
 static float* g_zeros16 = nullptr;
@@ -864,6 +876,31 @@
     FC_FIN_GEOMS(X)
 #undef X
     return -1;
+}
+
+constexpr int kStepGeo = geo_key(GEO_FAST, 1, 16, 8, 8), kStepMask = kFinBase | FL_MEET;
+static bool lean_kernels_on() {
+    static const bool lean = [] { const char* e = std::getenv("FLOCODER_AMD_LEAN_KERNELS"); return !(e && std::string(e) == "0"); }();
+    return lean;
+}
+bool conv_pipe_step_ok(const ConvDev& d, int tile) {
+    const ConvArgs& a = d.a;
+    return lean_kernels_on() && tile == TILE_M128N32 && a.KS == 3 && !d.bf3 && d.o_out >= 0 && !a.fin.gn1_out && !a.res_out && !a.stats_post && !a.out_act && !a.add &&
+           !d.fin_local && d.any_xf && !a.out_sh && !a.out_oy && !a.out_ox && a.Cout == kStepDim && d.ntiles == 1 && d.P * (16 / 4) <= 64 * 4 * kLeanNPL &&
+           d.gsz == geo_Tst(kStepGeo) && fin_geo_key(d, 128, 32, 512, false) == kStepGeo;
+}
+static int fin_step_attr() {
+    FC_HIP(hipFuncSetAttribute(reinterpret_cast<const void*>(&conv_pipe_kernel<4, 1, 1, 1, 1, 16, kLeanNPL, 3, 4, kStepMask | FL_STEP, 0, kStepGeo>),
+                               hipFuncAttributeMaxDynamicSharedMemorySize, 160 * 1024));
+    FC_HIP(hipFuncSetAttribute(reinterpret_cast<const void*>(&conv_pipe_kernel<4, 1, 1, 1, 1, 16, kLeanNPL, 3, 4, kStepMask | FL_STEP | FL_STAMP, 0, kStepGeo>),
+                               hipFuncAttributeMaxDynamicSharedMemorySize, 160 * 1024));
+    return FC_OK;
+}
+static int fin_step_launch(const ConvDev& d, int tile, int need, int grid, size_t lds, hipStream_t s, int* occ) {
+    if (!conv_pipe_step_ok(d, tile) || (need & ~FL_STAMP) != kStepMask) return fail(FC_E_STATE, "conv: the launch is not the one the step-closing flavour is compiled for");
+    if (!occ) step_route_log_add("step_close");
+    return (need & FL_STAMP) ? launch_pipe<4, 1, 1, 1, 1, 16, kLeanNPL, 3, 4, kStepMask | FL_STEP | FL_STAMP, 0, kStepGeo>(d, grid, lds, s, occ)
+                             : launch_pipe<4, 1, 1, 1, 1, 16, kLeanNPL, 3, 4, kStepMask | FL_STEP, 0, kStepGeo>(d, grid, lds, s, occ);
 }
 
 constexpr int kConv1Up = FL_STATS | FL_CAT | FL_RES;
@@ -969,6 +1006,7 @@
 #undef X
     FC_TRY((lean_attr<2, 0>()));
     FC_TRY(fin_geom_attr());
+    FC_TRY(fin_step_attr());
     FC_TRY(conv1_geom_attr());
     done = true;
     return FC_OK;
@@ -989,7 +1027,8 @@
 
 static int conv_pipe_dispatch(const ConvDev& d, int tile, int grid, size_t lds, hipStream_t s, int* occ) {
     if (d.bf3) return d.a.KS == 1 ? bf3_launch_ks<1>(d, tile, grid, lds, s, occ) : d.a.KS == 2 ? bf3_launch_ks<2>(d, tile, grid, lds, s, occ) : bf3_launch_ks<3>(d, tile, grid, lds, s, occ);
-    static const bool lean = [] { const char* e = std::getenv("FLOCODER_AMD_LEAN_KERNELS"); return !(e && std::string(e) == "0"); }();
+    const bool lean = lean_kernels_on();
+    if (d.a.fin.step && !(lean && d.a.KS == 3)) return fail(FC_E_STATE, "conv: the step-closing flavour is a lean 3x3 kernel");
     if (lean) {
         const bool small_tile = tile == TILE_M32N32K4;
         const int need = (d.a.fin.gamma ? FL_FIN : 0) | (d.a.res_out ? FL_RES : 0) | (d.a.stats_post ? FL_POST : 0) | (d.any_xf ? FL_XF : 0) |
@@ -1002,7 +1041,8 @@
             const bool w4 = small_tile && d.a.w4 && d.a.Cin % 32 == 0 && d.a.Cout % 32 == 0 && d.a.pad == 1 && !d.a.w_batch_stride &&
                             (!d.a.res_out || d.a.res_w4);
             const size_t lds_ww = (w4 && (need & FL_FIN)) ? ww_lds(d, tile, lds) : 0;
-            if (need & FL_FIN) r = fin_geom_launch(d, tile, w4, need, grid, lds, lds_ww, s, occ);
+            if ((need & FL_FIN) && d.a.fin.step) r = fin_step_launch(d, tile, need, grid, lds, s, occ);
+            else if (need & FL_FIN) r = fin_geom_launch(d, tile, w4, need, grid, lds, lds_ww, s, occ);
             else if (need & FL_STATS) r = conv1_geom_launch(d, tile, w4, need, grid, lds, s, occ);
             if (lds_ww) {
 #define X(F) if (r == -1 && need == (F)) r = lean_launch_ww<(F)>(d, tile, grid, lds_ww, s, occ);
@@ -1049,7 +1089,7 @@
                      ((d.a.out_act || d.a.add) ? FL_POSTOP : 0) | (d.o_out < 0 ? FL_NARROW : 0) | (d.TB > 1 ? FL_MULTI : 0) |
                      ((d.a.fin.gamma && !d.fin_local) ? FL_MEET : 0);
     const int ww = (d.a.KS == 3 && d.a.w4 && ww_lds(d, tile, lds)) ? d.a.Cin : 0;
-    const auto key = std::make_tuple(tile, d.a.KS, mask | (d.a.w4 ? FL_W4 : 0), lds, d.cpg, d.TB * 4096 + (d.TWl << 8) + d.tiles_x * d.tiles_y * d.NPG + (ww << 13));
+    const auto key = std::make_tuple(tile, d.a.KS, mask | (d.a.w4 ? FL_W4 : 0) | (d.a.fin.step ? FL_STEP : 0), lds, d.cpg, d.TB * 4096 + (d.TWl << 8) + d.tiles_x * d.tiles_y * d.NPG + (ww << 13));
     std::lock_guard<std::mutex> lk(mu);
     auto it = cache.find(key);
     if (it != cache.end()) return it->second;
diff --git a/flocoder_amd/csrc/elementwise.hip b/flocoder_amd/csrc/elementwise.hip
--- a/flocoder_amd/csrc/elementwise.hip
+++ b/flocoder_amd/csrc/elementwise.hip
@@ -1,3 +1,6 @@
+#include <mutex>
+#include <string>
+
 #include "common.h"
 #include "stats_dev.h"
 
@@ -207,9 +210,38 @@
     }
 }
 
+static std::mutex g_step_route_mu;
+static bool g_step_route_on = false;
+static std::string g_step_route_log;
+void step_route_log_set(bool on) { std::lock_guard<std::mutex> lk(g_step_route_mu); g_step_route_on = on; if (on) g_step_route_log.clear(); }
+std::string step_route_log_get() { std::lock_guard<std::mutex> lk(g_step_route_mu); return g_step_route_log; }
+void step_route_log_add(const char* what) {
+    std::lock_guard<std::mutex> lk(g_step_route_mu);
+    if (g_step_route_on) g_step_route_log += std::string(what) + "\n";
+}
+
+__global__ void __launch_bounds__(256) step_close_setup_kernel(StepClose* blk, const StepCloseHdr h, const float* fw, const float* fb,
+                                                               const float* iw, const float* ib, const unsigned* sync, int gsz) {
+    const int t = threadIdx.x;
+    if (t == 0) blk->h = h;
+    constexpr int NF = kStepDim * kStepCh, NI = kStepCh * kStepDim;
+    for (int i = t; i < kStepWeights; i += 256)
+        blk->w[i] = i < NF ? fw[(i % kStepDim) * kStepCh + i / kStepDim] : i < NF + kStepCh ? (fb ? fb[i - NF] : 0.f)
+                  : i < NF + kStepCh + NI ? iw[i - NF - kStepCh] : (ib ? ib[i - NF - kStepCh - NI] : 0.f);
+    for (int b = t; b < h.rows; b += 256) blk->base[b] = sync[b] / (unsigned)gsz + 1u;
+}
+
+int step_close_setup_launch(StepClose* blk, const StepCloseHdr& h, const float* fw, const float* fb, const float* iw, const float* ib,
+                            const unsigned* sync, int gsz, hipStream_t s) {
+    hipLaunchKernelGGL(step_close_setup_kernel, dim3(1), dim3(256), 0, s, blk, h, fw, fb, iw, ib, sync, gsz);
+    FC_HIP(hipGetLastError());
+    return FC_OK;
+}
+
 int init_conv_launch(const CondFetch& fetch, const float* x, int bmod, const float* w, const float* bias, float* out, int B, int Cin, int HW,
                      int Cout, hipStream_t s) {
     if (Cout & 3) return fail(FC_E_SHAPE, "init_conv: Cout must be a multiple of 4");
+    step_route_log_add("init_conv");
     const size_t total = (size_t)B * HW * (Cout / 4);
     const int grid = (int)((total + 255) / 256 < 4096 ? (total + 255) / 256 : 4096);
     const int extra = fetch.all ? (fetch.n4 + 255) / 256 < 512 ? (fetch.n4 + 255) / 256 : 512 : 0;
@@ -322,6 +354,7 @@
 int final_conv_launch(const float* x, const float* w, const float* bias, float* out, int B, int Cin, int HW, int Cout, const EulerTail& tail,
                       hipStream_t s) {
     if (Cin & 3) return fail(FC_E_SHAPE, "final_conv: Cin must be a multiple of 4");
+    step_route_log_add("final_conv");
     const size_t total = (size_t)B * HW;
     if (Cout <= 4 && total < (1ull << 31) && (Cin == 8 || Cin == 16 || Cin == 32 || Cin == 64)) {
         const dim3 g((unsigned)((total + 255) / 256));
diff --git a/flocoder_amd/csrc/plan.h b/flocoder_amd/csrc/plan.h
--- a/flocoder_amd/csrc/plan.h
+++ b/flocoder_amd/csrc/plan.h
@@ -36,6 +36,7 @@
     float* dmask_out = nullptr;
     EulerTail euler;
     CondFetch fetch;
+    const StepClose* step = nullptr;
 };
 using Op = std::function<int(const FwdCtx&, hipStream_t)>;
 
@@ -66,6 +67,9 @@
     int n_meet = 0;
     std::vector<unsigned*> fin_sync;
     std::vector<int> fin_kind;
+    StepClose* step_blk = nullptr;
+    const unsigned* step_sync = nullptr;
+    int step_gsz = 0;
     void release() {
         for (void* p : allocs) dev_free(p);
         *this = Plan();
@@ -213,6 +217,7 @@
     int* fin_err_word = nullptr;
     int conv_prec = 0;
     const ParamStore* store = nullptr;
+    Act step_out;
 
     int guard = 0;
     bool param_only = false;
@@ -365,9 +370,19 @@
         a.fin.err = fin_err_word ? fin_err_word : reinterpret_cast<int*>(sync + g.groups);
         if (!g.fin_local) { ++pl->n_meet; pl->fin_sync.push_back(sync); pl->fin_kind.push_back(0); }
         const int tile = g.tile;
+        float* sout = nullptr;
+        if (step_out.p && step_out.C == out.C && step_out.H == out.H && step_out.W == out.W && conv_step_close_possible(a, tile)) {
+            pl->step_blk = reinterpret_cast<StepClose*>(dmalloc(sizeof(StepClose) / sizeof(float) + (size_t)B));
+            if (err) return false;
+            pl->step_sync = sync; pl->step_gsz = g.gsz;
+            sout = step_out.p;
+        }
         const double fl = 2.0 * out.H * out.W * a.KS * a.KS * (double)a.Cin * a.Cout;
-        push([a, tile](const FwdCtx& c, hipStream_t s) { ConvArgs b = a; b.B = c.B; return conv_launch(b, tile, s); }, std::string(kTileNames[tile]) + "+fin", fl,
-             conv_bytes_ps(a), conv_bytes_fixed(a));
+        push([a, tile, sout](const FwdCtx& c, hipStream_t s) {
+            ConvArgs b = a; b.B = c.B;
+            if (c.step && sout) { b.fin.step = c.step; b.out = sout; }
+            return conv_launch(b, tile, s);
+        }, std::string(kTileNames[tile]) + "+fin", fl, conv_bytes_ps(a), conv_bytes_fixed(a));
         return true;
     }
 
diff --git a/flocoder_amd/csrc/unet.hip b/flocoder_amd/csrc/unet.hip
--- a/flocoder_amd/csrc/unet.hip
+++ b/flocoder_amd/csrc/unet.hip
@@ -604,7 +604,7 @@
         float* x0p = x0.p;
         b.scope = "init_conv";
         if (!c.mask_cond) {
-            b.push([=](const FwdCtx& cx, hipStream_t s) { return init_conv_launch(cx.fetch, cx.x, cx.x_mod, w, bias, x0p, cx.B, ch, HW, dim, s); }, "init_conv", 2.0 * HW * ch * dim);
+            b.push([=](const FwdCtx& cx, hipStream_t s) { return cx.step ? (int)FC_OK : init_conv_launch(cx.fetch, cx.x, cx.x_mod, w, bias, x0p, cx.B, ch, HW, dim, s); }, "init_conv", 2.0 * HW * ch * dim);
         } else {
             Act xi = b.act(dim, H, W), f1 = b.act(2 * dim, H, W), f2 = b.act(2 * dim, H, W);
             const bool keep = u->keep_all;
@@ -721,13 +721,15 @@
         pl->named[p + ".3"] = x;
     }
     if (b.err) return b.err;
+    if (!c.mask_cond && dim == kStepDim && ch == kStepCh) b.step_out = x0;
     x = b.resblock("final_res_block", x, &x0, dim, false, nullptr);
+    b.step_out = Act();
     if (b.err) return b.err;
     pl->head = x;
     {
         const float *xp = x.p, *w = u->P("final_conv.weight"), *bias = u->R("final_conv.bias");
         b.scope = "final_conv";
-        b.push([=](const FwdCtx& cx, hipStream_t s) { return final_conv_launch(xp, w, bias, cx.out, cx.B, dim, HW, ch, cx.euler, s); }, "final_conv", 2.0 * HW * dim * ch);
+        b.push([=](const FwdCtx& cx, hipStream_t s) { return cx.step ? (int)FC_OK : final_conv_launch(xp, w, bias, cx.out, cx.B, dim, HW, ch, cx.euler, s); }, "final_conv", 2.0 * HW * dim * ch);
     }
     if (b.err) return b.err;
     pl->maxB = maxB; pl->H = H; pl->W = W;
@@ -1054,7 +1056,12 @@
     return FC_OK;
 }
 
-int fc_debug_conv_routes(int on) { conv_route_log_set(on != 0); linattn_route_log_set(on != 0); return FC_OK; }
+int fc_debug_conv_routes(int on) { conv_route_log_set(on != 0); linattn_route_log_set(on != 0); step_route_log_set(on != 0); return FC_OK; }
+int fc_debug_step_routes_read(char* buf, int cap) {
+    const std::string r = step_route_log_get();
+    if (buf && cap > 0) { const size_t n = r.size() < (size_t)cap - 1 ? r.size() : (size_t)cap - 1; memcpy(buf, r.data(), n); buf[n] = 0; }
+    return (int)r.size();
+}
 int fc_debug_conv_routes_read(char* buf, int cap) {
     const std::string r = conv_route_log_get();
     if (buf && cap > 0) { const size_t n = r.size() < (size_t)cap - 1 ? r.size() : (size_t)cap - 1; memcpy(buf, r.data(), n); buf[n] = 0; }
diff --git a/flocoder_amd/csrc/unet_integrate.hip b/flocoder_amd/csrc/unet_integrate.hip
--- a/flocoder_amd/csrc/unet_integrate.hip
+++ b/flocoder_amd/csrc/unet_integrate.hip
@@ -223,7 +223,29 @@
 
 static bool euler_tail_ok(int method, bool cfg_on) { return method == FC_METHOD_EULER && !cfg_on; }
 
-static int enqueue_step(const CallFrame& f, int method, float cfg, float dt_euler, float t_scale, bool pre_on) {
+static bool step_close_ok(const CallFrame& f, int method, bool pre_on) {
+    const fc_unet* u = f.u;
+    const char* e = std::getenv("FLOCODER_AMD_STEP_CLOSE");
+    if (e && std::strcmp(e, "0") == 0) return false;
+    return euler_tail_ok(method, f.cfg_on) && pre_on && f.mask_mode == 0 && u->plan.step_blk != nullptr && u->S % 4 == 0 &&
+           u->S / 4 <= 256 * u->plan.step_gsz;
+}
+
+static int step_close_prologue(const CallFrame& f, float dt_euler, float t_scale, int n_steps) {
+    fc_unet* u = f.u;
+    const IntegratorState& ig = u->ig;
+    StepCloseHdr h;
+    h.y = ig.y; h.ts = ig.ts_dev; h.sc = ig.sc; h.tvec = ig.tvec; h.step = ig.step; h.evalc = ig.step + 1;
+    h.ss_all = ig.pre_ss; h.ss_dst = u->plan.ss; h.dt = dt_euler; h.t_scale = t_scale;
+    h.rows = f.rows; h.S = u->S; h.n_slices = n_steps;
+    const float *iw = u->P("init_conv.weight"), *ib = u->R("init_conv.bias");
+    FC_TRY(step_close_setup_launch(u->plan.step_blk, h, u->P("final_conv.weight"), u->R("final_conv.bias"), iw, ib, u->plan.step_sync,
+                                   u->plan.step_gsz, f.s));
+    const FwdCtx c = step_ctx(f, true);
+    return init_conv_launch(c.fetch, ig.y, f.B, iw, ib, u->plan.x0.p, f.rows, u->cfg.channels, u->H * u->W, u->cfg.dim, f.s);
+}
+
+static int enqueue_step(const CallFrame& f, int method, float cfg, float dt_euler, float t_scale, bool pre_on, bool step_close = false) {
     fc_unet* u = f.u;
     const IntegratorState& ig = u->ig;
     const bool cfg_on = f.cfg_on;
@@ -235,6 +257,7 @@
         c.x = ig.y;
         c.euler.y = ig.y; c.euler.dt = dt_euler; c.euler.step = ig.step; c.euler.ts = ig.ts_dev; c.euler.t_scale = t_scale;
         c.euler.sc = ig.sc; c.euler.tvec = ig.tvec; c.euler.rows = rows;
+        if (step_close) c.step = u->plan.step_blk;
         return run_plan(u->plan, c, s);
     }
     FC_TRY(ode_time_launch(ig.step, ig.ts_dev, t_scale, 0, ig.sc, ig.tvec, rows, s));
@@ -346,8 +369,10 @@
         FC_TRY(ode_time_launch(ig.step, ig.ts_dev, t_scale, 0, ig.sc, ig.tvec, rows, s));
     GraphKey key = graph_key(f, method == FC_METHOD_RK4 ? GraphKey::Rk4 : GraphKey::Euler, cfg_strength, t_scale);
     key.pre_on = pre_on; key.dt_euler = fbits(dt_euler);
+    const bool step_close = key.step_close = step_close_ok(f, method, pre_on);
+    if (step_close) FC_TRY(step_close_prologue(f, dt_euler, t_scale, n_steps));
     FC_TRY(replay_steps(f, key, n_steps, method == FC_METHOD_RK4 ? 4 : 1,
-                        [&] { return enqueue_step(f, method, cfg_strength, dt_euler, t_scale, pre_on); }));
+                        [&] { return enqueue_step(f, method, cfg_strength, dt_euler, t_scale, pre_on, step_close); }));
     return f.finish(x_dev);
 }
 
diff --git a/flocoder_amd/csrc/unet_priv.h b/flocoder_amd/csrc/unet_priv.h
--- a/flocoder_amd/csrc/unet_priv.h
+++ b/flocoder_amd/csrc/unet_priv.h
@@ -13,13 +13,14 @@
     int B = 0, mask_mode = 0;
     bool cfg_on = false, has_ids = false;
     bool pre_on = false;
+    bool step_close = false;
     int steps = 0;
     bool dense = false;
     uint32_t cfg_strength = 0, dt_euler = 0, t_scale = 0;
     int sde_scheme = 0, sde_noise = 0;
     uint32_t sde_sigma = 0;
     auto tie() const {
-        return std::tie(kind, B, mask_mode, cfg_on, has_ids, pre_on, steps, dense, cfg_strength, dt_euler, t_scale, sde_scheme, sde_noise,
+        return std::tie(kind, B, mask_mode, cfg_on, has_ids, pre_on, step_close, steps, dense, cfg_strength, dt_euler, t_scale, sde_scheme, sde_noise,
                         sde_sigma);
     }
     bool operator<(const GraphKey& o) const { return tie() < o.tie(); }
diff --git a/include/flocoder_amd.h b/include/flocoder_amd.h
--- a/include/flocoder_amd.h
+++ b/include/flocoder_amd.h
@@ -165,6 +165,7 @@
 int fc_debug_conv_routes(int on);
 int fc_debug_conv_routes_read(char* buf, int cap);
 int fc_debug_linattn_routes_read(char* buf, int cap);
+int fc_debug_step_routes_read(char* buf, int cap);
 int fc_debug_set_stamp_op(int op_index, void* buf_dev);
 int fc_debug_set_conv_precision(int mode);
 int fc_debug_conv(const float* src0_nhwc, int c0, const float* src1_nhwc, int c1, const float* w_oihw_dev, const float* bias_dev,
```

New measurement: 929.6 samples/s (median of 6 runs). 1.1% higher.
